# ZenGo-X/multi-party-ecdsa

Measured on AMD Instinct MI355X. Metric: GG20 signatures/sec (t=1, n=3; all parties of each session on the node's GPUs) + Paillier-2048 modexp/s per GPU, higher is better.
Workload: dtype u32 limbs (radix 2^29) / u64 accumulators

## Files before the change

multi_party_ecdsa_amd/csrc/mpe_gg20.h:

```cpp
#pragma once
#include <cstdio>
#include <cstdlib>

#include "mpe_gg20_msg.h"
#include "mpe_proofs.h"

namespace mpe {
namespace smp {
struct Bounds { uint32_t *q, *q3, *Nm2, *qNt, *q3Nt; };
__global__ void bounds_kernel(int count, const uint32_t* __restrict__ N, const uint32_t* __restrict__ Nt, Bounds b) {
  const int g = blockIdx.x * blockDim.x + threadIdx.x;
  if (g > count) return;
  const uint32_t q[8] = {0xD0364141u, 0xBFD25E8Cu, 0xAF48A03Bu, 0xBAAEDCE6u, 0xFFFFFFFEu, 0xFFFFFFFFu, 0xFFFFFFFFu, 0xFFFFFFFFu};
  uint32_t q2[16], q3[24];
  sm::mul(q2, q, 8, q, 8);
  sm::mul(q3, q2, 16, q, 8);
  if (g == count) {
    for (int j = 0; j < 8; ++j) b.q[j] = q[j];
    for (int j = 0; j < 24; ++j) b.q3[j] = q3[j];
    return;
  }
  const uint32_t two[1] = {2u};
  sm::sub(b.Nm2 + (size_t)g * 64, 64, N + (size_t)g * 64, 64, two, 1);
  sm::mul(b.qNt + (size_t)g * 72, Nt + (size_t)g * 64, 64, q, 8);
  sm::mul(b.q3Nt + (size_t)g * 88, Nt + (size_t)g * 64, 64, q3, 24);
}
}
}

struct mpe_gg20_keys {
  int t = 0, n = 0, S = 0, K = 1, n_own = 0;
  int signers[8] = {0};
  int nsets = 1;
  uint32_t sets4[256] = {0};
  uint32_t masks[256] = {0};
  uint32_t* d_sets = nullptr;
  int own[8] = {0};
  int own_slot[8] = {0};
  mpe_paillier* pub = nullptr;
  mpe_paillier* prv = nullptr;
  mpe_statements* stm = nullptr;
  void* blob = nullptr;
  size_t blob_bytes = 0;
  uint32_t* x = nullptr;
  uint32_t* X = nullptr;
  uint32_t* y = nullptr;
  uint32_t* gw = nullptr;
  mpe::smp::Bounds bounds{};
};

namespace mpe {
namespace gg {

struct Dim {
  int B, S, n, L, V, PV, K, n_own;
  int loc[8];
  int sg[8];
  int oslot[8];
  const int32_t* ks;
  ec::Enc enc;
  const int32_t* ss;
  const uint32_t* sets;
  uint32_t sg4;
  int nsets;
  int lparty;
};
__device__ __forceinline__ int ind_of(int i, int jj) { return jj < i ? jj : jj + 1; }
__device__ __forceinline__ int jme_of(int i, int ind) { return i < ind ? i : i - 1; }
__device__ __forceinline__ int ks_of(const Dim& d, int b) { return d.ks ? d.ks[b] : 0; }
__device__ __forceinline__ bool ss_valid(const Dim& d, int b) { return !d.ss || (unsigned)d.ss[b] < (unsigned)d.nsets; }
__device__ __forceinline__ int ss_of(const Dim& d, int b) { return d.ss && ss_valid(d, b) ? d.ss[b] : 0; }
__device__ __forceinline__ uint32_t set4_of(const Dim& d, int b) { return d.ss ? d.sets[ss_of(d, b)] : d.sg4; }
__device__ __forceinline__ int sg_of(const Dim& d, int b, int i) { return (int)((set4_of(d, b) >> (4 * i)) & 15u); }
__device__ __forceinline__ int rank_in(uint32_t set4, int S, int party) {
  int r = -1;
  for (int i = 0; i < S; ++i) if ((int)((set4 >> (4 * i)) & 15u) == party) r = i;
  return r;
}
__device__ __forceinline__ int loc_of(const Dim& d, int b, int li) {
  if (d.lparty < 0) return d.loc[li];
  const int r = rank_in(set4_of(d, b), d.S, d.lparty);
  return r < 0 ? 0 : r;
}
__device__ __forceinline__ int kpub(const Dim& d, int b, int i) { return ks_of(d, b) * d.n + sg_of(d, b, i); }
__device__ __forceinline__ int kown(const Dim& d, int b, int i) { return ks_of(d, b) * d.n_own + d.oslot[d.lparty >= 0 ? d.lparty : sg_of(d, b, i)]; }
__device__ __forceinline__ const uint32_t* gw_of(const Dim& d, const uint32_t* gw, int b, int ind) {
  return gw + (((size_t)ks_of(d, b) * d.nsets + ss_of(d, b)) * d.S + ind) * 16;
}

struct Slab { const uint32_t* p; long long off[8]; int W; };
__device__ __forceinline__ long long rec_index(const Slab& s, int j, int b) { return s.off[j] + b; }
__device__ __forceinline__ const uint32_t* rec_of(const Slab& s, int j, int b) { return s.p + (size_t)(s.off[j] + b) * (size_t)s.W; }

struct Idx {
  int32_t *kown_pi;
  int32_t *pi_ap, *kown_ap, *st_ap;
  int32_t *ca_vi, *kpub_vi, *st_vi;
  int32_t *ca_mb, *kpub_mb, *kown_mb;
  int32_t *pi_pp, *kown_pp, *st_pp;
  int32_t *ca_pv, *pi_pv, *kpub_pv, *st_pv;
};
__global__ void idx_kernel(Dim d, Idx x, int total) {
  const int g = blockIdx.x * blockDim.x + threadIdx.x;
  if (g >= total) return;
  const int S = d.S, n = d.n, L = d.L, P1 = S - 1;
  if (g < d.B * L) { const int b = g / L; x.kown_pi[g] = kown(d, b, loc_of(d, b, g % L)); }
  if (g < d.B * L * n) {
    const int pi = g / n, b = pi / L;
    x.pi_ap[g] = pi; x.kown_ap[g] = kown(d, b, loc_of(d, b, pi % L)); x.st_ap[g] = ks_of(d, b) * n + g % n;
  }
  if (g < d.B * L * P1 * d.V * n) {
    const int st = g % n, r1 = g / n, r2 = r1 / d.V, jj = r2 % P1, pi = r2 / P1, b = pi / L, i = loc_of(d, b, pi % L);
    const int ind = ind_of(i, jj);
    x.ca_vi[g] = ind * d.B + b; x.kpub_vi[g] = kpub(d, b, ind); x.st_vi[g] = ks_of(d, b) * n + st;
  }
  if (g < d.B * L * P1 * 2) {
    const int pp = g >> 1, jj = pp % P1, pi = pp / P1, b = pi / L, i = loc_of(d, b, pi % L), ind = ind_of(i, jj);
    x.ca_mb[g] = ind * d.B + b; x.kpub_mb[g] = kpub(d, b, ind); x.kown_mb[g] = kown(d, b, i);
  }
  if (g < d.B * L * P1) {
    const int jj = g % P1, pi = g / P1, b = pi / L, i = loc_of(d, b, pi % L);
    x.pi_pp[g] = pi; x.kown_pp[g] = kown(d, b, i); x.st_pp[g] = ks_of(d, b) * n + sg_of(d, b, ind_of(i, jj));
  }
  if (g < d.B * d.PV * S * P1) {
    const int jj = g % P1, r1 = g / P1, i = r1 % S, r2 = r1 / S, vl = r2 % d.PV, b = r2 / d.PV;
    x.ca_pv[g] = i * d.B + b; x.pi_pv[g] = b * L + vl; x.kpub_pv[g] = kpub(d, b, i);
    x.st_pv[g] = ks_of(d, b) * n + sg_of(d, b, ind_of(i, jj));
  }
}

__global__ void gather_field_kernel(Slab s, int S, int B, int src_off, int words, uint32_t* __restrict__ dst) {
  MPE_FOREGROUND();
  const size_t g = (size_t)blockIdx.x * blockDim.x + threadIdx.x;
  if (g >= (size_t)S * B * words) return;
  const int w = (int)(g % words);
  const size_t jb = g / words;
  dst[g] = rec_of(s, (int)(jb / B), (int)(jb % B))[src_off + w];
}
constexpr int NR = 9;
__device__ __forceinline__ void fail(int32_t* status, uint32_t* bad, int pi, int code, uint32_t mask) {
  if (status[pi] == 0) { status[pi] = code; bad[pi] = mask; }
}
__device__ __forceinline__ int resolve_status(const int32_t* status, size_t nPI, int pi, int upto, const uint32_t* bad, uint32_t* bad_out) {
  for (int r = 0; r <= upto; ++r) {
    const int st = status[(size_t)r * nPI + pi];
    if (st) { if (bad_out) *bad_out = bad[(size_t)r * nPI + pi]; return st; }
  }
  if (bad_out) *bad_out = 0;
  return 0;
}

__global__ void pack_field_kernel(int nitems, int per, int L, int B, int nsub, int sub0, int subw, int dst_off,
                                  const uint32_t* __restrict__ src, int words, const int32_t* __restrict__ status, int round,
                                  uint32_t* __restrict__ out) {
  MPE_FOREGROUND();
  const size_t g = (size_t)blockIdx.x * blockDim.x + threadIdx.x;
  if (g >= (size_t)nitems * words) return;
  const int w = (int)(g % words), item = (int)(g / words), pi = item / per, li = pi % L, b = pi / L;
  const bool stopped = resolve_status(status, (size_t)L * B, pi, round, nullptr, nullptr) != 0;
  out[((size_t)(li * B + b) * nsub + sub0 + item % per) * subw + dst_off + w] = stopped ? 0u : src[g];
}
__device__ __forceinline__ bool pt_ok(const uint32_t* p) { return ec::aff_valid(ec::aff_load(p)); }
__global__ void __launch_bounds__(64) validate_kernel(Dim d, Slab in, int round, int32_t* __restrict__ status, uint32_t* __restrict__ bad) {
  MPE_FOREGROUND();
  const int pi = blockIdx.x * blockDim.x + threadIdx.x;
  if (pi >= d.B * d.L) return;
  const int b = pi / d.L, i = loc_of(d, b, pi % d.L), P1 = d.S - 1;
  uint32_t mask = 0;
  for (int j = 0; j < d.S; ++j) {
    if (j == i) continue;
    const uint32_t* m = rec_of(in, j, b);
    bool good = true;
    if (round == 2) {
      for (int v = 0; v < 2; ++v) {
        const uint32_t* mb = m + (size_t)(jme_of(i, j) * 2 + v) * SUB1;
        good = good && pt_ok(mb + M1.b_pk.off) && pt_ok(mb + M1.b_R.off) && pt_ok(mb + M1.bt_pk.off) && pt_ok(mb + M1.bt_R.off);
      }
    } else if (round == 3) {
      good = pt_ok(m + M2.T.off) && pt_ok(m + M2.a1.off) && pt_ok(m + M2.a2.off) && pt_ok(m + M2.com.off);
    } else if (round == 4) {
      good = pt_ok(m + M3.g_gamma.off);
    } else if (round == 5) {
      for (int jj = 0; jj < P1; ++jj) good = good && pt_ok(m + (size_t)jj * SUB4 + M4P.u1.off);
      good = good && pt_ok(m + (size_t)P1 * SUB4 + M4R.R_dash.off);
    } else if (round == 6) {
      good = pt_ok(m + M5.S.off) && pt_ok(m + M5.T.off) && pt_ok(m + M5.A3.off);
    }
    if (!good) mask |= 1u << j;
  }
  if (mask) fail(status, bad, pi, 100 * round + 90, mask);
}

__device__ inline ec::U256 lagrange0(const int* sg, int S, int i) {
  ec::U256 num = ec::u256_one(), den = ec::u256_one();
  for (int j = 0; j < S; ++j) {
    if (j == i) continue;
    ec::U256 xj = ec::u256_zero(); xj.w[0] = (uint32_t)(sg[j] + 1);
    ec::U256 xi = ec::u256_zero(); xi.w[0] = (uint32_t)(sg[i] + 1);
    num = ec::sc_mul(num, xj);
    den = ec::sc_mul(den, ec::sc_sub(xj, xi));
  }
  return ec::sc_mul(num, ec::sc_inv(den));
}
__device__ inline ec::U256 lagrange0(uint32_t set4, int S, int i) {
  ec::U256 num = ec::u256_one(), den = ec::u256_one();
  ec::U256 xi = ec::u256_zero(); xi.w[0] = ((set4 >> (4 * i)) & 15u) + 1u;
  for (int j = 0; j < S; ++j) {
    if (j == i) continue;
    ec::U256 xj = ec::u256_zero(); xj.w[0] = ((set4 >> (4 * j)) & 15u) + 1u;
    num = ec::sc_mul(num, xj);
    den = ec::sc_mul(den, ec::sc_sub(xj, xi));
  }
  return ec::sc_mul(num, ec::sc_inv(den));
}
__global__ void __launch_bounds__(64) MPE_EC_OCC gw_kernel(Dim d, const uint32_t* __restrict__ Xs, uint32_t* __restrict__ gw) {
  const int g = blockIdx.x * blockDim.x + threadIdx.x;
  if (g >= d.K * d.nsets * d.S) return;
  const int kk = g / (d.nsets * d.S), j = g % d.S;
  const uint32_t set4 = d.sets[(g / d.S) % d.nsets];
  ec::aff_store(gw + (size_t)g * 16, ec::mul_aff(lagrange0(set4, d.S, j), ec::aff_load(Xs + ((size_t)kk * d.n + ((set4 >> (4 * j)) & 15u)) * 16)));
}

__global__ void __launch_bounds__(64) MPE_EC_OCC r0_kernel(Dim d, const uint32_t* __restrict__ xs, const uint32_t* __restrict__ k_in,
                          const uint32_t* __restrict__ gamma_in, const uint32_t* __restrict__ blind, uint32_t* __restrict__ kq,
                          uint32_t* __restrict__ gq, uint32_t* __restrict__ w, uint32_t* __restrict__ k64, uint32_t* __restrict__ g_gamma,
                          uint32_t* __restrict__ com, int32_t* __restrict__ status, uint32_t* __restrict__ bad) {
  const int pi = blockIdx.x * blockDim.x + threadIdx.x;
  if (pi >= d.B * d.L) return;
  const int b = pi / d.L, i = loc_of(d, b, pi % d.L);
  if (!ss_valid(d, b) || (d.lparty >= 0 && rank_in(set4_of(d, b), d.S, d.lparty) < 0)) fail(status, bad, pi, MPE_GG20_STATUS_BAD_SET, 0);
  const bool k_ok = ec::sc_is_canonical_nonzero(k_in + (size_t)pi * 8), g_ok = ec::sc_is_canonical_nonzero(gamma_in + (size_t)pi * 8);
  if (!k_ok || !g_ok) fail(status, bad, pi, MPE_GG20_STATUS_BAD_NONCE, 0);
  const ec::U256 k = ec::sc_reduce(k_in + (size_t)pi * 8, 8), g = ec::sc_reduce(gamma_in + (size_t)pi * 8, 8);
  const ec::U256 wi = ec::sc_mul(lagrange0(set4_of(d, b), d.S, i), ec::sc_reduce(xs + (size_t)kown(d, b, i) * 8, 8));
  ec::u256_store(kq + (size_t)pi * 8, k);
  ec::u256_store(gq + (size_t)pi * 8, g);
  ec::u256_store(w + (size_t)pi * 8, wi);
  for (int j = 0; j < 64; ++j) k64[(size_t)pi * 64 + j] = j < 8 ? k.w[j] : 0u;
  const ec::Aff gg = ec::jac_to_aff(ec::jac_mul_gen(g));
  ec::aff_store(g_gamma + (size_t)pi * 16, gg);
  ec::u256_store(com + (size_t)pi * 8, sig::commit_point(gg, blind + (size_t)pi * 8, d.enc));
}

__global__ void idx1_kernel(Dim d, Slab in0, int32_t* __restrict__ sub0_vi) {
  const int g = blockIdx.x * blockDim.x + threadIdx.x;
  const int P1 = d.S - 1;
  if (g >= d.B * d.L * P1 * d.V * d.n) return;
  const int st = g % d.n, r1 = g / d.n, r2 = r1 / d.V, jj = r2 % P1, pi = r2 / P1, b = pi / d.L, i = loc_of(d, b, pi % d.L);
  sub0_vi[g] = (int32_t)(rec_index(in0, ind_of(i, jj), b) * (d.n + 1) + st);
}
__global__ void mb_prep_kernel(Dim d, const uint32_t* __restrict__ gq, const uint32_t* __restrict__ w,
                               const uint32_t* __restrict__ beta_tag, uint32_t* __restrict__ bsel,
                               uint32_t* __restrict__ btq, uint32_t* __restrict__ beta) {
  const int mb = blockIdx.x * blockDim.x + threadIdx.x;
  if (mb >= d.B * d.L * (d.S - 1) * 2) return;
  const int pi = (mb >> 1) / (d.S - 1);
  const uint32_t* src = (mb & 1) ? w + (size_t)pi * 8 : gq + (size_t)pi * 8;
  for (int j = 0; j < 8; ++j) bsel[(size_t)mb * 8 + j] = src[j];
  const ec::U256 t = ec::sc_reduce(beta_tag + (size_t)mb * 64, 64);
  ec::u256_store(btq + (size_t)mb * 8, t);
  ec::u256_store(beta + (size_t)mb * 8, ec::sc_neg(t));
}
__global__ void status1_kernel(Dim d, const uint8_t* __restrict__ ok_vi, int32_t* __restrict__ status, uint32_t* __restrict__ bad) {
  const int pi = blockIdx.x * blockDim.x + threadIdx.x;
  if (pi >= d.B * d.L) return;
  const int per = (d.S - 1) * d.V * d.n;
  bool good = true;
  for (int q = 0; q < per; ++q) good = good && ok_vi[(size_t)pi * per + q];
  if (!good) fail(status, bad, pi, 101, 0);
}

__global__ void idx2_kernel(Dim d, Slab in1, int32_t* __restrict__ sub1_rv) {
  MPE_FOREGROUND();
  const int g = blockIdx.x * blockDim.x + threadIdx.x;
  const int P1 = d.S - 1;
  if (g >= d.B * d.L * P1 * 2) return;
  const int v = g & 1, pp = g >> 1, jj = pp % P1, pi = pp / P1, b = pi / d.L, i = loc_of(d, b, pi % d.L), ind = ind_of(i, jj);
  sub1_rv[g] = (int32_t)(rec_index(in1, ind, b) * (2 * P1) + jme_of(i, ind) * 2 + v);
}
__device__ __forceinline__ void r2a_finish(const Dim& d, int rv, int v, int pp, int b, int ind, const ec::Aff& Bpk, bool good,
                                           const uint32_t* gw, uint32_t* bpk_in, uint8_t* code) {
  uint8_t c = good ? 0 : 1;
  if (v == 1) { if (!c && !ec::aff_eq(Bpk, ec::aff_load(gw_of(d, gw, b, ind)))) c = 2; }
  else ec::aff_store(bpk_in + (size_t)pp * 16, Bpk);
  code[rv] = c;
}
__global__ void __launch_bounds__(64) MPE_EC_OCC r2a_kernel(Dim d, const int32_t* __restrict__ sub1_rv, const uint32_t* __restrict__ in1,
                           const uint32_t* __restrict__ alpha_full, const uint32_t* __restrict__ kq, const uint32_t* __restrict__ gw,
                           uint32_t* __restrict__ alpha, uint32_t* __restrict__ bpk_in, uint8_t* __restrict__ code) {
  MPE_FOREGROUND();
  const int rv = blockIdx.x * blockDim.x + threadIdx.x;
  const int P1 = d.S - 1;
  if (rv >= d.B * d.L * P1 * 2) return;
  const int v = rv & 1, pp = rv >> 1, jj = pp % P1, pi = pp / P1, b = pi / d.L, i = loc_of(d, b, pi % d.L), ind = ind_of(i, jj);
  const uint32_t* m = in1 + (size_t)sub1_rv[rv] * SUB1;
  const ec::U256 al = ec::sc_reduce(alpha_full + (size_t)rv * 64, 64);
  ec::u256_store(alpha + (size_t)rv * 8, al);
  const ec::Aff Bpk = ec::aff_load(m + M1.b_pk.off), BTpk = ec::aff_load(m + M1.bt_pk.off);
  const ec::Aff R1 = ec::aff_load(m + M1.b_R.off), R2 = ec::aff_load(m + M1.bt_R.off);
  const bool good = sig::mta_alpha_holds(al, ec::u256_load(kq + (size_t)pi * 8), Bpk, R1, ec::sc_reduce(m + M1.b_z.off, 8), BTpk, R2,
                                         ec::sc_reduce(m + M1.bt_z.off, 8), d.enc);
  r2a_finish(d, rv, v, pp, b, ind, Bpk, good, gw, bpk_in, code);
}

__global__ void __launch_bounds__(64) MPE_EC_OCC ped_ahead_kernel(Dim d, const uint32_t* __restrict__ l_in, const uint32_t* __restrict__ s1_in,
                                                       const uint32_t* __restrict__ s2_in, uint32_t* __restrict__ ped_pre) {
  const int pi = blockIdx.x * blockDim.x + threadIdx.x;
  if (pi >= d.B * d.L) return;
  uint32_t* o = ped_pre + (size_t)pi * 48;
  ec::aff_store(o, ec::jac_to_aff(ec::jac_mul_h2(ec::sc_reduce(l_in + (size_t)pi * 8, 8))));
  ec::aff_store(o + 16, ec::jac_to_aff(ec::jac_mul_gen(ec::sc_reduce(s1_in + (size_t)pi * 8, 8))));
  ec::aff_store(o + 32, ec::jac_to_aff(ec::jac_mul_h2(ec::sc_reduce(s2_in + (size_t)pi * 8, 8))));
}
struct Ped { uint32_t *T, *e, *a1, *a2, *z1, *z2; };
__global__ void __launch_bounds__(64) MPE_EC_OCC r2b_kernel(Dim d, const uint32_t* __restrict__ kq, const uint32_t* __restrict__ gq,
                           const uint32_t* __restrict__ w, const uint32_t* __restrict__ alpha,
                           const uint32_t* __restrict__ beta, const uint8_t* __restrict__ code, const uint32_t* __restrict__ l_in,
                           const uint32_t* __restrict__ s1_in, const uint32_t* __restrict__ s2_in,
                           uint32_t* __restrict__ delta_i, uint32_t* __restrict__ sigma_i, uint32_t* __restrict__ lq, Ped p,
                           int32_t* __restrict__ status, uint32_t* __restrict__ bad, const uint32_t* __restrict__ alpha_full,
                           uint32_t* __restrict__ miu, int fault_step, uint32_t fault_mask, const uint32_t* __restrict__ ped_pre) {
  MPE_FOREGROUND();
  const int pi = blockIdx.x * blockDim.x + threadIdx.x;
  if (pi >= d.B * d.L) return;
  const int P1 = d.S - 1;
  for (int jj = 0; jj < P1; ++jj)
    for (int w_ = 0; w_ < 64; ++w_) miu[((size_t)pi * P1 + jj) * 64 + w_] = alpha_full[(((size_t)pi * P1 + jj) * 2 + 1) * 64 + w_];
  const ec::U256 k = ec::u256_load(kq + (size_t)pi * 8);
  ec::U256 de = ec::sc_mul(k, ec::u256_load(gq + (size_t)pi * 8)), si = ec::sc_mul(k, ec::u256_load(w + (size_t)pi * 8));
  int st = 0;
  for (int jj = 0; jj < P1; ++jj) {
    const size_t m0 = ((size_t)pi * P1 + jj) * 2;
    de = ec::sc_add(de, ec::sc_add(ec::u256_load(alpha + m0 * 8), ec::u256_load(beta + m0 * 8)));
    si = ec::sc_add(si, ec::sc_add(ec::u256_load(alpha + (m0 + 1) * 8), ec::u256_load(beta + (m0 + 1) * 8)));
    for (int v = 0; v < 2 && !st; ++v) if (code[m0 + v]) st = 200 + code[m0 + v];
  }
  if (st) fail(status, bad, pi, st, 0);
  if ((fault_mask >> loc_of(d, pi / d.L, pi % d.L)) & 1u) {
    if (fault_step == 5) de = ec::sc_add(de, de);
    if (fault_step == 6) si = ec::sc_add(si, si);
  }
  ec::u256_store(delta_i + (size_t)pi * 8, de);
  ec::u256_store(sigma_i + (size_t)pi * 8, si);
  const ec::U256 l = ec::sc_reduce(l_in + (size_t)pi * 8, 8);
  ec::u256_store(lq + (size_t)pi * 8, l);
  const uint32_t* pre = ped_pre ? ped_pre + (size_t)pi * 48 : nullptr;
  const ec::Aff T = ec::jac_to_aff(ec::jac_add(ec::jac_mul_gen(si), pre ? ec::jac_from_aff(ec::aff_load(pre)) : ec::jac_mul_h2(l)));
  const ec::U256 s1 = ec::sc_reduce(s1_in + (size_t)pi * 8, 8), s2 = ec::sc_reduce(s2_in + (size_t)pi * 8, 8);
  const ec::Aff a1 = pre ? ec::aff_load(pre + 16) : ec::jac_to_aff(ec::jac_mul_gen(s1)), a2 = pre ? ec::aff_load(pre + 32) : ec::jac_to_aff(ec::jac_mul_h2(s2));
  ec::U256 e, z1, z2;
  sig::pedersen_prove_body(si, l, s1, s2, T, a1, a2, d.enc, e, z1, z2);
  ec::aff_store(p.T + (size_t)pi * 16, T);
  ec::u256_store(p.e + (size_t)pi * 8, e);
  ec::aff_store(p.a1 + (size_t)pi * 16, a1);
  ec::aff_store(p.a2 + (size_t)pi * 16, a2);
  ec::u256_store(p.z1 + (size_t)pi * 8, z1);
  ec::u256_store(p.z2 + (size_t)pi * 8, z2);
}

__device__ __forceinline__ bool words_eq(const uint32_t* a, const uint32_t* b, int n) {
  uint32_t o = 0;
  for (int i = 0; i < n; ++i) o |= a[i] ^ b[i];
  return o == 0;
}
__device__ __forceinline__ void r3_finish(int pi, bool com_ok, bool ped_ok, const ec::U256& sum, uint32_t* dinv, int32_t* status,
                                          uint32_t* bad) {
  if (!com_ok) fail(status, bad, pi, 303, 0);
  const bool inv_ok = !ec::u256_is_zero(sum);
  if (!inv_ok) fail(status, bad, pi, 301, 0);
  ec::u256_store(dinv + (size_t)pi * 8, inv_ok ? ec::sc_inv(sum) : ec::u256_zero());
  if (!ped_ok) fail(status, bad, pi, 302, 0);
}
__global__ void __launch_bounds__(64) MPE_EC_OCC r3_kernel(Dim d, Slab in2, uint32_t* __restrict__ dinv, int32_t* __restrict__ status,
                                                uint32_t* __restrict__ bad) {
  MPE_FOREGROUND();
  const int pi = blockIdx.x * blockDim.x + threadIdx.x;
  if (pi >= d.B * d.L) return;
  const int b = pi / d.L;
  ec::U256 sum = ec::u256_zero();
  bool com_ok = true, ped_ok = true;
  for (int j = 0; j < d.S; ++j) {
    const uint32_t* m = rec_of(in2, j, b);
    sum = ec::sc_add(sum, ec::sc_reduce(m + M2.delta.off, 8));
    com_ok = com_ok && words_eq(m + M2.T.off, m + M2.com.off, M2.T.words);
    const ec::Aff C = ec::aff_load(m + M2.com.off), a1 = ec::aff_load(m + M2.a1.off), a2 = ec::aff_load(m + M2.a2.off);
    const bool holds = sig::pedersen_verify_body(C, a1, a2, ec::sc_reduce(m + M2.z1.off, 8), ec::sc_reduce(m + M2.z2.off, 8), d.enc);
    ped_ok = ped_ok && holds;
  }
  r3_finish(pi, com_ok, ped_ok, sum, dinv, status, bad);
}

__global__ void __launch_bounds__(64) MPE_EC_OCC r4_kernel(Dim d, Slab in3, const uint32_t* __restrict__ dinv, const uint32_t* __restrict__ com_all,
                          const uint32_t* __restrict__ bpk_in, const uint32_t* __restrict__ kq, uint32_t* __restrict__ R,
                          uint32_t* __restrict__ Rbar, int32_t* __restrict__ status, uint32_t* __restrict__ bad, int with_rbar) {
  MPE_FOREGROUND();
  const int pi = blockIdx.x * blockDim.x + threadIdx.x;
  if (pi >= d.B * d.L) return;
  const int P1 = d.S - 1, b = pi / d.L, i = loc_of(d, b, pi % d.L);
  uint32_t mask = 0;
  for (int jj = 0; jj < P1; ++jj) {
    const int ind = ind_of(i, jj);
    const uint32_t* m = rec_of(in3, ind, b);
    const ec::Aff gg = ec::aff_load(m + M3.g_gamma.off);
    bool good = ec::aff_eq(ec::aff_load(bpk_in + ((size_t)pi * P1 + jj) * 16), gg);
    good = good && ec::u256_eq(sig::commit_point(gg, m + M3.blind.off, d.enc), ec::u256_load(com_all + ((size_t)ind * d.B + b) * 8));
    if (!good) mask |= 1u << ind;
  }
  if (mask) fail(status, bad, pi, 401, mask);
  ec::Jac acc = ec::jac_inf();
  for (int j = 0; j < d.S; ++j) acc = ec::jac_add(acc, ec::jac_from_aff(ec::aff_load(rec_of(in3, j, b) + M3.g_gamma.off)));
  const ec::Aff Rp = ec::mul_aff(ec::u256_load(dinv + (size_t)pi * 8), ec::jac_to_aff(acc));
  ec::aff_store(R + (size_t)pi * 16, Rp);
  if (with_rbar) ec::aff_store(Rbar + (size_t)pi * 16, ec::mul_aff(ec::u256_load(kq + (size_t)pi * 8), Rp));
}
__global__ void __launch_bounds__(64) MPE_EC_OCC r4_rbar_kernel(Dim d, const uint32_t* __restrict__ kq, const uint32_t* __restrict__ R, uint32_t* __restrict__ Rbar) {
  MPE_FOREGROUND();
  const int pi = blockIdx.x * blockDim.x + threadIdx.x;
  if (pi >= d.B * d.L) return;
  ec::aff_store(Rbar + (size_t)pi * 16, ec::mul_aff(ec::u256_load(kq + (size_t)pi * 8), ec::aff_load(R + (size_t)pi * 16)));
}

__global__ void idx5_kernel(Dim d, Slab in4, int32_t* __restrict__ sub4_pv, int32_t* __restrict__ rdash_pv) {
  const int g = blockIdx.x * blockDim.x + threadIdx.x;
  const int P1 = d.S - 1;
  if (g >= d.B * d.PV * d.S * P1) return;
  const int jj = g % P1, r1 = g / P1, i = r1 % d.S, b = r1 / d.S / d.PV;
  const long long r = rec_index(in4, i, b) * d.S;
  sub4_pv[g] = (int32_t)(r + jj); rdash_pv[g] = (int32_t)(r + P1);
}
struct Heg { uint32_t *S, *T, *A3, *z1, *z2; };
__global__ void __launch_bounds__(64) MPE_EC_OCC r5_status_kernel(Dim d, Slab in4, const uint8_t* __restrict__ pdl_ok, int32_t* __restrict__ status,
                                                       uint32_t* __restrict__ bad) {
  const int pi = blockIdx.x * blockDim.x + threadIdx.x;
  if (pi >= d.B * d.L) return;
  const int P1 = d.S - 1, li = pi % d.L, b = pi / d.L;
  const int vo = d.PV == 1 ? 0 : li;
  uint32_t mask = 0;
  for (int i = 0; i < d.S && !mask; ++i)
    for (int jj = 0; jj < P1; ++jj)
      if (!pdl_ok[(((size_t)b * d.PV + vo) * d.S + i) * P1 + jj]) mask = 1u << i;
  if (mask) fail(status, bad, pi, 501, mask);
  ec::Jac acc = ec::jac_inf();
  for (int j = 0; j < d.S; ++j) acc = ec::jac_add(acc, ec::jac_from_aff(ec::aff_load(rec_of(in4, j, b) + (size_t)P1 * SUB4 + M4R.R_dash.off)));
  if (!ec::jac_eq_aff(acc, ec::aff_gen())) fail(status, bad, pi, 502, 0);
}
__global__ void __launch_bounds__(64) MPE_EC_OCC r5_prove_kernel(Dim d, const uint32_t* __restrict__ R, const uint32_t* __restrict__ sigma_i,
                          const uint32_t* __restrict__ lq, const uint32_t* __restrict__ pedT, const uint32_t* __restrict__ s1_in,
                          const uint32_t* __restrict__ s2_in, Heg h) {
  const int pi = blockIdx.x * blockDim.x + threadIdx.x;
  if (pi >= d.B * d.L) return;
  const ec::Aff G = ec::aff_gen(), H = ec::aff_h2();
  const ec::Aff Rp = ec::aff_load(R + (size_t)pi * 16), T = ec::aff_load(pedT + (size_t)pi * 16);
  const ec::U256 si = ec::u256_load(sigma_i + (size_t)pi * 8), l = ec::u256_load(lq + (size_t)pi * 8);
  const ec::Aff Sp = ec::mul_aff(si, Rp);
  const ec::U256 s1 = ec::sc_reduce(s1_in + (size_t)pi * 8, 8), s2 = ec::sc_reduce(s2_in + (size_t)pi * 8, 8);
  ec::Aff TT, A3;
  ec::U256 z1, z2;
  sig::heg_prove_body<sig::VAR, sig::H2, sig::GEN>(l, si, s1, s2, Rp, H, G, T, Sp, d.enc, TT, A3, z1, z2);
  ec::aff_store(h.S + (size_t)pi * 16, Sp);
  ec::aff_store(h.T + (size_t)pi * 16, TT);
  ec::aff_store(h.A3 + (size_t)pi * 16, A3);
  ec::u256_store(h.z1 + (size_t)pi * 8, z1);
  ec::u256_store(h.z2 + (size_t)pi * 8, z2);
}

__global__ void __launch_bounds__(64) MPE_EC_OCC r6_kernel(Dim d, Slab in5, const uint32_t* __restrict__ R, const uint32_t* __restrict__ tvec,
                          const uint32_t* __restrict__ y, int32_t* __restrict__ status, uint32_t* __restrict__ bad) {
  const int pi = blockIdx.x * blockDim.x + threadIdx.x;
  if (pi >= d.B * d.L) return;
  const int b = pi / d.L;
  const ec::Aff G = ec::aff_gen(), H = ec::aff_h2(), Rp = ec::aff_load(R + (size_t)pi * 16);
  uint32_t mask = 0;
  ec::Jac acc = ec::jac_inf();
  for (int j = 0; j < d.S; ++j) {
    const uint32_t* m = rec_of(in5, j, b);
    const ec::Aff E = ec::aff_load(m + M5.S.off), TT = ec::aff_load(m + M5.T.off), A3 = ec::aff_load(m + M5.A3.off),
                  D = ec::aff_load(tvec + ((size_t)j * d.B + b) * 16);
    if (!sig::heg_verify_body<sig::VAR, sig::H2, sig::GEN>(Rp, H, G, D, E, TT, A3, ec::sc_reduce(m + M5.z1.off, 8), ec::sc_reduce(m + M5.z2.off, 8), d.enc))
      mask |= 1u << j;
    acc = ec::jac_add_aff(acc, E);
  }
  if (mask) fail(status, bad, pi, 601, mask);
  if (!ec::jac_eq_aff(acc, ec::aff_load(y + (size_t)ks_of(d, b) * 16))) fail(status, bad, pi, 602, 0);
}

struct JacSlots { ec::Jac v[64]; };

__global__ void __launch_bounds__(64) MPE_EC_OCC r2a_group_kernel(Dim d, const int32_t* __restrict__ sub1_rv, const uint32_t* __restrict__ in1,
                           const uint32_t* __restrict__ alpha_full, const uint32_t* __restrict__ kq, const uint32_t* __restrict__ gw,
                           uint32_t* __restrict__ alpha, uint32_t* __restrict__ bpk_in, uint8_t* __restrict__ code) {
  MPE_FOREGROUND();
  __shared__ JacSlots vs, fs;
  const int gid = blockIdx.x * 64 + threadIdx.x, rv = gid >> 2, sub = gid & 3, base = (int)threadIdx.x - sub;
  const int P1 = d.S - 1;
  const bool live = rv < d.B * d.L * P1 * 2;
  const int rvc = live ? rv : 0;
  const int v = rvc & 1, pp = rvc >> 1, jj = pp % P1, pi = pp / P1, b = pi / d.L, i = loc_of(d, b, pi % d.L), ind = ind_of(i, jj);
  const uint32_t* m = in1 + (size_t)sub1_rv[rvc] * SUB1;
  const ec::U256 al = ec::sc_reduce(alpha_full + (size_t)rvc * 64, 64);
  const ec::Aff Bpk = ec::aff_load(m + M1.b_pk.off), BTpk = ec::aff_load(m + M1.bt_pk.off);
  const ec::Aff R1 = ec::aff_load(m + M1.b_R.off), R2 = ec::aff_load(m + M1.bt_R.off);
  ec::Jac res = ec::jac_inf(), fr = ec::jac_inf();
  if (live && sub < 3) {
    const ec::U256 sc = sub == 0 ? ec::u256_load(kq + (size_t)pi * 8) : (sub == 1 ? sig::dlog_challenge(R1, Bpk, d.enc) : sig::dlog_challenge(R2, BTpk, d.enc));
    res = ec::jac_mul(sc, sub == 2 ? BTpk : Bpk);
    const ec::U256 fk = sub == 0 ? al : ec::sc_reduce(m + (sub == 1 ? M1.b_z.off : M1.bt_z.off), 8);
    fr = ec::jac_mul_gen(fk);
  }
  vs.v[threadIdx.x] = res;
  fs.v[threadIdx.x] = fr;
  __syncthreads();
  if (!live || sub) return;
  ec::u256_store(alpha + (size_t)rv * 8, al);
  const bool good = sig::mta_relation_holds(fs.v[base], vs.v[base], BTpk)
                    && sig::dlog_holds(fs.v[base + 1], vs.v[base + 1], R1) && sig::dlog_holds(fs.v[base + 2], vs.v[base + 2], R2);
  r2a_finish(d, rv, v, pp, b, ind, Bpk, good, gw, bpk_in, code);
}

__global__ void __launch_bounds__(64) MPE_EC_OCC r3_group_kernel(Dim d, int G, Slab in2, uint32_t* __restrict__ dinv, int32_t* __restrict__ status,
                                                      uint32_t* __restrict__ bad) {
  MPE_FOREGROUND();
  __shared__ JacSlots vs, fs;
  const int gid = blockIdx.x * 64 + threadIdx.x, pi = gid / G, sub = gid % G, base = (int)threadIdx.x - sub;
  const bool live = pi < d.B * d.L;
  const int b = live ? pi / d.L : 0;
  ec::Jac res = ec::jac_inf(), fr = ec::jac_inf();
  if (live && sub < d.S) {
    const uint32_t* m = rec_of(in2, sub, b);
    const ec::Aff C = ec::aff_load(m + M2.com.off), a1 = ec::aff_load(m + M2.a1.off), a2 = ec::aff_load(m + M2.a2.off);
    res = ec::jac_mul(sig::pedersen_challenge(C, a1, a2, d.enc), C);
  }
  if (live && sub < 2 * d.S) {
    const uint32_t* m = rec_of(in2, sub >> 1, b);
    fr = ec::jac_mul_fixed(ec::sc_reduce(m + ((sub & 1) ? M2.z2.off : M2.z1.off), 8), sub & 1);
  }
  vs.v[threadIdx.x] = res;
  fs.v[threadIdx.x] = fr;
  __syncthreads();
  if (!live || sub) return;
  ec::U256 sum = ec::u256_zero();
  bool com_ok = true, ped_ok = true;
  for (int j = 0; j < d.S; ++j) {
    const uint32_t* m = rec_of(in2, j, b);
    sum = ec::sc_add(sum, ec::sc_reduce(m + M2.delta.off, 8));
    com_ok = com_ok && words_eq(m + M2.T.off, m + M2.com.off, M2.T.words);
    const ec::Aff a1 = ec::aff_load(m + M2.a1.off), a2 = ec::aff_load(m + M2.a2.off);
    const bool holds = sig::pedersen_holds(fs.v[base + 2 * j], fs.v[base + 2 * j + 1], vs.v[base + j], a1, a2);
    ped_ok = ped_ok && holds;
  }
  r3_finish(pi, com_ok, ped_ok, sum, dinv, status, bad);
}

__global__ void __launch_bounds__(64) MPE_EC_OCC r6_group_kernel(Dim d, int G, Slab in5, const uint32_t* __restrict__ R, const uint32_t* __restrict__ tvec,
                          const uint32_t* __restrict__ y, int32_t* __restrict__ status, uint32_t* __restrict__ bad) {
  __shared__ JacSlots vs, fs;
  const int gid = blockIdx.x * 64 + threadIdx.x, pi = gid / G, sub = gid % G, base = (int)threadIdx.x - sub;
  const bool live = pi < d.B * d.L;
  const int pic = live ? pi : 0, b = pic / d.L;
  const ec::Aff Gp = ec::aff_gen(), H = ec::aff_h2(), Rp = ec::aff_load(R + (size_t)pic * 16);
  ec::Jac res = ec::jac_inf(), fr = ec::jac_inf();
  if (live && sub < 3 * d.S) {
    const int j = sub / 3, kind = sub % 3;
    const uint32_t* m = rec_of(in5, j, b);
    const ec::Aff E = ec::aff_load(m + M5.S.off), TT = ec::aff_load(m + M5.T.off), A3 = ec::aff_load(m + M5.A3.off),
                  D = ec::aff_load(tvec + ((size_t)j * d.B + b) * 16);
    const ec::U256 e = sig::heg_challenge(TT, A3, Rp, H, Gp, D, E, d.enc);
    res = ec::jac_mul(kind == 1 ? ec::sc_reduce(m + M5.z2.off, 8) : e, kind == 0 ? D : (kind == 1 ? Rp : E));
  }
  if (live && sub < 2 * d.S) {
    const uint32_t* m = rec_of(in5, sub >> 1, b);
    fr = ec::jac_mul_fixed(ec::sc_reduce(m + ((sub & 1) ? M5.z2.off : M5.z1.off), 8), (sub & 1) ? 0 : 1);
  }
  vs.v[threadIdx.x] = res;
  fs.v[threadIdx.x] = fr;
  __syncthreads();
  if (!live || sub) return;
  uint32_t mask = 0;
  ec::Jac acc = ec::jac_inf();
  for (int j = 0; j < d.S; ++j) {
    const uint32_t* m = rec_of(in5, j, b);
    const ec::Aff E = ec::aff_load(m + M5.S.off), TT = ec::aff_load(m + M5.T.off), A3 = ec::aff_load(m + M5.A3.off);
    if (!sig::heg_holds(fs.v[base + 2 * j], fs.v[base + 2 * j + 1], vs.v[base + 3 * j], TT, vs.v[base + 3 * j + 1], vs.v[base + 3 * j + 2], A3))
      mask |= 1u << j;
    acc = ec::jac_add_aff(acc, E);
  }
  if (mask) fail(status, bad, pi, 601, mask);
  if (!ec::jac_eq_aff(acc, ec::aff_load(y + (size_t)ks_of(d, b) * 16))) fail(status, bad, pi, 602, 0);
}

__global__ void __launch_bounds__(64) MPE_EC_OCC r7_kernel(Dim d, const uint32_t* __restrict__ msg, const uint32_t* __restrict__ R,
                          const uint32_t* __restrict__ kq, const uint32_t* __restrict__ sigma_i, uint32_t* __restrict__ mq,
                          uint32_t* __restrict__ rq, uint32_t* __restrict__ s_i, int fault_step, uint32_t fault_mask) {
  const int pi = blockIdx.x * blockDim.x + threadIdx.x;
  if (pi >= d.B * d.L) return;
  const int b = pi / d.L;
  const ec::U256 m = ec::sc_reduce(msg + (size_t)b * 8, 8), r = ec::sc_reduce(R + (size_t)pi * 16, 8);
  ec::u256_store(mq + (size_t)pi * 8, m);
  ec::u256_store(rq + (size_t)pi * 8, r);
  ec::U256 si = ec::sc_add(ec::sc_mul(m, ec::u256_load(kq + (size_t)pi * 8)), ec::sc_mul(r, ec::u256_load(sigma_i + (size_t)pi * 8)));
  if (fault_step == 7 && ((fault_mask >> loc_of(d, b, pi % d.L)) & 1u)) si = ec::sc_add(si, si);
  ec::u256_store(s_i + (size_t)pi * 8, si);
}
__device__ __forceinline__ bool output_signature_check(ec::U256& s, int& recid, const ec::U256& m, const ec::U256& r, const ec::U256& ry,
                                                       const uint32_t* y16) {
  recid = (int)(ry.w[0] & 1u);
  const ec::U256 neg = ec::sc_neg(s);
  {
    bool gt = false;
    for (int j = 7; j >= 0; --j) { if (s.w[j] != neg.w[j]) { gt = s.w[j] > neg.w[j]; break; } }
    if (gt) { s = neg; recid ^= 1; }
  }
  bool okv = !ec::u256_is_zero(s);
  if (okv) {
    const ec::U256 bi = ec::sc_inv(s), u1 = ec::sc_mul(m, bi), u2 = ec::sc_mul(r, bi);
    const ec::Aff V = ec::jac_to_aff(ec::jac_add(ec::jac_mul_gen(u1), ec::jac_mul(u2, ec::aff_load(y16))));
    okv = !V.inf && ec::u256_eq(ec::sc_reduce(V.x.w, 8), r);
  }
  return okv;
}
__global__ void __launch_bounds__(64) MPE_EC_OCC complete_kernel(Dim d, Slab in6, const uint32_t* __restrict__ R, const uint32_t* __restrict__ mq,
                          const uint32_t* __restrict__ rq, const uint32_t* __restrict__ s_i, const uint32_t* __restrict__ y,
                          int32_t* __restrict__ status, uint32_t* __restrict__ bad, uint32_t* __restrict__ r_out,
                          uint32_t* __restrict__ s_out, int32_t* __restrict__ recid_out) {
  const int pi = blockIdx.x * blockDim.x + threadIdx.x;
  if (pi >= d.B * d.L) return;
  const int li = pi % d.L, b = pi / d.L, i = loc_of(d, b, li);
  ec::U256 s = ec::u256_load(s_i + (size_t)pi * 8);
  for (int j = 0; j < d.S; ++j) if (j != i) s = ec::sc_add(s, ec::sc_reduce(rec_of(in6, j, b) + M7.s_i.off, 8));
  const ec::U256 m = ec::u256_load(mq + (size_t)pi * 8), r = ec::u256_load(rq + (size_t)pi * 8);
  const ec::U256 ry = ec::sc_reduce(R + (size_t)pi * 16 + 8, 8);
  int recid;
  const bool okv = output_signature_check(s, recid, m, r, ry, y + (size_t)ks_of(d, b) * 16);
  const size_t nPI = (size_t)d.B * d.L;
  if (!okv) fail(status + 8 * nPI, bad + 8 * nPI, pi, 701, 0);
  const bool good = resolve_status(status, nPI, pi, NR - 1, nullptr, nullptr) == 0;
  const size_t o = (size_t)li * d.B + b;
  ec::u256_store(r_out + o * 8, good ? r : ec::u256_zero());
  ec::u256_store(s_out + o * 8, good ? s : ec::u256_zero());
  recid_out[o] = good ? recid : 0;
}
__global__ void result_kernel(Dim d, const int32_t* __restrict__ status, const uint32_t* __restrict__ bad, const uint32_t* __restrict__ R,
                              int32_t* __restrict__ st_out, uint32_t* __restrict__ bad_out, uint32_t* __restrict__ R_out) {
  const int pi = blockIdx.x * blockDim.x + threadIdx.x;
  if (pi >= d.B * d.L) return;
  const size_t o = (size_t)(pi % d.L) * d.B + pi / d.L;
  uint32_t bm = 0;
  const int stv = resolve_status(status, (size_t)d.B * d.L, pi, NR - 1, bad, &bm);
  if (st_out) st_out[o] = stv;
  if (bad_out) bad_out[o] = bm;
  if (R_out) for (int j = 0; j < 16; ++j) R_out[o * 16 + j] = R[(size_t)pi * 16 + j];
}
__global__ void sign_finish_kernel(int B, int L, int b0, const int32_t* __restrict__ pst, const uint32_t* __restrict__ pr,
                                   const uint32_t* __restrict__ ps, const int32_t* __restrict__ prec, const uint32_t* __restrict__ pR,
                                   uint32_t* __restrict__ r_out, uint32_t* __restrict__ s_out, int32_t* __restrict__ recid_out,
                                   uint32_t* __restrict__ R_out, int32_t* __restrict__ status) {
  const int b = blockIdx.x * blockDim.x + threadIdx.x;
  if (b >= B) return;
  int st = 0;
  for (int li = 0; li < L; ++li) { const int s = pst[(size_t)li * B + b]; if (s && (!st || s < st)) st = s; }
  const size_t o = (size_t)b0 + b;
  for (int j = 0; j < 8; ++j) { r_out[o * 8 + j] = st ? 0u : pr[(size_t)b * 8 + j]; s_out[o * 8 + j] = st ? 0u : ps[(size_t)b * 8 + j]; }
  recid_out[o] = st ? 0 : prec[b];
  if (R_out) for (int j = 0; j < 16; ++j) R_out[o * 16 + j] = pR[(size_t)b * 16 + j];
  status[o] = st;
}

enum class PdlStage { idle, first_queued, ready };
struct Ahead {
  bool lockstep = false;
  uint32_t* cinv = nullptr;
  uint8_t* cinv_ok = nullptr; bool cinv_done = false;
  uint32_t* ped = nullptr;
  uint32_t *pdl_bn = nullptr, *pdl_scratch = nullptr;
  PdlStage pdl = PdlStage::idle;
};

}
}

struct mpe_gg20_session {
  mpe_ctx* ctx = nullptr;
  const mpe_gg20_keys* K = nullptr;
  int B = 0, L = 0, dedup = 0, next_round = 0;
  bool any_set = false;
  bool failed = false;
  mpe::gg::Dim d{};
  mpe_gg20_nonces Z{};
  void* mem = nullptr;
  size_t mem_bytes = 0;
  bool from_cache = false;
  mpe::gg::Idx ix{};
  uint32_t *kq = nullptr, *gq = nullptr, *w = nullptr, *k64 = nullptr, *g_gamma = nullptr, *com = nullptr, *c_a = nullptr, *beta = nullptr;
  uint32_t *ca_all = nullptr, *com_all = nullptr, *bpk_in = nullptr, *delta_i = nullptr, *sigma_i = nullptr, *lq = nullptr, *pedT = nullptr;
  uint32_t *tvec = nullptr, *dinv = nullptr, *R = nullptr, *Rbar = nullptr, *mq = nullptr, *rq = nullptr, *s_i = nullptr, *bad = nullptr;
  uint32_t *sig_r = nullptr, *sig_s = nullptr;
  uint32_t* miu = nullptr;
  int32_t *status = nullptr, *sig_recid = nullptr;
  int32_t *sub0_vi = nullptr, *sub4_pv = nullptr, *rdash_pv = nullptr;
  uint8_t *ok_vi = nullptr, *ok_pv = nullptr;
  mpe::gg::Ahead ahead{};
  int fault_step = 0;
  uint32_t fault_mask = 0;
  char* tmp = nullptr;
  size_t tmp_bytes = 0;
};

namespace mpe {
namespace gg {

static void gg_trace(const mpe_ctx* ctx, hipStream_t st, const char* what, int rc) {
  if (!ctx->gg20_trace) return;
  const hipError_t e = hipStreamSynchronize(st);
  fprintf(stderr, "[gg20] %-28s rc=%d sync=%s\n", what, rc, hipGetErrorString(e));
  fflush(stderr);
}
#define GG_LAUNCH(kernel, nitems, ...)                                                                   \
  do {                                                                                                    \
    if (rc == MPE_OK && (nitems) > 0)                                                                     \
      hipLaunchKernelGGL(kernel, dim3(blocks_for((int)(nitems), 64)), dim3(64), 0, st, __VA_ARGS__);      \
    gg_trace(s->ctx, st, #kernel, rc);                                                                            \
  } while (0)

static Counts counts_of(const Dim& d) { return counts_of(d.B, d.S, d.n, d.L, d.V, d.PV); }
static void dim_of_keys(Dim& d, const mpe_gg20_keys* K, const int32_t* d_keyset, const int32_t* d_sigset) {
  d.S = K->S; d.n = K->n; d.K = K->K; d.n_own = K->n_own; d.ks = d_keyset;
  d.ss = d_sigset; d.sets = K->d_sets; d.sg4 = K->sets4[0]; d.nsets = K->nsets; d.lparty = -1;
  for (int i = 0; i < 8; ++i) { d.sg[i] = K->signers[i]; d.oslot[i] = K->own_slot[i] < 0 ? 0 : K->own_slot[i]; }
}
static int local_parties(Dim& d, const mpe_gg20_keys* K, int n_local, const int32_t* h_local, const int32_t* d_sigset, int by_party) {
  if (n_local < 1 || n_local > K->S || !h_local) return MPE_E_ARG;
  d.L = n_local;
  for (int i = 0; i < 8; ++i) d.loc[i] = 0;
  if (by_party) {
    if (n_local != 1) { mpe_set_error_msg("gg20: one local party by index"); return MPE_E_ARG; }
    const int p = h_local[0];
    if (p < 0 || p >= K->n || K->own_slot[p] < 0) { mpe_set_error_msg("gg20: the local party's secrets are not in the key object"); return MPE_E_ARG; }
    if (d_sigset) { d.lparty = p; return MPE_OK; }
    for (int i = 0; i < K->S; ++i) if (K->signers[i] == p) { d.loc[0] = i; return MPE_OK; }
    mpe_set_error_msg("gg20: the local party is not a signer"); return MPE_E_ARG;
  }
  for (int i = 0; i < n_local; ++i) {
    if (h_local[i] < 0 || h_local[i] >= K->S || (i && h_local[i] <= h_local[i - 1])) return MPE_E_ARG;
    d.loc[i] = h_local[i];
    for (int k = 0; k < (d_sigset ? K->nsets : 1); ++k)
      if (K->own_slot[(K->sets4[k] >> (4 * h_local[i])) & 15u] < 0) { mpe_set_error_msg("gg20: a local party's secrets are not in the key object"); return MPE_E_ARG; }
  }
  return MPE_OK;
}
static bool small_batch(const mpe_ctx* ctx, size_t items) { return ctx->allow_par && items <= (size_t)ctx->par_items; }
static size_t ec_lanes_fit(const mpe_ctx* ctx) { return ctx->ec_lane_groups ? (size_t)ctx->cus * 4 * 64 * 2 / ctx->device_share : 0; }
static size_t layout(mpe_gg20_session* s, char* base) {
  const Dim& d = s->d;
  const Counts c = counts_of(d);
  Bump m(base);
  Idx& x = s->ix;
  x.kown_pi = m.i(c.nPI);
  x.pi_ap = m.i(c.nAP); x.kown_ap = m.i(c.nAP); x.st_ap = m.i(c.nAP);
  x.ca_vi = m.i(c.nVI); x.kpub_vi = m.i(c.nVI); x.st_vi = m.i(c.nVI);
  x.ca_mb = m.i(c.nMB); x.kpub_mb = m.i(c.nMB); x.kown_mb = m.i(c.nMB);
  x.pi_pp = m.i(c.nPP); x.kown_pp = m.i(c.nPP); x.st_pp = m.i(c.nPP);
  x.ca_pv = m.i(c.nPV); x.pi_pv = m.i(c.nPV); x.kpub_pv = m.i(c.nPV); x.st_pv = m.i(c.nPV);
  s->kq = m.w(c.nPI * 8); s->gq = m.w(c.nPI * 8); s->w = m.w(c.nPI * 8); s->k64 = m.w(c.nPI * 64);
  s->g_gamma = m.w(c.nPI * 16); s->com = m.w(c.nPI * 8); s->c_a = m.w(c.nPI * 128); s->beta = m.w(c.nMB * 8);
  s->ca_all = m.w(c.SB * 128); s->com_all = m.w(c.SB * 8); s->bpk_in = m.w(c.nPP * 16);
  s->delta_i = m.w(c.nPI * 8); s->sigma_i = m.w(c.nPI * 8); s->lq = m.w(c.nPI * 8); s->pedT = m.w(c.nPI * 16);
  s->tvec = m.w(c.SB * 16); s->dinv = m.w(c.nPI * 8); s->R = m.w(c.nPI * 16); s->Rbar = m.w(c.nPI * 16);
  s->mq = m.w(c.nPI * 8); s->rq = m.w(c.nPI * 8); s->s_i = m.w(c.nPI * 8); s->bad = m.w(c.nPI * NR);
  s->sig_r = m.w(c.nPI * 8); s->sig_s = m.w(c.nPI * 8); s->miu = m.w(c.nPP * 64);
  s->status = m.i(c.nPI * NR); s->sig_recid = m.i(c.nPI);
  s->sub0_vi = m.i(c.nVI); s->ok_vi = m.f(c.nVI); s->sub4_pv = m.i(c.nPV); s->rdash_pv = m.i(c.nPV); s->ok_pv = m.f(c.nPV);
  Ahead& a = s->ahead; const bool small = small_batch(s->ctx, c.nVI);
  a.cinv = small ? m.w(c.nVI * 128) : nullptr; a.cinv_ok = small ? m.f(c.nVI) : nullptr;
  a.ped = m.w(c.nPI * 48);
  a.pdl_bn = small ? m.w(c.nPP * 128) : nullptr; a.pdl_scratch = small ? m.w(modexp_nn_scratch_words(c.nPP)) : nullptr;
  s->tmp_bytes = tmp_bytes_of(c);
  s->tmp = (char*)m.take(s->tmp_bytes);
  return m.off;
}
static Slab slab_of(const mpe_gg20_session* s, const uint32_t* p, const int64_t* h_off, int round) {
  Slab sl;
  sl.p = p; sl.W = msg_words(s->d.S, s->d.n, round);
  for (int j = 0; j < 8; ++j) sl.off[j] = j < s->d.S ? (h_off ? (long long)h_off[j] : (long long)j * s->B) : 0;
  return sl;
}
static int round_enter(mpe_gg20_session* s, int round, const void* in, const void* out, bool need_in, bool need_out) {
  if (!s || (need_in && !in) || (need_out && !out)) return MPE_E_ARG;
  if (s->failed) { mpe_set_error_msg("gg20: a round call of this batch failed (or the batch was aborted): re-arm the session"); return MPE_E_ARG; }
  if (s->next_round != round) { mpe_set_error_msg("gg20: rounds must be run in order"); return MPE_E_ARG; }
  s->d.enc = s->ctx->enc;
  return MPE_OK;
}
static int round_exit(mpe_gg20_session* s, int rc, const char* what) {
  if (rc != MPE_OK) { s->failed = true; return rc; }
  const hipError_t e = hipGetLastError();
  if (e != hipSuccess) { s->failed = true; mpe_set_error(what, e); return MPE_E_HIP; }
  s->next_round++;
  return MPE_OK;
}
#define STAT(r) (s->status + (size_t)(r) * c.nPI)
#define BADR(r) (s->bad + (size_t)(r) * c.nPI)
#define PACK(nitems, per, nsub, sub0, subw, field, src)                                                                                 \
  GG_LAUNCH(pack_field_kernel, (size_t)(nitems) * (field).words, (int)(nitems), (int)(per), d.L, d.B, (int)(nsub), (int)(sub0), (int)(subw),   \
            (field).off, (const uint32_t*)(src), (field).words, s->status, s->next_round, d_out)

static bool round1_merges(const mpe_ctx* ctx, const Counts& c) {
  const bool par = small_batch(ctx, c.nVI);
  const size_t resident_groups = (size_t)ctx->cus * ctx->modexp_waves_per_cu * 16 / ctx->device_share;
  return ctx->merge_r1 && ctx->use_pair && ctx->use_multiexp && c.nVI > 0 && c.nMB > 0 && c.nVI + c.nMB < ((size_t)1 << 30) &&
         (!par || 4 * (c.nVI + c.nMB) > (size_t)ctx->merge_r1_quarters * resident_groups);
}
__global__ void ca_all_from_local_kernel(int S, int B, const uint32_t* __restrict__ c_a, uint32_t* __restrict__ ca_all) {
  const size_t g = (size_t)blockIdx.x * blockDim.x + threadIdx.x;
  if (g >= (size_t)S * B * 128) return;
  const int w = (int)(g % 128);
  const size_t jb = g / 128;
  const int ind = (int)(jb / B), b = (int)(jb % B);
  ca_all[g] = c_a[((size_t)b * S + ind) * 128 + w];
}
static size_t ws_need_inversion_ahead(const mpe_paillier* pk, size_t nVI) { return nVI * (128 + 128 + 1) * 4 + modinv_ws_words(pk->ms_nn, (int)nVI) * 4 + 16384; }

static bool pdl_ahead_eligible(const mpe_gg20_session* s, const Counts& c) {
  const mpe_ctx* ctx = s->ctx; const Ahead& a = s->ahead;
  return a.lockstep && a.pdl_bn && ctx->use_prio && !ctx->no_pdl_ahead && ctx->use_pair && ctx->use_crt && ctx->use_pown && c.nPP > 0 && small_batch(ctx, c.nPP);
}
static int pdl_ahead_queue(mpe_gg20_session* s, const Counts& c, bool finish) {
  mpe_ctx* ctx = s->ctx; const mpe_paillier* prv = s->K->prv; Ahead& a = s->ahead; hipStream_t sa = ctx->aux[1];
  const int phase = !finish ? 1 : (a.pdl == PdlStage::first_queued ? 2 : 0);
  const int keep = ctx->ladder_prio;
  ctx->ladder_prio = 0;
  const int rc = modexp_nn(ctx, prv, (int)c.nPP, sel_of(s->ix.kown_pp, prv->nkeys), rows(s->Z.pdl_beta, 64, nullptr, 64),
                           tab_rows(prv->N, 64, s->ix.kown_pp, prv->nkeys), 64, true, a.pdl_bn, sa, true, a.pdl_scratch, phase);
  ctx->ladder_prio = keep;
  if (rc == MPE_OK && !finish) a.pdl = PdlStage::first_queued;
  else if (rc == MPE_OK) { (void)hipEventRecord(ctx->ev_ahead, sa); a.pdl = PdlStage::ready; }
  gg_trace(ctx, sa, finish ? "PDL beta^N, ahead" : "PDL beta^N, first ladder, ahead", rc);
  return rc;
}
static Handed pdl_ahead_take(const mpe_gg20_session* s) { return s->ahead.pdl == PdlStage::ready ? Handed{s->ahead.pdl_bn, s->ctx->ev_ahead} : Handed{}; }
static void pdl_ahead_consumed(mpe_gg20_session* s) { if (s->ahead.pdl == PdlStage::ready) s->ahead.pdl = PdlStage::idle; }
static void ahead_drain(mpe_gg20_session* s, hipStream_t st) {
  mpe_ctx* ctx = s->ctx; Ahead& a = s->ahead;
  if (a.pdl == PdlStage::idle) return;
  if (a.pdl == PdlStage::first_queued) (void)hipEventRecord(ctx->ev_ahead, ctx->aux[1]);
  (void)hipStreamWaitEvent(st, ctx->ev_ahead, 0);
  a.pdl = PdlStage::idle;
}

static int round0(mpe_gg20_session* s, uint32_t* d_out, hipStream_t st) {
  int rc = round_enter(s, 0, nullptr, d_out, false, true);
  if (rc != MPE_OK) return rc;
  mpe_ctx* ctx = s->ctx; const mpe_gg20_keys* K = s->K; const Dim& d = s->d; const Counts c = counts_of(d); const mpe_gg20_nonces& Z = s->Z; Ahead& a = s->ahead;
  const int n = d.n;
  (void)hipMemsetAsync(d_out, 0, c.nPI * (size_t)msg_words(d.S, n, 0) * 4, st);
  const bool par = small_batch(ctx, c.nAP);
  const size_t nXN = c.nPI + c.nAP;
  bool all_local_in_order = d.L == d.S;
  for (int l = 0; l < d.L && all_local_in_order; ++l) all_local_in_order = d.loc[l] == l;
  const bool ahead = par && a.lockstep && a.cinv && all_local_in_order && !ctx->no_r1_inversion_ahead && round1_merges(ctx, c);
  a.cinv_done = false;
  if (par && rc == MPE_OK) {
    rc = ws_reserve(ctx, ws_need_encrypt((int)c.nPI) + ws_need_alice_generate((int)c.nAP) + nXN * (64 + 128 + 1 + CRT_WS_WORDS) * 4 + 65536 +
                         (ahead ? ws_need_inversion_ahead(K->pub, c.nVI) : 0), st);
    if (rc == MPE_OK) ctx->ws_hold++;
  }
  const bool held = par && rc == MPE_OK;
  const uint32_t *rn_pre = nullptr, *bn_pre = nullptr;
  Fork g(ctx, st, 2, held, 2);
  GG_LAUNCH(r0_kernel, c.nPI, d, K->x, Z.k, Z.gamma, Z.blind, s->kq, s->gq, s->w, s->k64, s->g_gamma, s->com, STAT(0), BADR(0));
  if (g.on) (void)hipEventRecord(ctx->ev_fork[0], st);
  GG_LAUNCH(ped_ahead_kernel, c.nPI, d, Z.l, Z.ped_s1, Z.ped_s2, a.ped);
  hipEvent_t xn_ready = nullptr;
  if (held && ctx->merge_xn) {
    hipStream_t sx = g.s(1);
    uint32_t* xs = ws_array<uint32_t>(ctx, nXN * 64);
    uint32_t* xn = ws_array<uint32_t>(ctx, nXN * 128);
    int32_t* kx = ws_array<int32_t>(ctx, nXN);
    if (!xs || !xn || !kx) rc = MPE_E_NOMEM;
    if (rc == MPE_OK) {
      (void)hipMemcpyAsync(xs, Z.r_a, c.nPI * 64 * 4, hipMemcpyDeviceToDevice, sx);
      (void)hipMemcpyAsync(xs + c.nPI * 64, Z.al_beta, c.nAP * 64 * 4, hipMemcpyDeviceToDevice, sx);
      (void)hipMemcpyAsync(kx, s->ix.kown_pi, c.nPI * 4, hipMemcpyDeviceToDevice, sx);
      (void)hipMemcpyAsync(kx + c.nPI, s->ix.kown_ap, c.nAP * 4, hipMemcpyDeviceToDevice, sx);
      rc = modexp_nn(ctx, K->prv, (int)nXN, key_selector(K->prv, kx), rows(xs, 64, nullptr, 64), key_rows(K->prv, K->prv->N, 64, kx), 64, true, xn, sx, true);
      rn_pre = xn; bn_pre = xn + c.nPI * 128;
      if (rc == MPE_OK && g.on) { (void)hipEventRecord(ctx->ev_mid, sx); xn_ready = ctx->ev_mid; }
    }
  }
  if (g.on) (void)hipStreamWaitEvent(g.s(1), ctx->ev_fork[0], 0);
  if (rc == MPE_OK) rc = paillier_encrypt(ctx, K->prv, (int)c.nPI, s->ix.kown_pi, s->k64, Z.r_a, s->c_a, true, g.s(1), rn_pre);
  gg_trace(s->ctx, st, "encrypt k", rc);
  hipEvent_t c_ready = nullptr;
  if (ahead && held && g.on && xn_ready && rc == MPE_OK) {
    hipStream_t sx = g.s(1);
    (void)hipEventRecord(ctx->ev_mid, sx); c_ready = ctx->ev_mid;
    hipLaunchKernelGGL(ca_all_from_local_kernel, dim3((unsigned)((c.SB * 128 + 255) / 256)), dim3(256), 0, sx, d.S, d.B, s->c_a, s->ca_all);
    Seq q{ctx, sx, (int)c.nVI};
    const Rows ksel = sel_of(s->ix.kpub_vi, K->pub->nkeys);
    uint8_t* ok = q.flags();
    uint32_t* cred = q.modmul(K->pub->ms_nn, ksel, rows(s->ca_all, 128, s->ix.ca_vi), rows(K->pub->ms_nn->one_words, 0, nullptr, 1));
    uint32_t* cinv = q.modinv(K->pub->ms_nn, ksel, rows(cred, 128), ok);
    rc = q.rc;
    if (rc == MPE_OK) {
      (void)hipMemcpyAsync(a.cinv, cinv, c.nVI * 128 * 4, hipMemcpyDeviceToDevice, sx);
      (void)hipMemcpyAsync(a.cinv_ok, ok, c.nVI, hipMemcpyDeviceToDevice, sx);
      a.cinv_done = true;
    }
    gg_trace(s->ctx, sx, "round 1's inversion, ahead", rc);
  }
  Bump t(s->tmp);
  const Round0Tmp r0 = Round0Tmp::carve(t, c);
  mpe_alice_proof ap{r0.z, r0.e, r0.s, r0.s1, r0.s2};
  mpe_alice_nonces an{Z.al_alpha, Z.al_beta, Z.al_gamma, Z.al_rho};
  if (rc == MPE_OK)
    rc = alice_generate(ctx, K->prv, K->stm, (int)c.nAP, s->ix.kown_ap, s->ix.st_ap, rows(s->kq, 8, s->ix.pi_ap),
                        rows(s->c_a, 128, s->ix.pi_ap), rows(Z.r_a, 64, s->ix.pi_ap), &an, &ap, st, &g, Handed{bn_pre, c_ready ? c_ready : xn_ready}, c_ready);
  g.join();
  if (rc == MPE_OK && c_ready && pdl_ahead_eligible(s, c)) { (void)hipStreamWaitEvent(ctx->aux[1], c_ready, 0); rc = pdl_ahead_queue(s, c, false); }
  if (held) ctx->ws_hold--;
  gg_trace(s->ctx, st, "alice_generate", rc);
  PACK(c.nAP, n, n + 1, 0, SUB0, M0A.z, ap.z); PACK(c.nAP, n, n + 1, 0, SUB0, M0A.e, ap.e); PACK(c.nAP, n, n + 1, 0, SUB0, M0A.s, ap.s);
  PACK(c.nAP, n, n + 1, 0, SUB0, M0A.s1, ap.s1); PACK(c.nAP, n, n + 1, 0, SUB0, M0A.s2, ap.s2);
  PACK(c.nPI, 1, n + 1, n, SUB0, M0L.c, s->c_a); PACK(c.nPI, 1, n + 1, n, SUB0, M0L.com, s->com);
  return round_exit(s, rc, "gg20 round0");
}

__global__ void gather_rows_kernel(int n, Rows src, int src_words, int words, uint32_t* __restrict__ dst) {
  const size_t g = (size_t)blockIdx.x * blockDim.x + threadIdx.x;
  if (g >= (size_t)n * words) return;
  const int w = (int)(g % words), i = (int)(g / words);
  dst[g] = w < src_words ? row_of(src, i)[w] : 0u;
}
static size_t ws_need_round1_merged(const mpe_paillier* pk, size_t nVI, size_t nMB) {
  return (nVI + nMB) * (size_t)(64 + 128 + 8 + 1 + 128) * 4 + nVI * (128 + 128 + 1) * 4 + modinv_ws_words(pk->ms_nn, (int)nVI) * 4 + 65536;
}
static int round1_merged_ladders(mpe_ctx* ctx, const mpe_paillier* pk, size_t nVI, const int32_t* kpub_vi, Rows cipher_vi, Rows s_vi, Rows e_vi,
                                 size_t nMB, const int32_t* kpub_mb, Rows ca_mb, const uint32_t* bsel, const uint32_t* mb_r,
                                 const uint32_t** m_vi, const uint8_t** inv_ok_vi, const uint32_t** x_mb, hipStream_t st,
                                 Handed cinv_pre = {}, const uint8_t* cinv_ok_pre = nullptr) {
  const size_t n = nVI + nMB;
  Seq q{ctx, st, (int)nVI};
  const Rows ksel = sel_of(kpub_vi, pk->nkeys);
  const uint8_t* inv_ok = cinv_ok_pre;
  const uint32_t* cinv = cinv_pre.p;
  cinv_pre.wait(st);
  if (!cinv_pre) {
    uint8_t* ok = q.flags();
    uint32_t* cred = q.modmul(pk->ms_nn, ksel, cipher_vi, rows(pk->ms_nn->one_words, 0, nullptr, 1));
    cinv = q.modinv(pk->ms_nn, ksel, rows(cred, 128), ok);
    inv_ok = ok;
  }
  if (q.rc != MPE_OK) return q.rc;
  uint32_t* b1 = ws_array<uint32_t>(ctx, n * 64);
  uint32_t* b2 = ws_array<uint32_t>(ctx, n * 128);
  uint32_t* e2 = ws_array<uint32_t>(ctx, n * 8);
  int32_t* key = ws_array<int32_t>(ctx, n);
  uint32_t* out = ws_array<uint32_t>(ctx, n * 128);
  if (!b1 || !b2 || !e2 || !key || !out) { mpe_set_error_msg("round1: workspace under-reserved"); return MPE_E_NOMEM; }
  auto gather = [&](size_t cnt, Rows src, int sw, int words, uint32_t* dst) {
    if (cnt) hipLaunchKernelGGL(gather_rows_kernel, dim3((unsigned)((cnt * words + 255) / 256)), dim3(256), 0, st, (int)cnt, src, sw, words, dst);
  };
  gather(nVI, s_vi, 64, 64, b1);              gather(nMB, rows(mb_r, 64), 64, 64, b1 + nVI * 64);
  gather(nVI, rows(cinv, 128), 128, 128, b2); gather(nMB, ca_mb, 128, 128, b2 + nVI * 128);
  gather(nVI, e_vi, 8, 8, e2);                gather(nMB, rows(bsel, 8), 8, 8, e2 + nVI * 8);
  (void)hipMemcpyAsync(key, kpub_vi, nVI * 4, hipMemcpyDeviceToDevice, st);
  (void)hipMemcpyAsync(key + nVI, kpub_mb, nMB * 4, hipMemcpyDeviceToDevice, st);
  MPE_TRY(modexp_nn2(ctx, pk, (int)n, key_selector(pk, key), rows(b1, 64, nullptr, 64), key_rows(pk, pk->N, 64, key), 64, rows(b2, 128), rows(e2, 8), 8, out, st));
  *m_vi = out; *inv_ok_vi = inv_ok; *x_mb = out + nVI * 128;
  return MPE_OK;
}

static int round1(mpe_gg20_session* s, const uint32_t* d_in, const int64_t* h_off, uint32_t* d_out, hipStream_t st) {
  int rc = round_enter(s, 1, d_in, d_out, true, true);
  if (rc != MPE_OK) return rc;
  mpe_ctx* ctx = s->ctx; const mpe_gg20_keys* K = s->K; const Dim& d = s->d; const Counts c = counts_of(d); const mpe_gg20_nonces& Z = s->Z;
  const int n = d.n, P1 = d.S - 1;
  const Slab in0 = slab_of(s, d_in, h_off, 0);
  (void)hipMemsetAsync(d_out, 0, c.nPI * (size_t)msg_words(d.S, n, 1) * 4, st);
  GG_LAUNCH(gather_field_kernel, c.SB * M0L.c.words, in0, d.S, d.B, n * SUB0 + M0L.c.off, M0L.c.words, s->ca_all);
  GG_LAUNCH(gather_field_kernel, c.SB * M0L.com.words, in0, d.S, d.B, n * SUB0 + M0L.com.off, M0L.com.words, s->com_all);
  Bump t(s->tmp);
  int32_t* sub0_vi = s->sub0_vi;
  uint8_t* ok_vi = s->ok_vi;
  const Round1Tmp r1 = Round1Tmp::carve(t, c);
  uint32_t *bsel = r1.bsel, *btq = r1.btq, *c_b = r1.c_b;
  uint32_t *Bpk = r1.Bpk, *BR = r1.BR, *Bz = r1.Bz, *BTpk = r1.BTpk, *BTR = r1.BTR, *BTz = r1.BTz;
  GG_LAUNCH(idx1_kernel, c.nVI, d, in0, sub0_vi);
  const bool par = small_batch(ctx, c.nVI);
  const bool merged = round1_merges(ctx, c);
  const bool ahead = merged && s->ahead.cinv_done;
  s->ahead.cinv_done = false;
  if (par && !merged && rc == MPE_OK) { rc = ws_reserve(ctx, ws_need_alice_verify((int)c.nVI) + ws_need_mul_add_enc((int)c.nMB), st); if (rc == MPE_OK) ctx->ws_hold++; }
  bool held = par && !merged && rc == MPE_OK;
  const uint32_t *m_vi = nullptr, *x_mb = nullptr;
  const uint8_t* inv_ok_vi = nullptr;
  AliceProofRows pr{rows(d_in + M0A.z.off, SUB0, sub0_vi), rows(d_in + M0A.e.off, SUB0, sub0_vi), rows(d_in + M0A.s.off, SUB0, sub0_vi),
                    rows(d_in + M0A.s1.off, SUB0, sub0_vi), rows(d_in + M0A.s2.off, SUB0, sub0_vi)};
  if (merged && rc == MPE_OK) {
    rc = ws_reserve(ctx, ws_need_alice_verify((int)c.nVI) + ws_need_mul_add_enc((int)c.nMB) + ws_need_round1_merged(K->pub, c.nVI, c.nMB), st);
    if (rc == MPE_OK) { ctx->ws_hold++; held = true; }
  }
  if (rc == MPE_OK && c.nMB > 0)
    hipLaunchKernelGGL(mb_prep_kernel, dim3(blocks_for((int)c.nMB, 64)), dim3(64), 0, st, d, s->gq, s->w, Z.mb_beta_tag, bsel, btq, s->beta);
  Fork g(ctx, st, 2, held && par, 2);
  hipEvent_t m_ready = nullptr;
  auto dlog_proofs = [&](hipStream_t sd) {
    if (rc != MPE_OK || c.nMB == 0) return;
    hipLaunchKernelGGL(dlog_prove_kernel, dim3(blocks_for((int)c.nMB, 64)), dim3(64), 0, sd, (int)c.nMB, ctx->enc, bsel, Z.mb_nonce_b, Bpk, BR, Bz);
    hipLaunchKernelGGL(dlog_prove_kernel, dim3(blocks_for((int)c.nMB, 64)), dim3(64), 0, sd, (int)c.nMB, ctx->enc, btq, Z.mb_nonce_bt, BTpk, BTR, BTz);
  };
  const bool dlog_first = ahead && g.on && !ctx->no_r1_dlog_first;
  if (dlog_first) dlog_proofs(st);
  {
    hipStream_t st2 = g.s(1);
    if (merged && rc == MPE_OK) {
      rc = round1_merged_ladders(ctx, K->pub, c.nVI, s->ix.kpub_vi, rows(s->ca_all, 128, s->ix.ca_vi), with_words(pr.s, 64), pr.e, c.nMB, s->ix.kpub_mb,
                                 rows(s->ca_all, 128, s->ix.ca_mb), bsel, Z.mb_r, &m_vi, &inv_ok_vi, &x_mb, st2,
                                 ahead ? Handed{s->ahead.cinv} : Handed{}, ahead ? s->ahead.cinv_ok : nullptr);
      if (rc == MPE_OK && g.on) { (void)hipEventRecord(ctx->ev_mid, st2); m_ready = ctx->ev_mid; }
      gg_trace(s->ctx, st2, "round 1 merged ladders", rc);
    }
    if (rc == MPE_OK)
      rc = paillier_mul_add_enc(ctx, K->pub, (int)c.nMB, s->ix.kpub_mb, rows(s->ca_all, 128, s->ix.ca_mb), rows(bsel, 8), 8, Z.mb_beta_tag,
                                Z.mb_r, c_b, st2, x_mb);
    gg_trace(s->ctx, st2, "MessageB ciphertext", rc);
    if (!dlog_first) dlog_proofs(st2);
  }
  if (rc == MPE_OK)
    rc = alice_verify(ctx, K->pub, K->stm, (int)c.nVI, s->ix.kpub_vi, s->ix.st_vi, rows(s->ca_all, 128, s->ix.ca_vi), pr, ok_vi, st, Handed{m_vi, m_ready}, inv_ok_vi);
  gg_trace(s->ctx, st, "alice_verify", rc);
  g.join();
  if (held) ctx->ws_hold--;
  GG_LAUNCH(status1_kernel, c.nPI, d, ok_vi, STAT(1), BADR(1));
  const int per = 2 * P1;
  PACK(c.nMB, per, per, 0, SUB1, M1.c, c_b); PACK(c.nMB, per, per, 0, SUB1, M1.b_pk, Bpk); PACK(c.nMB, per, per, 0, SUB1, M1.b_R, BR);
  PACK(c.nMB, per, per, 0, SUB1, M1.b_z, Bz); PACK(c.nMB, per, per, 0, SUB1, M1.bt_pk, BTpk); PACK(c.nMB, per, per, 0, SUB1, M1.bt_R, BTR);
  PACK(c.nMB, per, per, 0, SUB1, M1.bt_z, BTz);
  return round_exit(s, rc, "gg20 round1");
}

static int round2(mpe_gg20_session* s, const uint32_t* d_in, const int64_t* h_off, uint32_t* d_out, hipStream_t st) {
  int rc = round_enter(s, 2, d_in, d_out, true, true);
  if (rc != MPE_OK) return rc;
  mpe_ctx* ctx = s->ctx; const mpe_gg20_keys* K = s->K; const Dim& d = s->d; const Counts c = counts_of(d); const mpe_gg20_nonces& Z = s->Z;
  const Slab in1 = slab_of(s, d_in, h_off, 1);
  (void)hipMemsetAsync(d_out, 0, c.nPI * (size_t)W2 * 4, st);
  GG_LAUNCH(validate_kernel, c.nPI, d, in1, 2, STAT(2), BADR(2));
  Bump t(s->tmp);
  const Round2Tmp r2 = Round2Tmp::carve(t, c);
  int32_t* sub1_rv = r2.sub1_rv;
  uint32_t *alpha_full = r2.alpha_full, *alpha = r2.alpha;
  uint8_t* code = r2.code;
  Ped ped{s->pedT, r2.e, r2.a1, r2.a2, r2.z1, r2.z2};
  GG_LAUNCH(idx2_kernel, c.nMB, d, in1, sub1_rv);
  const bool pdl_ahead = rc == MPE_OK && pdl_ahead_eligible(s, c) && ensure_aux(ctx);
  if (pdl_ahead) { (void)hipEventRecord(ctx->ev_fork[0], st); (void)hipStreamWaitEvent(ctx->aux[1], ctx->ev_fork[0], 0); }
  if (rc == MPE_OK)
    rc = paillier_decrypt(ctx, K->prv, (int)c.nMB, s->ix.kown_mb, rows(d_in + M1.c.off, SUB1, sub1_rv), alpha_full, st);
  gg_trace(s->ctx, st, "decrypt", rc);
  if (pdl_ahead && rc == MPE_OK) rc = pdl_ahead_queue(s, c, true);
  if (c.nMB * 4 <= ec_lanes_fit(ctx)) GG_LAUNCH(r2a_group_kernel, c.nMB * 4, d, sub1_rv, d_in, alpha_full, s->kq, K->gw, alpha, s->bpk_in, code);
  else GG_LAUNCH(r2a_kernel, c.nMB, d, sub1_rv, d_in, alpha_full, s->kq, K->gw, alpha, s->bpk_in, code);
  GG_LAUNCH(r2b_kernel, c.nPI, d, s->kq, s->gq, s->w, alpha, s->beta, code, Z.l, Z.ped_s1, Z.ped_s2, s->delta_i, s->sigma_i, s->lq, ped,
            STAT(2), BADR(2), alpha_full, s->miu, s->fault_step, s->fault_mask, s->ahead.ped);
  PACK(c.nPI, 1, 1, 0, W2, M2.delta, s->delta_i); PACK(c.nPI, 1, 1, 0, W2, M2.T, ped.T); PACK(c.nPI, 1, 1, 0, W2, M2.e, ped.e);
  PACK(c.nPI, 1, 1, 0, W2, M2.a1, ped.a1); PACK(c.nPI, 1, 1, 0, W2, M2.a2, ped.a2); PACK(c.nPI, 1, 1, 0, W2, M2.com, ped.T);
  PACK(c.nPI, 1, 1, 0, W2, M2.z1, ped.z1); PACK(c.nPI, 1, 1, 0, W2, M2.z2, ped.z2);
  return round_exit(s, rc, "gg20 round2");
}

static int round3(mpe_gg20_session* s, const uint32_t* d_in, const int64_t* h_off, uint32_t* d_out, hipStream_t st) {
  int rc = round_enter(s, 3, d_in, d_out, true, true);
  if (rc != MPE_OK) return rc;
  mpe_ctx* ctx = s->ctx; const Dim& d = s->d; const Counts c = counts_of(d);
  const Slab in2 = slab_of(s, d_in, h_off, 2);
  (void)hipMemsetAsync(d_out, 0, c.nPI * (size_t)W3 * 4, st);
  GG_LAUNCH(validate_kernel, c.nPI, d, in2, 3, STAT(3), BADR(3));
  GG_LAUNCH(gather_field_kernel, c.SB * M2.T.words, in2, d.S, d.B, M2.T.off, M2.T.words, s->tvec);
  const int g3 = 2 * d.S <= 4 ? 4 : (2 * d.S <= 8 ? 8 : 16);
  if (c.nPI * g3 <= ec_lanes_fit(ctx)) GG_LAUNCH(r3_group_kernel, c.nPI * g3, d, g3, in2, s->dinv, STAT(3), BADR(3));
  else GG_LAUNCH(r3_kernel, c.nPI, d, in2, s->dinv, STAT(3), BADR(3));
  PACK(c.nPI, 1, 1, 0, W3, M3.blind, s->Z.blind); PACK(c.nPI, 1, 1, 0, W3, M3.g_gamma, s->g_gamma);
  return round_exit(s, rc, "gg20 round3");
}

static int round4(mpe_gg20_session* s, const uint32_t* d_in, const int64_t* h_off, uint32_t* d_out, hipStream_t st) {
  int rc = round_enter(s, 4, d_in, d_out, true, true);
  if (rc != MPE_OK) return rc;
  mpe_ctx* ctx = s->ctx; const mpe_gg20_keys* K = s->K; const Dim& d = s->d; const Counts c = counts_of(d); const mpe_gg20_nonces& Z = s->Z;
  const int S = d.S, P1 = S - 1;
  const Slab in3 = slab_of(s, d_in, h_off, 3);
  (void)hipMemsetAsync(d_out, 0, c.nPI * (size_t)msg_words(S, d.n, 4) * 4, st);
  GG_LAUNCH(validate_kernel, c.nPI, d, in3, 4, STAT(4), BADR(4));
  Fork g(ctx, st, 2, small_batch(ctx, c.nPP), 2);
  hipEvent_t R_ready = nullptr;
  if (rc == MPE_OK && c.nPI > 0) {
    hipLaunchKernelGGL(r4_kernel, dim3(blocks_for((int)c.nPI, 64)), dim3(64), 0, g.s(1), d, in3, s->dinv, s->com_all, s->bpk_in, s->kq, s->R, s->Rbar,
                       STAT(4), BADR(4), g.on ? 0 : 1);
    if (g.on) {
      (void)hipEventRecord(ctx->ev_mid, g.s(1)); R_ready = ctx->ev_mid;
      hipLaunchKernelGGL(r4_rbar_kernel, dim3(blocks_for((int)c.nPI, 64)), dim3(64), 0, g.s(1), d, s->kq, s->R, s->Rbar);
    }
  }
  Bump t(s->tmp);
  const Round4Tmp r4 = Round4Tmp::carve(t, c);
  mpe_pdl_proof pp{r4.z, r4.u1, r4.u2, r4.u3, r4.s1, r4.s2, r4.s3};
  mpe_pdl_nonces pn{Z.pdl_alpha, Z.pdl_beta, Z.pdl_rho, Z.pdl_gamma};
  if (rc == MPE_OK)
    rc = pdl_prove(ctx, K->prv, K->stm, (int)c.nPP, s->ix.kown_pp, s->ix.st_pp, rows(s->c_a, 128, s->ix.pi_pp), rows(s->Rbar, 16, s->ix.pi_pp),
                   rows(s->R, 16, s->ix.pi_pp), rows(s->kq, 8, s->ix.pi_pp), rows(Z.r_a, 64, s->ix.pi_pp), &pn, &pp, st, &g,
                   pdl_ahead_take(s), R_ready);
  else g.join();
  if (rc == MPE_OK) pdl_ahead_consumed(s);
  gg_trace(s->ctx, st, "pdl_prove", rc);
  PACK(c.nPP, P1, S, 0, SUB4, M4P.z, pp.z); PACK(c.nPP, P1, S, 0, SUB4, M4P.u1, pp.u1); PACK(c.nPP, P1, S, 0, SUB4, M4P.u2, pp.u2);
  PACK(c.nPP, P1, S, 0, SUB4, M4P.u3, pp.u3); PACK(c.nPP, P1, S, 0, SUB4, M4P.s1, pp.s1); PACK(c.nPP, P1, S, 0, SUB4, M4P.s2, pp.s2);
  PACK(c.nPP, P1, S, 0, SUB4, M4P.s3, pp.s3);
  PACK(c.nPI, 1, S, P1, SUB4, M4R.R_dash, s->Rbar);
  return round_exit(s, rc, "gg20 round4");
}

static int round5(mpe_gg20_session* s, const uint32_t* d_in, const int64_t* h_off, uint32_t* d_out, hipStream_t st) {
  int rc = round_enter(s, 5, d_in, d_out, true, true);
  if (rc != MPE_OK) return rc;
  mpe_ctx* ctx = s->ctx; const mpe_gg20_keys* K = s->K; const Dim& d = s->d; const Counts c = counts_of(d); const mpe_gg20_nonces& Z = s->Z;
  const Slab in4 = slab_of(s, d_in, h_off, 4);
  (void)hipMemsetAsync(d_out, 0, c.nPI * (size_t)W5 * 4, st);
  GG_LAUNCH(validate_kernel, c.nPI, d, in4, 5, STAT(5), BADR(5));
  Bump t(s->tmp);
  int32_t *sub4_pv = s->sub4_pv, *rdash_pv = s->rdash_pv;
  uint8_t* ok_pv = s->ok_pv;
  const Round5Tmp r5 = Round5Tmp::carve(t, c);
  Heg heg{r5.S, r5.T, r5.A3, r5.z1, r5.z2};
  GG_LAUNCH(idx5_kernel, c.nPV, d, in4, sub4_pv, rdash_pv);
  const bool par = small_batch(ctx, c.nPV);
  PdlProofRows pr{rows(d_in + M4P.z.off, SUB4, sub4_pv), rows(d_in + M4P.u1.off, SUB4, sub4_pv), rows(d_in + M4P.u2.off, SUB4, sub4_pv),
                  rows(d_in + M4P.u3.off, SUB4, sub4_pv), rows(d_in + M4P.s1.off, SUB4, sub4_pv), rows(d_in + M4P.s2.off, SUB4, sub4_pv),
                  rows(d_in + M4P.s3.off, SUB4, sub4_pv)};
  Fork g(ctx, st, 2, par, 2);
  if (rc == MPE_OK && c.nPI > 0)
    hipLaunchKernelGGL(r5_prove_kernel, dim3(blocks_for((int)c.nPI, 64)), dim3(64), 0, g.s(1), d, s->R, s->sigma_i, s->lq, s->pedT, Z.heg_s1, Z.heg_s2, heg);
  if (rc == MPE_OK)
    rc = pdl_verify(ctx, K->pub, K->stm, (int)c.nPV, s->ix.kpub_pv, s->ix.st_pv, rows(s->ca_all, 128, s->ix.ca_pv), rows(d_in + M4R.R_dash.off, SUB4, rdash_pv),
                    rows(s->R, 16, s->ix.pi_pv), pr, ok_pv, st);
  gg_trace(s->ctx, st, "pdl_verify", rc);
  g.join();
  GG_LAUNCH(r5_status_kernel, c.nPI, d, in4, ok_pv, STAT(5), BADR(5));
  PACK(c.nPI, 1, 1, 0, W5, M5.S, heg.S); PACK(c.nPI, 1, 1, 0, W5, M5.T, heg.T); PACK(c.nPI, 1, 1, 0, W5, M5.A3, heg.A3);
  PACK(c.nPI, 1, 1, 0, W5, M5.z1, heg.z1); PACK(c.nPI, 1, 1, 0, W5, M5.z2, heg.z2);
  return round_exit(s, rc, "gg20 round5");
}

static int round6(mpe_gg20_session* s, const uint32_t* d_in, const int64_t* h_off, hipStream_t st) {
  int rc = round_enter(s, 6, d_in, nullptr, true, false);
  if (rc != MPE_OK) return rc;
  mpe_ctx* ctx = s->ctx; const Dim& d = s->d; const Counts c = counts_of(d);
  const Slab in5 = slab_of(s, d_in, h_off, 5);
  GG_LAUNCH(validate_kernel, c.nPI, d, in5, 6, STAT(6), BADR(6));
  const int g6 = 3 * d.S <= 8 ? 8 : (3 * d.S <= 16 ? 16 : 32);
  if (c.nPI * g6 <= ec_lanes_fit(ctx)) GG_LAUNCH(r6_group_kernel, c.nPI * g6, d, g6, in5, s->R, s->tvec, s->K->y, STAT(6), BADR(6));
  else GG_LAUNCH(r6_kernel, c.nPI, d, in5, s->R, s->tvec, s->K->y, STAT(6), BADR(6));
  return round_exit(s, rc, "gg20 round6");
}

static int round7(mpe_gg20_session* s, const uint32_t* d_msg, uint32_t* d_out, hipStream_t st) {
  int rc = round_enter(s, 7, d_msg, d_out, true, true);
  if (rc != MPE_OK) return rc;
  const Dim& d = s->d; const Counts c = counts_of(d);
  GG_LAUNCH(r7_kernel, c.nPI, d, d_msg, s->R, s->kq, s->sigma_i, s->mq, s->rq, s->s_i, s->fault_step, s->fault_mask);
  PACK(c.nPI, 1, 1, 0, W6, M7.s_i, s->s_i);
  return round_exit(s, rc, "gg20 round7");
}
static int complete(mpe_gg20_session* s, const uint32_t* d_in, const int64_t* h_off, hipStream_t st) {
  int rc = round_enter(s, 8, d_in, nullptr, true, false);
  if (rc != MPE_OK) return rc;
  const Dim& d = s->d; const Counts c = counts_of(d);
  const Slab in6 = slab_of(s, d_in, h_off, 7);
  GG_LAUNCH(complete_kernel, c.nPI, d, in6, s->R, s->mq, s->rq, s->s_i, s->K->y, s->status, s->bad, s->sig_r, s->sig_s, s->sig_recid);
  return round_exit(s, rc, "gg20 complete");
}

static void launch_idx(mpe_gg20_session* s, hipStream_t st) {
  const Counts c = counts_of(s->d);
  size_t total = 0;
  for (const size_t v : {c.nVI, c.nMB, c.nAP, c.nPV, c.nPI}) if (v > total) total = v;
  hipLaunchKernelGGL(idx_kernel, dim3(blocks_for((int)total, 64)), dim3(64), 0, st, s->d, s->ix, (int)total);
}
static hipError_t wipe_batch_state(mpe_gg20_session* s, hipStream_t st) {
  ahead_drain(s, st);
  return hipMemsetAsync(s->kq, 0, (size_t)((char*)s->mem + s->mem_bytes - (char*)s->kq), st);
}

static void session_release(mpe_gg20_session* s, hipStream_t st) {
  if (!s) return;
  ahead_drain(s, st);
  if (s->mem) {
    (void)hipMemsetAsync(s->mem, 0, s->mem_bytes, st);
    if (s->from_cache) s->ctx->sess_in_use = false;
    else { (void)hipStreamSynchronize(st); (void)hipFree(s->mem); }
  }
  delete s;
}

}
}

extern "C" {

int mpe_gg20_keys_create(mpe_ctx* ctx, int t, int n, int n_signers, const int32_t* h_signers, int nkeysets, int n_own,
                         const int32_t* h_own, const uint32_t* d_x, const uint32_t* d_p, const uint32_t* d_q, const uint32_t* d_N,
                         const uint32_t* d_Nt, const uint32_t* d_h1, const uint32_t* d_h2, const uint32_t* d_y, const uint32_t* d_X,
                         mpe_gg20_keys** out, void* stream) {
  return mpe_gg20_keys_create_sets(ctx, t, n, n_signers, 1, h_signers, nkeysets, n_own, h_own, d_x, d_p, d_q, d_N, d_Nt, d_h1, d_h2, d_y, d_X, out, stream);
}

int mpe_gg20_keys_create_sets(mpe_ctx* ctx, int t, int n, int n_signers, int n_sets, const int32_t* h_sets, int nkeysets, int n_own,
                              const int32_t* h_own, const uint32_t* d_x, const uint32_t* d_p, const uint32_t* d_q, const uint32_t* d_N,
                              const uint32_t* d_Nt, const uint32_t* d_h1, const uint32_t* d_h2, const uint32_t* d_y, const uint32_t* d_X,
                              mpe_gg20_keys** out, void* stream) {
  const int32_t* h_signers = h_sets;
  if (!ctx || !h_signers || !h_own || !d_x || !d_p || !d_q || !d_N || !d_Nt || !d_h1 || !d_h2 || !d_y || !d_X || !out) return MPE_E_ARG;
  if (n < 2 || n > 8 || n_signers < 2 || n_signers > n || t < 1 || n_signers <= t || nkeysets < 1 || n_own < 1 || n_own > n) return MPE_E_ARG;
  if (n_sets < 1 || n_sets > 256) return MPE_E_ARG;
  uint32_t sets4[256], masks[256];
  for (int k = 0; k < n_sets; ++k) {
    const int32_t* row = h_sets + (size_t)k * n_signers;
    sets4[k] = 0; masks[k] = 0;
    for (int i = 0; i < n_signers; ++i) {
      if (row[i] < 0 || row[i] >= n || (i && row[i] <= row[i - 1])) return MPE_E_ARG;
      sets4[k] |= (uint32_t)row[i] << (4 * i); masks[k] |= 1u << row[i];
    }
    for (int m = 0; m < k; ++m) if (sets4[m] == sets4[k]) { mpe_set_error_msg("gg20 keys: two equal signer sets"); return MPE_E_ARG; }
  }
  for (int i = 0; i < n_own; ++i)
    if (h_own[i] < 0 || h_own[i] >= n || (i && h_own[i] <= h_own[i - 1])) return MPE_E_ARG;
  hipStream_t st = (hipStream_t)stream;
  mpe_gg20_keys* K = new (std::nothrow) mpe_gg20_keys();
  if (!K) return MPE_E_NOMEM;
  K->t = t; K->n = n; K->S = n_signers; K->K = nkeysets; K->n_own = n_own; K->nsets = n_sets;
  for (int k = 0; k < n_sets; ++k) { K->sets4[k] = sets4[k]; K->masks[k] = masks[k]; }
  for (int a = 0; a < 8; ++a) K->own_slot[a] = -1;
  for (int i = 0; i < n_signers; ++i) K->signers[i] = h_signers[i];
  for (int i = 0; i < n_own; ++i) { K->own[i] = h_own[i]; K->own_slot[h_own[i]] = i; }
  const size_t kk = (size_t)nkeysets;
  const size_t ngw = kk * n_sets * n_signers;
  const size_t words = kk * n_own * 8 + kk * n * 16 + kk * 16 + ngw * 16 + 32 + kk * n * (64 + 72 + 88) + 2 * (size_t)n_sets;
  hipError_t e = hipMalloc(&K->blob, words * 4);
  if (e != hipSuccess) { delete K; mpe_set_error("hipMalloc(gg20 keys)", e); return MPE_E_NOMEM; }
  K->blob_bytes = words * 4;
  K->x = (uint32_t*)K->blob; K->X = K->x + kk * n_own * 8; K->y = K->X + kk * n * 16; K->gw = K->y + kk * 16;
  K->bounds.q = K->gw + ngw * 16; K->bounds.q3 = K->bounds.q + 8; K->bounds.Nm2 = K->bounds.q3 + 24;
  K->bounds.qNt = K->bounds.Nm2 + kk * n * 64; K->bounds.q3Nt = K->bounds.qNt + kk * n * 72;
  K->d_sets = K->bounds.q3Nt + kk * n * 88;
  (void)hipMemcpyAsync(K->d_sets, K->sets4, (size_t)n_sets * 4, hipMemcpyHostToDevice, st);
  (void)hipMemcpyAsync(K->d_sets + n_sets, K->masks, (size_t)n_sets * 4, hipMemcpyHostToDevice, st);
  hipLaunchKernelGGL(mpe::smp::bounds_kernel, dim3(mpe::blocks_for(nkeysets * n + 1, 64)), dim3(64), 0, st, nkeysets * n, d_N, d_Nt, K->bounds);
  (void)hipMemcpyAsync(K->x, d_x, kk * n_own * 8 * 4, hipMemcpyDeviceToDevice, st);
  (void)hipMemcpyAsync(K->X, d_X, kk * n * 16 * 4, hipMemcpyDeviceToDevice, st);
  (void)hipMemcpyAsync(K->y, d_y, kk * 16 * 4, hipMemcpyDeviceToDevice, st);
  {
    mpe::gg::Dim d{};
    d.S = n_signers; d.n = n; d.K = nkeysets; d.nsets = n_sets; d.sets = K->d_sets; d.lparty = -1;
    hipLaunchKernelGGL(mpe::gg::gw_kernel, dim3(mpe::blocks_for((int)ngw, 64)), dim3(64), 0, st, d, K->X, K->gw);
  }
  int rc = mpe_paillier_create_public(ctx, nkeysets * n, d_N, &K->pub, stream);
  if (rc == MPE_OK) rc = mpe_paillier_create_private(ctx, nkeysets * n_own, d_p, d_q, &K->prv, stream);
  if (rc == MPE_OK) {
    size_t free_b = 0, total_b = 0;
    (void)hipMemGetInfo(&free_b, &total_b);
    size_t budget = ctx->fb_budget_bytes ? ctx->fb_budget_bytes : free_b / 4;
    if (!ctx->fb_budget_bytes && mpe_statements_table_bytes(nkeysets * n, 4) > budget && mpe_statements_table_bytes(nkeysets * n, 4) <= free_b / 2) budget = free_b / 2;
    int wb = ctx->fb_window_bits;
    while (wb > 4 && mpe_statements_table_bytes(nkeysets * n, wb) > budget) --wb;
    if (mpe_statements_table_bytes(nkeysets * n, wb) > budget) wb = 0;
    rc = mpe_statements_create_wb(ctx, nkeysets * n, d_Nt, d_h1, d_h2, wb, &K->stm, stream);
  }
  if (rc != MPE_OK) { mpe_gg20_keys_destroy(K); return rc; }
  *out = K;
  return MPE_OK;
}

int mpe_gg20_keys_destroy(mpe_gg20_keys* K) {
  if (!K) return MPE_E_ARG;
  if (K->pub) mpe_paillier_destroy(K->pub);
  if (K->prv) mpe_paillier_destroy(K->prv);
  if (K->stm) mpe_statements_destroy(K->stm);
  if (K->blob) { (void)hipMemset(K->blob, 0, K->blob_bytes); (void)hipFree(K->blob); }
  delete K;
  return MPE_OK;
}
int mpe_gg20_keys_fb_window_bits(const mpe_gg20_keys* K) { return (K && K->stm) ? K->stm->fb_wb : MPE_E_ARG; }

int mpe_gg20_msg_words(int n_signers, int n, int round) { return mpe::gg::msg_words(n_signers, n, round); }

int mpe_gg20_session_create(mpe_ctx* ctx, const mpe_gg20_keys* keys, int batch, int n_local, const int32_t* h_local,
                            const int32_t* d_keyset, const mpe_gg20_nonces* nonces, int dedup_verify, mpe_gg20_session** out, void* stream) {
  return mpe_gg20_session_create_sets(ctx, keys, batch, n_local, h_local, d_keyset, nullptr, 0, nonces, dedup_verify, out, stream);
}
int mpe_gg20_session_create_sets(mpe_ctx* ctx, const mpe_gg20_keys* keys, int batch, int n_local, const int32_t* h_local, const int32_t* d_keyset,
                                 const int32_t* d_sigset, int local_by_party, const mpe_gg20_nonces* nonces, int dedup_verify,
                                 mpe_gg20_session** out, void* stream) {
  if (!ctx || !keys || !nonces || !out || batch <= 0 || n_local < 1 || n_local > keys->S || !h_local) return MPE_E_ARG;
  mpe::gg::Dim d0{};
  mpe::gg::dim_of_keys(d0, keys, d_keyset, d_sigset);
  MPE_TRY(mpe::gg::local_parties(d0, keys, n_local, h_local, d_sigset, local_by_party));
  if (keys->K > 1 && !d_keyset) return MPE_E_ARG;
  hipStream_t st = (hipStream_t)stream;
  mpe_gg20_session* s = new (std::nothrow) mpe_gg20_session();
  if (!s) return MPE_E_NOMEM;
  s->ctx = ctx; s->K = keys; s->B = batch; s->L = n_local; s->dedup = dedup_verify ? 1 : 0; s->Z = *nonces; s->any_set = d_sigset != nullptr;
  mpe::gg::Dim& d = s->d;
  d = d0;
  d.B = batch; d.V = dedup_verify ? 1 : 2; d.PV = dedup_verify ? 1 : n_local; d.enc = ctx->enc;
  const size_t bytes = mpe::gg::layout(s, nullptr);
  if (!ctx->sess_in_use) {
    if (bytes > ctx->sess_bytes) {
      if (ctx->sess_buf) { (void)hipStreamSynchronize(st); (void)hipFree(ctx->sess_buf); ctx->sess_buf = nullptr; ctx->sess_bytes = 0; }
      const hipError_t e = hipMalloc(&ctx->sess_buf, bytes);
      if (e != hipSuccess) { delete s; mpe_set_error("hipMalloc(gg20 session)", e); return MPE_E_NOMEM; }
      ctx->sess_bytes = bytes;
    }
    s->mem = ctx->sess_buf; s->from_cache = true; ctx->sess_in_use = true;
  } else {
    const hipError_t e = hipMalloc(&s->mem, bytes);
    if (e != hipSuccess) { delete s; mpe_set_error("hipMalloc(gg20 session)", e); return MPE_E_NOMEM; }
  }
  s->mem_bytes = bytes;
  (void)mpe::gg::layout(s, (char*)s->mem);
  const mpe::gg::Counts c = mpe::gg::counts_of(d);
  (void)hipMemsetAsync(s->status, 0, c.nPI * mpe::gg::NR * 4, st);
  (void)hipMemsetAsync(s->bad, 0, c.nPI * mpe::gg::NR * 4, st);
  mpe::gg::launch_idx(s, st);
  const hipError_t e = hipGetLastError();
  if (e != hipSuccess) { mpe_set_error("gg20 idx_kernel", e); mpe::gg::session_release(s, st); return MPE_E_HIP; }
  *out = s;
  return MPE_OK;
}
int mpe_gg20_session_destroy(mpe_gg20_session* s, void* stream) {
  if (!s) return MPE_E_ARG;
  mpe::gg::session_release(s, (hipStream_t)stream);
  return MPE_OK;
}

int mpe_gg20_session_rearm(mpe_gg20_session* s, const int32_t* d_keyset, const mpe_gg20_nonces* nonces, void* stream) {
  return mpe_gg20_session_rearm_sets(s, d_keyset, nullptr, nonces, stream);
}
int mpe_gg20_session_rearm_sets(mpe_gg20_session* s, const int32_t* d_keyset, const int32_t* d_sigset, const mpe_gg20_nonces* nonces, void* stream) {
  if (!s || !nonces) return MPE_E_ARG;
  if (s->K->K > 1 && !d_keyset) return MPE_E_ARG;
  if (d_sigset && !s->any_set) { mpe_set_error_msg("gg20 session rearm: the session was created without per-session signer sets"); return MPE_E_ARG; }
  if (s->next_round != 0 && s->next_round <= 8 && !s->failed) { mpe_set_error_msg("gg20 session rearm: the previous batch has not completed (finish it, or mpe_gg20_session_abort)"); return MPE_E_ARG; }
  hipStream_t st = (hipStream_t)stream;
  const hipError_t em = mpe::gg::wipe_batch_state(s, st);
  if (em != hipSuccess) { mpe_set_error("gg20 session rearm (wipe)", em); return MPE_E_HIP; }
  s->Z = *nonces; s->d.ks = d_keyset; s->d.ss = d_sigset; s->next_round = 0; s->failed = false; s->fault_step = 0; s->fault_mask = 0;
  mpe::gg::launch_idx(s, st);
  const hipError_t e = hipGetLastError();
  if (e != hipSuccess) { mpe_set_error("gg20 session rearm", e); return MPE_E_HIP; }
  return MPE_OK;
}

int mpe_gg20_session_abort(mpe_gg20_session* s, void* stream) {
  if (!s) return MPE_E_ARG;
  const hipError_t em = mpe::gg::wipe_batch_state(s, (hipStream_t)stream);
  if (em != hipSuccess) { mpe_set_error("gg20 session abort (wipe)", em); return MPE_E_HIP; }
  s->failed = true;
  s->next_round = 9;
  return MPE_OK;
}

int mpe_gg20_session_fault_inject(mpe_gg20_session* s, int step, uint32_t party_mask) {
  if (!s || (step != 0 && step != 5 && step != 6 && step != 7)) return MPE_E_ARG;
  s->fault_step = step; s->fault_mask = party_mask;
  return MPE_OK;
}
int mpe_gg20_round0(mpe_gg20_session* s, uint32_t* d_out, void* stream) { return s ? mpe::gg::round0(s, d_out, (hipStream_t)stream) : MPE_E_ARG; }
int mpe_gg20_round1(mpe_gg20_session* s, const uint32_t* d_in, const int64_t* h_in_off, uint32_t* d_out, void* stream) {
  return s ? mpe::gg::round1(s, d_in, h_in_off, d_out, (hipStream_t)stream) : MPE_E_ARG;
}
int mpe_gg20_round2(mpe_gg20_session* s, const uint32_t* d_in, const int64_t* h_in_off, uint32_t* d_out, void* stream) {
  return s ? mpe::gg::round2(s, d_in, h_in_off, d_out, (hipStream_t)stream) : MPE_E_ARG;
}
int mpe_gg20_round3(mpe_gg20_session* s, const uint32_t* d_in, const int64_t* h_in_off, uint32_t* d_out, void* stream) {
  return s ? mpe::gg::round3(s, d_in, h_in_off, d_out, (hipStream_t)stream) : MPE_E_ARG;
}
int mpe_gg20_round4(mpe_gg20_session* s, const uint32_t* d_in, const int64_t* h_in_off, uint32_t* d_out, void* stream) {
  return s ? mpe::gg::round4(s, d_in, h_in_off, d_out, (hipStream_t)stream) : MPE_E_ARG;
}
int mpe_gg20_round5(mpe_gg20_session* s, const uint32_t* d_in, const int64_t* h_in_off, uint32_t* d_out, void* stream) {
  return s ? mpe::gg::round5(s, d_in, h_in_off, d_out, (hipStream_t)stream) : MPE_E_ARG;
}
int mpe_gg20_round6(mpe_gg20_session* s, const uint32_t* d_in, const int64_t* h_in_off, void* stream) {
  return s ? mpe::gg::round6(s, d_in, h_in_off, (hipStream_t)stream) : MPE_E_ARG;
}
int mpe_gg20_round7(mpe_gg20_session* s, const uint32_t* d_msg, uint32_t* d_out, void* stream) {
  return s ? mpe::gg::round7(s, d_msg, d_out, (hipStream_t)stream) : MPE_E_ARG;
}
int mpe_gg20_complete(mpe_gg20_session* s, const uint32_t* d_in, const int64_t* h_in_off, void* stream) {
  return s ? mpe::gg::complete(s, d_in, h_in_off, (hipStream_t)stream) : MPE_E_ARG;
}
int mpe_gg20_session_result(const mpe_gg20_session* s, int32_t* d_status, uint32_t* d_bad_actors, uint32_t* d_r, uint32_t* d_s,
                            int32_t* d_recid, uint32_t* d_R, void* stream) {
  if (!s) return MPE_E_ARG;
  hipStream_t st = (hipStream_t)stream;
  const mpe::gg::Counts c = mpe::gg::counts_of(s->d);
  hipLaunchKernelGGL(mpe::gg::result_kernel, dim3(mpe::blocks_for((int)c.nPI, 64)), dim3(64), 0, st, s->d, s->status, s->bad, s->R, d_status,
                     d_bad_actors, d_R);
  if (s->next_round > 8) {
    if (d_r) (void)hipMemcpyAsync(d_r, s->sig_r, c.nPI * 32, hipMemcpyDeviceToDevice, st);
    if (d_s) (void)hipMemcpyAsync(d_s, s->sig_s, c.nPI * 32, hipMemcpyDeviceToDevice, st);
    if (d_recid) (void)hipMemcpyAsync(d_recid, s->sig_recid, c.nPI * 4, hipMemcpyDeviceToDevice, st);
  } else if (d_r || d_s || d_recid) {
    mpe_set_error_msg("gg20: the signature exists after mpe_gg20_complete");
    return MPE_E_ARG;
  }
  const hipError_t e = hipGetLastError();
  if (e != hipSuccess) { mpe_set_error("gg20 result", e); return MPE_E_HIP; }
  return MPE_OK;
}

}

namespace mpe {
namespace gg {

struct LockstepChunk {
  mpe_gg20_session* s;
  int b0, B;
  const uint32_t* msg;
  uint32_t* M6;
  int32_t* pst; uint32_t *pr, *ps; int32_t* prec; uint32_t* pR;
};
template <class Tail>
static int lockstep_pass(mpe_ctx* ctx, const mpe_gg20_keys* keys, int batch, const int32_t* d_keyset, const int32_t* d_sigset, const mpe_gg20_nonces* nonces,
                         int dedup_verify, int chunk, void* stream, Tail tail) {
  const int S = keys->S, n = keys->n;
  for (int k = 0; k < (d_sigset ? keys->nsets : 1); ++k)
    for (int i = 0; i < S; ++i)
      if (keys->own_slot[(keys->sets4[k] >> (4 * i)) & 15u] < 0) { mpe_set_error_msg("mpe_gg20_sign needs every signer's secrets"); return MPE_E_ARG; }
  hipStream_t st = (hipStream_t)stream;
  int maxw = 0;
  for (int r = 0; r < 8; ++r) { const int w = mpe::gg::msg_words(S, n, r); if (w > maxw) maxw = w; }
  if (chunk <= 0) {
    const size_t P = (size_t)S * (S - 1), V = dedup_verify ? 1 : 2, PV = dedup_verify ? 1 : S;
    const size_t nVI = P * V * n, nPV = PV * P;
    const size_t words = (size_t)S * 1200 + (size_t)S * n * 260 + nVI * 8 + P * 2 * 300 + P * 470 + nPV * 8 +
                         (nVI > nPV ? nVI : nPV) * 2300 + (size_t)S * n * 2100 +
                         2 * (size_t)S * maxw;
    size_t fit = ((size_t)64 << 30) / (words * 4);
    fit = fit >= 1024 ? (fit / 1024) * 1024 : (fit ? fit : 1);
    chunk = (int)(fit < 65536 ? fit : 65536);
  }
  int32_t local[8];
  for (int i = 0; i < S; ++i) local[i] = i;
  const int Bc = batch < chunk ? batch : chunk;
  size_t slab_off[7];
  const size_t slab_one = (size_t)S * Bc * maxw, slab_words = 2 * slab_one;
  for (int q = 0; q < 7; ++q) slab_off[q] = (q & 1) ? slab_one : 0;
  const size_t res_words = (size_t)S * Bc * (1 + 8 + 8 + 1 + 16);
  const size_t need = (slab_words + res_words) * 4 + 4096;
  if (need > ctx->slab_bytes) {
    if (ctx->slab_buf) { (void)hipStreamSynchronize(st); (void)hipFree(ctx->slab_buf); ctx->slab_buf = nullptr; ctx->slab_bytes = 0; }
    const hipError_t e = hipMalloc(&ctx->slab_buf, need);
    if (e != hipSuccess) { mpe_set_error("hipMalloc(gg20 message slabs)", e); return MPE_E_NOMEM; }
    ctx->slab_bytes = need;
  }
  uint32_t* M[7];
  for (int q = 0; q < 7; ++q) M[q] = (uint32_t*)ctx->slab_buf + slab_off[q];
  int32_t* pst = (int32_t*)((uint32_t*)ctx->slab_buf + slab_words);
  uint32_t* pr = (uint32_t*)(pst + (size_t)S * Bc);
  uint32_t* ps = pr + (size_t)S * Bc * 8;
  int32_t* prec = (int32_t*)(ps + (size_t)S * Bc * 8);
  uint32_t* pR = (uint32_t*)(prec + (size_t)S * Bc);
  for (int b0 = 0; b0 < batch; b0 += chunk) {
    const int B = batch - b0 < chunk ? batch - b0 : chunk;
    const size_t oPI = (size_t)b0 * S, oAP = oPI * n, oPP = oPI * (S - 1), oMB = oPP * 2;
    mpe_gg20_nonces Z = *nonces;
    Z.k += oPI * 8; Z.gamma += oPI * 8; Z.blind += oPI * 8; Z.r_a += oPI * 64;
    Z.al_alpha += oAP * 24; Z.al_beta += oAP * 64; Z.al_gamma += oAP * 88; Z.al_rho += oAP * 72;
    Z.mb_beta_tag += oMB * 64; Z.mb_r += oMB * 64; Z.mb_nonce_b += oMB * 8; Z.mb_nonce_bt += oMB * 8;
    Z.l += oPI * 8; Z.ped_s1 += oPI * 8; Z.ped_s2 += oPI * 8;
    Z.pdl_alpha += oPP * 24; Z.pdl_beta += oPP * 64; Z.pdl_rho += oPP * 72; Z.pdl_gamma += oPP * 88;
    Z.heg_s1 += oPI * 8; Z.heg_s2 += oPI * 8;
    if (Z.msg) Z.msg += (size_t)b0 * 8;
    mpe_gg20_session* s = nullptr;
    int rc = mpe_gg20_session_create_sets(ctx, keys, B, S, local, d_keyset ? d_keyset + b0 : nullptr, d_sigset ? d_sigset + b0 : nullptr, 0, &Z, dedup_verify, &s, stream);
    if (rc != MPE_OK) return rc;
    s->ahead.lockstep = true;
    rc = mpe::gg::round0(s, M[0], st);
    if (rc == MPE_OK) rc = mpe::gg::round1(s, M[0], nullptr, M[1], st);
    if (rc == MPE_OK) rc = mpe::gg::round2(s, M[1], nullptr, M[2], st);
    if (rc == MPE_OK) rc = mpe::gg::round3(s, M[2], nullptr, M[3], st);
    if (rc == MPE_OK) rc = mpe::gg::round4(s, M[3], nullptr, M[4], st);
    if (rc == MPE_OK) rc = mpe::gg::round5(s, M[4], nullptr, M[5], st);
    if (rc == MPE_OK) rc = mpe::gg::round6(s, M[5], nullptr, st);
    if (rc == MPE_OK) rc = tail(LockstepChunk{s, b0, B, Z.msg, M[6], pst, pr, ps, prec, pR}, st);
    mpe::gg::session_release(s, st);
    if (rc != MPE_OK) return rc;
  }
  (void)hipMemsetAsync(ctx->slab_buf, 0, need, st);
  return mpe_ctx_wipe(ctx, stream);
}

}
}

extern "C" {

int mpe_gg20_sign(mpe_ctx* ctx, const mpe_gg20_keys* keys, int batch, const int32_t* d_keyset, const mpe_gg20_nonces* nonces, uint32_t* d_r,
                  uint32_t* d_s, int32_t* d_recid, uint32_t* d_R, int32_t* d_status, int dedup_verify, int chunk, void* stream) {
  return mpe_gg20_sign_sets(ctx, keys, batch, d_keyset, nullptr, nonces, d_r, d_s, d_recid, d_R, d_status, dedup_verify, chunk, stream);
}
int mpe_gg20_sign_sets(mpe_ctx* ctx, const mpe_gg20_keys* keys, int batch, const int32_t* d_keyset, const int32_t* d_sigset, const mpe_gg20_nonces* nonces,
                       uint32_t* d_r, uint32_t* d_s, int32_t* d_recid, uint32_t* d_R, int32_t* d_status, int dedup_verify, int chunk, void* stream) {
  if (!ctx || !keys || !nonces || !d_r || !d_s || !d_recid || !d_status || batch < 0) return MPE_E_ARG;
  const int S = keys->S;
  return mpe::gg::lockstep_pass(ctx, keys, batch, d_keyset, d_sigset, nonces, dedup_verify, chunk, stream, [&](const mpe::gg::LockstepChunk& c, hipStream_t st) {
    int rc = mpe::gg::round7(c.s, c.msg, c.M6, st);
    if (rc == MPE_OK) rc = mpe::gg::complete(c.s, c.M6, nullptr, st);
    if (rc == MPE_OK) rc = mpe_gg20_session_result(c.s, c.pst, nullptr, c.pr, c.ps, c.prec, c.pR, stream);
    if (rc == MPE_OK)
      hipLaunchKernelGGL(mpe::gg::sign_finish_kernel, dim3(mpe::blocks_for(c.B, 64)), dim3(64), 0, st, c.B, S, c.b0, c.pst, c.pr, c.ps, c.prec, c.pR, d_r, d_s,
                         d_recid, d_R, d_status);
    return rc;
  });
}

}
```

multi_party_ecdsa_amd/csrc/mpe_gg20_msg.h:

```cpp
#pragma once
#include <algorithm>
#include <cstddef>
#include <cstdint>

namespace mpe {
namespace gg {

struct Field { int off, words; };
struct NamedField { const char* name; Field f; };

constexpr int SUB0 = 256, SUB1 = 208, W2 = 96, W3 = 24, SUB4 = 450, W5 = 64, W6 = 8;

constexpr struct { Field z{0, 64}, e{64, 8}, s{72, 64}, s1{136, 25}, s2{161, 89}; } M0A{};
constexpr struct { Field c{0, 128}, com{128, 8}; } M0L{};
constexpr struct { Field c{0, 128}, b_pk{128, 16}, b_R{144, 16}, b_z{160, 8}, bt_pk{168, 16}, bt_R{184, 16}, bt_z{200, 8}; } M1{};
constexpr struct { Field delta{0, 8}, T{8, 16}, e{24, 8}, a1{32, 16}, a2{48, 16}, com{64, 16}, z1{80, 8}, z2{88, 8}; } M2{};
constexpr struct { Field blind{0, 8}, g_gamma{8, 16}; } M3{};
constexpr struct { Field z{0, 64}, u1{64, 16}, u2{80, 128}, u3{208, 64}, s1{272, 25}, s2{297, 64}, s3{361, 89}; } M4P{};
constexpr struct { Field R_dash{0, 16}; } M4R{};
constexpr struct { Field S{0, 16}, T{16, 16}, A3{32, 16}, z1{48, 8}, z2{56, 8}; } M5{};
constexpr struct { Field s_i{0, 8}; } M7{};

constexpr NamedField M0A_FIELDS[] = {{"z", M0A.z}, {"e", M0A.e}, {"s", M0A.s}, {"s1", M0A.s1}, {"s2", M0A.s2}};
constexpr NamedField M0L_FIELDS[] = {{"c", M0L.c}, {"com", M0L.com}};
constexpr NamedField M1_FIELDS[] = {{"c", M1.c}, {"b_pk", M1.b_pk}, {"b_R", M1.b_R}, {"b_z", M1.b_z},
                                    {"bt_pk", M1.bt_pk}, {"bt_R", M1.bt_R}, {"bt_z", M1.bt_z}};
constexpr NamedField M2_FIELDS[] = {{"delta", M2.delta}, {"T", M2.T}, {"e", M2.e}, {"a1", M2.a1}, {"a2", M2.a2}, {"com", M2.com},
                                    {"z1", M2.z1}, {"z2", M2.z2}};
constexpr NamedField M3_FIELDS[] = {{"blind", M3.blind}, {"g_gamma", M3.g_gamma}};
constexpr NamedField M4P_FIELDS[] = {{"z", M4P.z}, {"u1", M4P.u1}, {"u2", M4P.u2}, {"u3", M4P.u3}, {"s1", M4P.s1}, {"s2", M4P.s2},
                                     {"s3", M4P.s3}};
constexpr NamedField M4R_FIELDS[] = {{"R_dash", M4R.R_dash}};
constexpr NamedField M5_FIELDS[] = {{"S", M5.S}, {"T", M5.T}, {"A3", M5.A3}, {"z1", M5.z1}, {"z2", M5.z2}};
constexpr NamedField M7_FIELDS[] = {{"s_i", M7.s_i}};

template <class Record, int N>
constexpr int packed_end(const Record&, const NamedField (&fields)[N]) {
  if (sizeof(Record) != N * sizeof(Field)) return -1;
  int end = 0;
  for (int i = 0; i < N; ++i) {
    if (fields[i].f.off < end || fields[i].f.words <= 0) return -1;
    end = fields[i].f.off + fields[i].f.words;
  }
  return end;
}
static_assert(packed_end(M0A, M0A_FIELDS) == 250 && 250 <= SUB0, "Alice sub-record: 250 words, padded to SUB0 (part of the format)");
static_assert(packed_end(M0L, M0L_FIELDS) > 0 && packed_end(M0L, M0L_FIELDS) <= SUB0, "M0 last sub-record");
static_assert(packed_end(M1, M1_FIELDS) == SUB1, "M1 MessageB sub-record");
static_assert(packed_end(M2, M2_FIELDS) == W2, "M2");
static_assert(packed_end(M3, M3_FIELDS) == W3, "M3");
static_assert(packed_end(M4P, M4P_FIELDS) == SUB4, "M4 PDL sub-record");
static_assert(packed_end(M4R, M4R_FIELDS) > 0 && packed_end(M4R, M4R_FIELDS) <= SUB4, "M4 R_dash sub-record");
static_assert(packed_end(M5, M5_FIELDS) == W5, "M5");
static_assert(packed_end(M7, M7_FIELDS) == W6, "M7");

inline int msg_words(int S, int n, int round) {
  switch (round) {
    case 0: return SUB0 * (n + 1);
    case 1: return SUB1 * 2 * (S - 1);
    case 2: return W2;
    case 3: return W3;
    case 4: return SUB4 * S;
    case 5: return W5;
    case 7: return W6;
    default: return 0;
  }
}

struct Bump {
  char* base; size_t off = 0;
  explicit Bump(char* b) : base(b) {}
  void* take(size_t bytes) { const size_t o = off; off = (off + bytes + 255) & ~(size_t)255; return base ? base + o : nullptr; }
  uint32_t* w(size_t words) { return (uint32_t*)take(words * 4); }
  int32_t* i(size_t count) { return (int32_t*)take(count * 4); }
  uint8_t* f(size_t count) { return (uint8_t*)take(count); }
};
struct Counts { size_t nPI, nAP, nVI, nMB, nPP, nPV, SB; };
inline Counts counts_of(int B, int S, int n, int L, int V, int PV) {
  const size_t P1 = S - 1;
  Counts c;
  c.nPI = (size_t)B * L; c.nAP = c.nPI * n; c.nPP = c.nPI * P1; c.nMB = c.nPP * 2; c.nVI = c.nPP * V * n;
  c.nPV = (size_t)B * PV * S * P1; c.SB = (size_t)S * B;
  return c;
}
struct Round0Tmp {
  uint32_t *z, *e, *s, *s1, *s2;
  static Round0Tmp carve(Bump& t, const Counts& c) {
    return {t.w(c.nAP * M0A.z.words), t.w(c.nAP * M0A.e.words), t.w(c.nAP * M0A.s.words), t.w(c.nAP * M0A.s1.words), t.w(c.nAP * M0A.s2.words)};
  }
};
struct Round1Tmp {
  uint32_t *bsel, *btq, *c_b, *Bpk, *BR, *Bz, *BTpk, *BTR, *BTz;
  static Round1Tmp carve(Bump& t, const Counts& c) {
    return {t.w(c.nMB * 8), t.w(c.nMB * 8), t.w(c.nMB * M1.c.words), t.w(c.nMB * M1.b_pk.words), t.w(c.nMB * M1.b_R.words),
            t.w(c.nMB * M1.b_z.words), t.w(c.nMB * M1.bt_pk.words), t.w(c.nMB * M1.bt_R.words), t.w(c.nMB * M1.bt_z.words)};
  }
};
struct Round2Tmp {
  int32_t* sub1_rv;
  uint32_t *alpha_full, *alpha;
  uint8_t* code;
  uint32_t *e, *a1, *a2, *z1, *z2;
  static Round2Tmp carve(Bump& t, const Counts& c) {
    return {t.i(c.nMB), t.w(c.nMB * 64), t.w(c.nMB * 8), t.f(c.nMB),
            t.w(c.nPI * M2.e.words), t.w(c.nPI * M2.a1.words), t.w(c.nPI * M2.a2.words), t.w(c.nPI * M2.z1.words), t.w(c.nPI * M2.z2.words)};
  }
};
struct Round4Tmp {
  uint32_t *z, *u1, *u2, *u3, *s1, *s2, *s3;
  static Round4Tmp carve(Bump& t, const Counts& c) {
    return {t.w(c.nPP * M4P.z.words), t.w(c.nPP * M4P.u1.words), t.w(c.nPP * M4P.u2.words), t.w(c.nPP * M4P.u3.words),
            t.w(c.nPP * M4P.s1.words), t.w(c.nPP * M4P.s2.words), t.w(c.nPP * M4P.s3.words)};
  }
};
struct Round5Tmp {
  uint32_t *S, *T, *A3, *z1, *z2;
  static Round5Tmp carve(Bump& t, const Counts& c) {
    return {t.w(c.nPI * M5.S.words), t.w(c.nPI * M5.T.words), t.w(c.nPI * M5.A3.words), t.w(c.nPI * M5.z1.words), t.w(c.nPI * M5.z2.words)};
  }
};
template <class RoundTmp>
size_t tmp_take(const Counts& c) { Bump t(nullptr); (void)RoundTmp::carve(t, c); return t.off; }
inline size_t tmp_bytes_of(const Counts& c) {
  return std::max({tmp_take<Round0Tmp>(c), tmp_take<Round1Tmp>(c), tmp_take<Round2Tmp>(c), tmp_take<Round4Tmp>(c), tmp_take<Round5Tmp>(c)});
}

}
}
```

multi_party_ecdsa_amd/csrc/mpe_mta.h:

```cpp
#pragma once
#include "mpe_proofs.h"

namespace mpe {

__global__ void mta_idx_kernel(int total, int nst, int nkeys, const int32_t* __restrict__ key_idx, int32_t* __restrict__ b_of,
                               int32_t* __restrict__ st_of, int32_t* __restrict__ key_of_item) {
  const int g = blockIdx.x * blockDim.x + threadIdx.x;
  if (g >= total) return;
  const int b = g / nst;
  b_of[g] = b;
  st_of[g] = g - b * nst;
  key_of_item[g] = key_of(key_idx, nkeys, b);
}
__global__ void mta_all_kernel(int B, int nst, const uint8_t* __restrict__ ok_items, uint8_t* __restrict__ ok) {
  const int b = blockIdx.x * blockDim.x + threadIdx.x;
  if (b >= B) return;
  bool v = true;
  for (int s = 0; s < nst; ++s) v = v && ok_items[(size_t)b * nst + s];
  ok[b] = v ? 1 : 0;
}
__global__ void mta_beta_kernel(int B, const uint32_t* __restrict__ beta_tag, uint32_t* __restrict__ btq, uint32_t* __restrict__ beta) {
  const int i = blockIdx.x * blockDim.x + threadIdx.x;
  if (i >= B) return;
  const ec::U256 t = ec::sc_reduce(beta_tag + (size_t)i * 64, 64);
  ec::u256_store(btq + (size_t)i * 8, t);
  ec::u256_store(beta + (size_t)i * 8, ec::sc_neg(t));
}
__global__ void __launch_bounds__(64) MPE_EC_OCC mta_alpha_kernel(int B, ec::Enc enc, const uint32_t* __restrict__ share, const uint32_t* __restrict__ a,
                                 const uint32_t* __restrict__ pk, const uint32_t* __restrict__ R, const uint32_t* __restrict__ z,
                                 const uint32_t* __restrict__ tpk, const uint32_t* __restrict__ tR, const uint32_t* __restrict__ tz,
                                 uint32_t* __restrict__ alpha, uint8_t* __restrict__ ok) {
  const int i = blockIdx.x * blockDim.x + threadIdx.x;
  if (i >= B) return;
  const ec::U256 al = ec::sc_reduce(share + (size_t)i * 64, 64);
  ec::u256_store(alpha + (size_t)i * 8, al);
  const ec::Aff Bpk = ec::aff_load(pk + (size_t)i * 16), BTpk = ec::aff_load(tpk + (size_t)i * 16);
  const ec::Aff R1 = ec::aff_load(R + (size_t)i * 16), R2 = ec::aff_load(tR + (size_t)i * 16);
  if (!ec::aff_valid(Bpk) || !ec::aff_valid(BTpk) || !ec::aff_valid(R1) || !ec::aff_valid(R2)) { ok[i] = 0; return; }
  ok[i] = sig::mta_alpha_holds(al, ec::sc_reduce(a + (size_t)i * 8, 8), Bpk, R1, ec::sc_reduce(z + (size_t)i * 8, 8), BTpk, R2,
                               ec::sc_reduce(tz + (size_t)i * 8, 8), enc) ? 1 : 0;
}

static int mta_message_b_tail(mpe_ctx* ctx, const mpe_paillier* pk, int batch, const int32_t* d_key_idx, const uint32_t* d_b, const uint32_t* d_ca,
                              const uint32_t* d_r, const uint32_t* d_beta_tag, const uint32_t* d_nonce_b, const uint32_t* d_nonce_bt, uint32_t* btq,
                              uint32_t* d_cb, uint32_t* d_beta, const mpe_dlog_proof* b_proof, const mpe_dlog_proof* beta_tag_proof, hipStream_t st) {
  MPE_TRY(paillier_mul_add_enc(ctx, pk, batch, d_key_idx, rows(d_ca, 128), rows(d_b, 8), 8, d_beta_tag, d_r, d_cb,
                               st));
  MPE_LAUNCH_1D(mta_beta_kernel, batch, st, batch, d_beta_tag, btq, d_beta);
  MPE_LAUNCH_1D(dlog_prove_kernel, batch, st, batch, ctx->enc, d_b, d_nonce_b, b_proof->pk, b_proof->R, b_proof->z);
  MPE_LAUNCH_1D(dlog_prove_kernel, batch, st, batch, ctx->enc, btq, d_nonce_bt, beta_tag_proof->pk, beta_tag_proof->R, beta_tag_proof->z);
  return MPE_OK;
}

}

extern "C" {

int mpe_mta_message_a(mpe_ctx* ctx, const mpe_paillier* pk, const mpe_statements* stm, int batch, const int32_t* d_key_idx,
                      const uint32_t* d_a, const uint32_t* d_r, const mpe_alice_nonces* nonces, uint32_t* d_c,
                      const mpe_alice_proof* proofs, void* stream) {
  if (!ctx || !pk || !stm || !d_a || !d_r || !nonces || !d_c || !proofs || batch < 0) return MPE_E_ARG;
  if (!d_key_idx && pk->nkeys != 1 && pk->nkeys < batch) return MPE_E_ARG;
  if (batch == 0) return MPE_OK;
  hipStream_t st = (hipStream_t)stream;
  const int nst = stm->count, total = batch * nst;
  MPE_TRY(mpe::ws_reserve(ctx, ((size_t)total * 2100 + (size_t)batch * 1000) * 4 + (1u << 20), st));
  char* top = (char*)ctx->ws + ctx->ws_bytes;
  int32_t* b_of = (int32_t*)(top -= ((size_t)total * 4 + 255) & ~(size_t)255);
  int32_t* st_of = (int32_t*)(top -= ((size_t)total * 4 + 255) & ~(size_t)255);
  int32_t* key_it = (int32_t*)(top -= ((size_t)total * 4 + 255) & ~(size_t)255);
  uint32_t* a64 = (uint32_t*)(top -= ((size_t)batch * 64 * 4 + 255) & ~(size_t)255);
  mpe::WsTop hold(ctx, top);
  MPE_LAUNCH_1D(mpe::mta_idx_kernel, total, st, total, nst, pk->nkeys, d_key_idx, b_of, st_of, key_it);
  (void)hipMemsetAsync(a64, 0, (size_t)batch * 64 * 4, st);
  (void)hipMemcpy2DAsync(a64, 64 * 4, d_a, 8 * 4, 8 * 4, batch, hipMemcpyDeviceToDevice, st);
  MPE_TRY(mpe::paillier_encrypt(ctx, pk, batch, d_key_idx, a64, d_r, d_c, true, st));
  return mpe::alice_generate(ctx, pk, stm, total, key_it, st_of, mpe::rows(d_a, 8, b_of), mpe::rows(d_c, 128, b_of),
                             mpe::rows(d_r, 64, b_of), nonces, proofs, st);
}

int mpe_mta_message_b(mpe_ctx* ctx, const mpe_paillier* pk, const mpe_statements* stm, int batch, const int32_t* d_key_idx,
                      const uint32_t* d_b, const uint32_t* d_ca, const mpe_alice_proof* range_proofs, const uint32_t* d_r,
                      const uint32_t* d_beta_tag, const uint32_t* d_nonce_b, const uint32_t* d_nonce_bt, uint32_t* d_cb,
                      uint32_t* d_beta, const mpe_dlog_proof* b_proof, const mpe_dlog_proof* beta_tag_proof, uint8_t* d_ok,
                      void* stream) {
  if (!ctx || !pk || !stm || !d_b || !d_ca || !range_proofs || !d_r || !d_beta_tag || !d_nonce_b || !d_nonce_bt || !d_cb ||
      !d_beta || !b_proof || !beta_tag_proof || !d_ok || batch < 0)
    return MPE_E_ARG;
  if (!d_key_idx && pk->nkeys != 1 && pk->nkeys < batch) return MPE_E_ARG;
  if (batch == 0) return MPE_OK;
  hipStream_t st = (hipStream_t)stream;
  const int nst = stm->count, total = batch * nst;
  MPE_TRY(mpe::ws_reserve(ctx, ((size_t)total * 2400 + (size_t)batch * 700) * 4 + (1u << 20), st));
  char* top = (char*)ctx->ws + ctx->ws_bytes;
  auto take = [&](size_t bytes) { top -= (bytes + 255) & ~(size_t)255; return (void*)top; };
  int32_t* b_of = (int32_t*)take((size_t)total * 4);
  int32_t* st_of = (int32_t*)take((size_t)total * 4);
  int32_t* key_it = (int32_t*)take((size_t)total * 4);
  uint8_t* ok_items = (uint8_t*)take((size_t)total);
  uint32_t* btq = (uint32_t*)take((size_t)batch * 8 * 4);
  mpe::WsTop hold(ctx, top);
  MPE_LAUNCH_1D(mpe::mta_idx_kernel, total, st, total, nst, pk->nkeys, d_key_idx, b_of, st_of, key_it);
  MPE_TRY(mpe::alice_verify(ctx, pk, stm, total, key_it, st_of, mpe::rows(d_ca, 128, b_of), mpe::dense(range_proofs), ok_items, st));
  MPE_LAUNCH_1D(mpe::mta_all_kernel, batch, st, batch, nst, ok_items, d_ok);
  return mpe::mta_message_b_tail(ctx, pk, batch, d_key_idx, d_b, d_ca, d_r, d_beta_tag, d_nonce_b, d_nonce_bt, btq, d_cb, d_beta, b_proof, beta_tag_proof, st);
}

int mpe_mta_verify_get_alpha(mpe_ctx* ctx, const mpe_paillier* sk, int batch, const int32_t* d_key_idx, const uint32_t* d_cb,
                             const mpe_dlog_proof* b_proof, const mpe_dlog_proof* beta_tag_proof, const uint32_t* d_a,
                             uint32_t* d_alpha, uint32_t* d_alice_share, uint8_t* d_ok, void* stream) {
  if (!ctx || !sk || !d_cb || !b_proof || !beta_tag_proof || !d_a || !d_alpha || !d_alice_share || !d_ok || batch < 0) return MPE_E_ARG;
  if (!sk->has_private) { mpe_set_error_msg("mpe_mta_verify_get_alpha: key set has no private part"); return MPE_E_ARG; }
  if (!d_key_idx && sk->nkeys != 1 && sk->nkeys < batch) return MPE_E_ARG;
  if (batch == 0) return MPE_OK;
  hipStream_t st = (hipStream_t)stream;
  MPE_TRY(mpe::paillier_decrypt(ctx, sk, batch, d_key_idx, mpe::rows(d_cb, 128), d_alice_share, st));
  MPE_LAUNCH_1D(mpe::mta_alpha_kernel, batch, st, batch, ctx->enc, d_alice_share, d_a, b_proof->pk, b_proof->R, b_proof->z,
                beta_tag_proof->pk, beta_tag_proof->R, beta_tag_proof->z, d_alpha, d_ok);
  return MPE_OK;
}

}
```

multi_party_ecdsa_amd/csrc/mpe_proofs.h:

```cpp
#pragma once
#include "mpe_sigma_dev.h"
#include "mpe_internal.h"
#include "mpe_modinv.h"
#include "mpe_paillier.h"
#include "mpe_small.h"

struct mpe_statements {
  int count = 0;
  void* blob = nullptr;
  uint32_t* Nt = nullptr;
  uint32_t* h1 = nullptr;
  uint32_t* h2 = nullptr;
  mpe_modset* ms = nullptr;
  int fb_wb = 8;
  uint32_t* fb_tab = nullptr;
};

#include "mpe_fixedbase.h"

extern "C" int mpe_statements_create_wb(mpe_ctx* ctx, int count, const uint32_t* d_Nt, const uint32_t* d_h1, const uint32_t* d_h2,
                                        int wb, mpe_statements** out, void* stream);
static inline size_t mpe_statements_table_bytes(int count, int wb) {
  return (size_t)2 * count * mpe::fb_windows(wb) * ((size_t)1 << wb) * mpe::Cfg2048::K * sizeof(uint32_t);
}

namespace mpe {

static int launch_fb_modexp(mpe_ctx* ctx, const mpe_statements* stm, int B, Rows st_sel, int which, Rows exps, int ew,
                            uint32_t* out, hipStream_t st) {
  if (B == 0) return MPE_OK;
  using C = Cfg2048;
  const int cap = ctx->cus * ctx->modexp_waves_per_cu;
  int split = 1;
  if (ctx->fb_split > 0) { while (split * 2 <= ctx->fb_split && split * 2 <= (int)C::GROUPS) split *= 2; }
  else if (ctx->adaptive_lanes) { while (split * 2 <= (int)C::GROUPS && ((long)B * split * 2 + C::GROUPS - 1) / C::GROUPS <= cap / 2) split *= 2; }
  const int per_wave = C::GROUPS / split;
  const int units = (B + per_wave - 1) / per_wave;
  const int grid = ladder_grid(ctx, units, cap);
  int32_t* sst = (int32_t*)tables_for(ctx, SCHED_WORDS * sizeof(int32_t), st);
  if (!sst) return MPE_E_NOMEM;
  const SchedArgs sched = ladder_sched(ctx, units, cap, sst, st);
  ModsetView v;
  v.n_limbs = stm->ms->n_limbs; v.one_limbs = stm->ms->one_limbs; v.r2_limbs = stm->ms->r2_limbs;
  v.r2h_limbs = stm->ms->r2h_limbs; v.n0inv = stm->ms->n0inv; v.count = stm->ms->count;
  prof_begin(ctx, st, 5, C::BITS, ew, B, stm->fb_wb);
  hipLaunchKernelGGL(fb_modexp_kernel<C>, dim3(grid), dim3(64), 0, st, B, v, st_sel, which, stm->fb_tab, stm->fb_wb, exps, ew, out, sched, split);
  prof_end(ctx, st);
  hipError_t e = hipGetLastError();
  if (e != hipSuccess) { mpe_set_error("fb_modexp_kernel", e); return MPE_E_HIP; }
  return MPE_OK;
}

__global__ void __launch_bounds__(64) MPE_EC_OCC ec_mul_kernel(int B, const uint32_t* __restrict__ k, int kw, const uint32_t* __restrict__ P,
                              uint32_t* __restrict__ out) {
  const int i = blockIdx.x * blockDim.x + threadIdx.x;
  if (i >= B) return;
  const ec::U256 s = ec::sc_reduce(k + (size_t)i * kw, kw);
  const ec::Jac r = P ? ec::jac_mul(s, ec::aff_load(P + (size_t)i * 16)) : ec::jac_mul_gen(s);
  ec::aff_store(out + (size_t)i * 16, ec::jac_to_aff(r));
}
__global__ void __launch_bounds__(64) MPE_EC_OCC ec_add_kernel(int B, const uint32_t* __restrict__ P, const uint32_t* __restrict__ Q,
                              uint32_t* __restrict__ out) {
  const int i = blockIdx.x * blockDim.x + threadIdx.x;
  if (i >= B) return;
  const ec::Jac r = ec::jac_add(ec::jac_from_aff(ec::aff_load(P + (size_t)i * 16)),
                                ec::jac_from_aff(ec::aff_load(Q + (size_t)i * 16)));
  ec::aff_store(out + (size_t)i * 16, ec::jac_to_aff(r));
}

__global__ void __launch_bounds__(64) MPE_EC_OCC dlog_prove_kernel(int B, ec::Enc enc, const uint32_t* __restrict__ sk, const uint32_t* __restrict__ nonce,
                                  uint32_t* __restrict__ pk, uint32_t* __restrict__ R, uint32_t* __restrict__ z) {
  const int i = blockIdx.x * blockDim.x + threadIdx.x;
  if (i >= B) return;
  ec::Aff P, Rp;
  ec::U256 zz;
  sig::dlog_prove_body(ec::sc_reduce(sk + (size_t)i * 8, 8), ec::sc_reduce(nonce + (size_t)i * 8, 8), enc, P, Rp, zz);
  ec::aff_store(pk + (size_t)i * 16, P);
  ec::aff_store(R + (size_t)i * 16, Rp);
  ec::u256_store(z + (size_t)i * 8, zz);
}
__global__ void __launch_bounds__(64) MPE_EC_OCC dlog_verify_kernel(int B, ec::Enc enc, const uint32_t* __restrict__ pk, const uint32_t* __restrict__ R,
                                   const uint32_t* __restrict__ z, uint8_t* __restrict__ ok) {
  const int i = blockIdx.x * blockDim.x + threadIdx.x;
  if (i >= B) return;
  const ec::Aff P = ec::aff_load(pk + (size_t)i * 16), Rp = ec::aff_load(R + (size_t)i * 16);
  if (!ec::aff_valid(P) || !ec::aff_valid(Rp)) { ok[i] = 0; return; }
  ok[i] = sig::dlog_verify_body(P, Rp, ec::sc_reduce(z + (size_t)i * 8, 8), enc) ? 1 : 0;
}

__global__ void muladd_kernel(int B, Rows a, int na, Rows b, int nb, Rows c, int nc, uint32_t* __restrict__ r, int nr) {
  MPE_FOREGROUND();
  const int i = blockIdx.x * blockDim.x + threadIdx.x;
  if (i >= B) return;
  uint32_t x[90], y[90], t[180];
  sm::copy(x, row_of(a, i), na);
  sm::copy(y, row_of(b, i), nb);
  sm::mul(t, x, na, y, nb);
  for (int j = na + nb; j < nr; ++j) t[j] = 0;
  const uint32_t one[1] = {1};
  const uint32_t* cp = c.p ? row_of(c, i) : one;
  sm::add(t, nr, t, nr, cp, c.p ? nc : 1);
  uint32_t* o = r + (size_t)i * nr;
  for (int j = 0; j < nr; ++j) o[j] = t[j];
}

enum { HF_BIGINT = 0, HF_BIGINT_PLUS1 = 1, HF_POINT_COMPRESSED = 2 };
struct HashField { Rows r; int words; int kind; };
struct HashDesc { HashField f[14]; int n; };
__global__ void __launch_bounds__(64) MPE_EC_OCC hash_kernel(int B, ec::Enc enc, HashDesc d, uint32_t* __restrict__ out) {
  MPE_FOREGROUND();
  const int i = blockIdx.x * blockDim.x + threadIdx.x;
  if (i >= B) return;
  ec::Sha256 s;
  ec::sha_init(s);
  for (int k = 0; k < d.n; ++k) {
    const uint32_t* p = row_of(d.f[k].r, i);
    if (d.f[k].kind == HF_POINT_COMPRESSED) {
      ec::sha_point_compressed(s, ec::aff_load(p));
    } else if (d.f[k].kind == HF_BIGINT_PLUS1) {
      uint32_t t[130];
      const uint32_t one[1] = {1};
      t[d.f[k].words] = sm::add(t, d.f[k].words, p, d.f[k].words, one, 1);
      ec::sha_bigint(s, t, d.f[k].words + 1, enc);
    } else {
      ec::sha_bigint(s, p, d.f[k].words, enc);
    }
  }
  ec::u256_store(out + (size_t)i * 8, ec::sha_final(s));
}
static HashField hf(Rows r, int words, int kind = HF_BIGINT) { return HashField{r, words, kind}; }

__global__ void s1_range_kernel(int B, Rows s1, int words, uint8_t* __restrict__ ok) {
  const int i = blockIdx.x * blockDim.x + threadIdx.x;
  if (i >= B) return;
  uint32_t q[8], q2[16], q3[24];
  for (int j = 0; j < 8; ++j) q[j] = ec::FQ[j];
  sm::mul(q2, q, 8, q, 8);
  sm::mul(q3, q2, 16, q, 8);
  ok[i] = sm::cmp(row_of(s1, i), words, q3, 24) <= 0 ? 1 : 0;
}
__global__ void and_flags_kernel(int B, uint8_t* __restrict__ ok, const uint8_t* __restrict__ a, const uint8_t* __restrict__ b,
                                 const uint32_t* __restrict__ x, Rows y, int words) {
  const int i = blockIdx.x * blockDim.x + threadIdx.x;
  if (i >= B) return;
  bool v = ok[i] != 0;
  if (a) v = v && a[i];
  if (b) v = v && b[i];
  if (x) v = v && sm::cmp(x + (size_t)i * words, words, row_of(y, i), words) == 0;
  ok[i] = v ? 1 : 0;
}
__global__ void fill_u8_kernel(int B, uint8_t* p, uint8_t v) {
  const int i = blockIdx.x * blockDim.x + threadIdx.x;
  if (i < B) p[i] = v;
}
__global__ void __launch_bounds__(64) MPE_EC_OCC pdl_u1_check_kernel(int B, Rows s1, const uint32_t* __restrict__ e, Rows G, Rows Q, Rows u1,
                                    uint8_t* __restrict__ ok) {
  const int i = blockIdx.x * blockDim.x + threadIdx.x;
  if (i >= B) return;
  const ec::U256 a = ec::sc_reduce(row_of(s1, i), 25);
  const ec::U256 ne = ec::sc_neg(ec::sc_reduce(e + (size_t)i * 8, 8));
  const ec::Aff Gp = ec::aff_load(row_of(G, i)), Qp = ec::aff_load(row_of(Q, i)), U1 = ec::aff_load(row_of(u1, i));
  if (!ec::aff_valid(Gp) || !ec::aff_valid(Qp) || !ec::aff_valid(U1)) { ok[i] = 0; return; }
  const ec::Jac l = ec::jac_add(ec::jac_mul(a, Gp), ec::jac_mul(ne, Qp));
  if (!ec::jac_eq_aff(l, U1)) ok[i] = 0;
}
__global__ void __launch_bounds__(64) MPE_EC_OCC ec_mul_rows_kernel(int B, Rows k, int kw, Rows P, uint32_t* __restrict__ out) {
  MPE_FOREGROUND();
  const int i = blockIdx.x * blockDim.x + threadIdx.x;
  if (i >= B) return;
  const ec::U256 s = ec::sc_reduce(row_of(k, i), kw);
  const ec::Jac r = P.p ? ec::jac_mul(s, ec::aff_load(row_of(P, i))) : ec::jac_mul_gen(s);
  ec::aff_store(out + (size_t)i * 16, ec::jac_to_aff(r));
}

struct Seq {
  mpe_ctx* ctx;
  hipStream_t st;
  int B;
  int rc = MPE_OK;
  uint32_t* words(size_t per_item) {
    uint32_t* p = ws_array<uint32_t>(ctx, (size_t)B * per_item);
    if (!p && rc == MPE_OK) { rc = MPE_E_NOMEM; mpe_set_error_msg("workspace under-reserved"); }
    return p;
  }
  uint8_t* flags() {
    uint8_t* p = ws_array<uint8_t>(ctx, (size_t)B);
    if (!p && rc == MPE_OK) { rc = MPE_E_NOMEM; mpe_set_error_msg("workspace under-reserved"); }
    return p;
  }
  uint32_t* fb_modexp(const mpe_statements* stm, Rows sel, int which, Rows base, Rows exps, int ew) {
    if (!stm->fb_tab || !ctx->use_fixed_base) return modexp(stm->ms, sel, base, exps, ew);
    uint32_t* o = words(64);
    if (rc == MPE_OK) rc = launch_fb_modexp(ctx, stm, B, sel, which, exps, ew, o, st);
    return o;
  }
  uint32_t* modexp(const mpe_modset* ms, Rows sel, Rows base, Rows exps, int ew) {
    uint32_t* o = words(ms->bits / 32);
    if (rc == MPE_OK) rc = launch_modexp(ctx, ms, B, sel, base, no_rows(), exps, ew, o, st);
    return o;
  }
  uint32_t* modexp_nn(const mpe_paillier* pk, Rows sel, Rows base, Rows exps, int ew, bool holder, bool pow_n = false) {
    uint32_t* o = words(128);
    if (rc == MPE_OK) rc = mpe::modexp_nn(ctx, pk, B, sel, base, exps, ew, holder, o, st, pow_n);
    return o;
  }
  uint32_t* modexp_nn2(const mpe_paillier* pk, Rows sel, Rows base, Rows exps, int ew, Rows base2, Rows exps2, int ew2) {
    uint32_t* o = words(128);
    if (rc == MPE_OK) rc = mpe::modexp_nn2(ctx, pk, B, sel, base, exps, ew, base2, exps2, ew2, o, st);
    return o;
  }
  uint32_t* modexp_n(const mpe_paillier* pk, const int32_t* key_idx, Rows sel, Rows base, Rows exps, int ew) {
    if (!(pk->has_private && ctx->use_crt && ctx->use_pair && ctx->use_crt_n)) return modexp(pk->ms_n, sel, base, exps, ew);
    uint32_t* o = words(64);
    if (rc == MPE_OK) rc = mpe::modexp_n_holder(ctx, pk, B, key_idx, base, exps, ew, o, st);
    return o;
  }
  uint32_t* modmul(const mpe_modset* ms, Rows sel, Rows a, Rows b) {
    uint32_t* o = words(ms->bits / 32);
    if (rc == MPE_OK) rc = launch_modmul(ctx, ms, B, sel, a, b, o, st);
    return o;
  }
  void modmul_to(const mpe_modset* ms, Rows sel, Rows a, Rows b, uint32_t* o) {
    if (rc == MPE_OK) rc = launch_modmul(ctx, ms, B, sel, a, b, o, st);
  }
  uint32_t* modinv(const mpe_modset* ms, Rows sel, Rows a, uint8_t* ok) {
    uint32_t* o = words(ms->bits / 32);
    if (rc == MPE_OK) rc = launch_modinv(ctx, ms, B, sel, a, o, ok, st);
    return o;
  }
  void muladd(Rows a, int na, Rows b, int nb, Rows c, int nc, uint32_t* r, int nr) {
    if (rc != MPE_OK) return;
    hipLaunchKernelGGL(muladd_kernel, dim3(blocks_for(B, 64)), dim3(64), 0, st, B, a, na, b, nb, c, nc, r, nr);
  }
  void hash(const HashDesc& d, uint32_t* out) {
    if (rc != MPE_OK) return;
    hipLaunchKernelGGL(hash_kernel, dim3(blocks_for(B, 64)), dim3(64), 0, st, B, ctx->enc, d, out);
  }
  int finish(const char* what) {
    if (rc != MPE_OK) return rc;
    hipError_t e = hipGetLastError();
    if (e != hipSuccess) { mpe_set_error(what, e); return MPE_E_HIP; }
    return MPE_OK;
  }
};

static Rows sel_of(const int32_t* idx, int count) { return Rows{nullptr, idx, (idx == nullptr && count != 1) ? 1 : 0, 0}; }
static Rows tab_rows(const uint32_t* table, int stride, const int32_t* idx, int count, int words = 0) {
  if (idx) return Rows{table, idx, stride, words};
  return Rows{table, nullptr, count == 1 ? 0 : stride, words};
}

struct AliceProofRows { Rows z, e, s, s1, s2; };
struct PdlProofRows { Rows z, u1, u2, u3, s1, s2, s3; };
static AliceProofRows dense(const mpe_alice_proof* p) {
  return AliceProofRows{rows(p->z, 64), rows(p->e, 8), rows(p->s, 64), rows(p->s1, 25), rows(p->s2, 89)};
}
static PdlProofRows dense(const mpe_pdl_proof* p) {
  return PdlProofRows{rows(p->z, 64), rows(p->u1, 16), rows(p->u2, 128), rows(p->u3, 64), rows(p->s1, 25), rows(p->s2, 64),
                      rows(p->s3, 89)};
}
static Rows with_words(Rows r, int words) { r.words = words; return r; }
struct Handed {
  const uint32_t* p = nullptr; hipEvent_t ready = nullptr; explicit operator bool() const { return p != nullptr; }
  void wait(hipStream_t st) const { if (p && ready) (void)hipStreamWaitEvent(st, ready, 0); }
};

static inline size_t ws_need_alice_generate(int B) { return (size_t)B * (1400 + CRT_WS_WORDS + MODEXP_N_HOLDER_WS_WORDS) * 4 + 65536; }
static inline size_t ws_need_alice_verify(int B) { return (size_t)B * 2200 * 4 + 65536; }
static int merge_rc(const Seq& a, const Seq& b, const Seq& c) { return a.rc != MPE_OK ? a.rc : (b.rc != MPE_OK ? b.rc : c.rc); }

static int alice_generate(mpe_ctx* ctx, const mpe_paillier* pk, const mpe_statements* stm, int B, const int32_t* key_idx,
                          const int32_t* st_idx, Rows a, Rows cipher, Rows r,
                          const mpe_alice_nonces* nn, const mpe_alice_proof* out, hipStream_t st, Fork* outer = nullptr,
                          Handed bn_pre = {}, hipEvent_t cipher_ready = nullptr) {
  MPE_TRY(ws_reserve(ctx, ws_need_alice_generate(B), st));
  Fork f(ctx, st, 3, B <= ctx->par_items);
  Seq q{ctx, f.s(0), B}, q1{ctx, f.s(1), B}, q2{ctx, f.s(2), B};
  const Rows ksel = sel_of(key_idx, pk->nkeys), ssel = sel_of(st_idx, stm->count);
  const Rows h1 = tab_rows(stm->h1, 64, st_idx, stm->count), h2 = tab_rows(stm->h2, 64, st_idx, stm->count);
  const Rows Nrow = tab_rows(pk->N, 64, key_idx, pk->nkeys);
  uint32_t* z1 = q1.fb_modexp(stm, ssel, 0, h1,a, 8);
  uint32_t* z2 = q1.fb_modexp(stm, ssel, 1, h2,rows(nn->rho, 72), 72);
  q1.modmul_to(stm->ms, ssel, rows(z1, 64), rows(z2, 64), out->z);
  uint32_t* gu = q.words(128);
  q.muladd(rows(nn->alpha, 24), 24, Nrow, 64, no_rows(), 0, gu, 128);
  bn_pre.wait(f.s(0));
  const uint32_t* bn = bn_pre ? bn_pre.p : q.modexp_nn(pk, ksel, rows(nn->beta, 64, nullptr, 64), Nrow, 64, true, true);
  uint32_t* u = q.modmul(pk->ms_nn, ksel, rows(gu, 128), rows(bn, 128));
  uint32_t* w1 = q2.fb_modexp(stm, ssel, 0, h1,rows(nn->alpha, 24), 24);
  uint32_t* w2 = q2.fb_modexp(stm, ssel, 1, h2,rows(nn->gamma, 88), 88);
  uint32_t* w = q2.modmul(stm->ms, ssel, rows(w1, 64), rows(w2, 64));
  f.join();
  if (cipher_ready) (void)hipStreamWaitEvent(st, cipher_ready, 0);
  else if (outer) outer->join();
  q.rc = merge_rc(q, q1, q2);
  HashDesc d;
  d.n = 6;
  d.f[0] = hf(Nrow, 64); d.f[1] = hf(Nrow, 64, HF_BIGINT_PLUS1); d.f[2] = hf(cipher, 128);
  d.f[3] = hf(rows(out->z, 64), 64); d.f[4] = hf(rows(u, 128), 128); d.f[5] = hf(rows(w, 64), 64);
  q.hash(d, out->e);
  uint32_t* re = q.modexp_n(pk, key_idx, ksel, r, rows(out->e, 8), 8);
  q.modmul_to(pk->ms_n, ksel, rows(re, 64), rows(nn->beta, 64), out->s);
  q.muladd(rows(out->e, 8), 8, a, 8, rows(nn->alpha, 24), 24, out->s1, 25);
  q.muladd(rows(out->e, 8), 8, rows(nn->rho, 72), 72, rows(nn->gamma, 88), 88, out->s2, 89);
  return q.finish("alice_generate");
}

static int alice_verify(mpe_ctx* ctx, const mpe_paillier* pk, const mpe_statements* stm, int B, const int32_t* key_idx,
                        const int32_t* st_idx, Rows cipher, const AliceProofRows& pr, uint8_t* ok, hipStream_t st,
                        Handed m_pre = {}, const uint8_t* inv_ok_pre = nullptr) {
  MPE_TRY(ws_reserve(ctx, ws_need_alice_verify(B), st));
  Fork f(ctx, st, 3, B <= ctx->par_items);
  Seq q{ctx, f.s(0), B}, q1{ctx, f.s(1), B}, q2{ctx, f.s(2), B};
  const Rows ksel = sel_of(key_idx, pk->nkeys), ssel = sel_of(st_idx, stm->count);
  const Rows h1 = tab_rows(stm->h1, 64, st_idx, stm->count), h2 = tab_rows(stm->h2, 64, st_idx, stm->count);
  const Rows Nrow = tab_rows(pk->N, 64, key_idx, pk->nkeys);
  MPE_LAUNCH_1D(s1_range_kernel, B, st, B, pr.s1, 25, ok);
  uint8_t *inv_ok1 = q.flags(), *inv_ok2 = q.flags();
  uint32_t* ze = q1.modexp(stm->ms, ssel, pr.z, pr.e, 8);
  uint32_t* zei = q1.modinv(stm->ms, ssel, rows(ze, 64), inv_ok1);
  uint32_t* a1 = q2.fb_modexp(stm, ssel, 0, h1,pr.s1, 25);
  uint32_t* a2 = q2.fb_modexp(stm, ssel, 1, h2,pr.s2, 89);
  uint32_t* a12 = q2.modmul(stm->ms, ssel, rows(a1, 64), rows(a2, 64));
  uint32_t* gs1 = q.words(128);
  q.muladd(pr.s1, 25, Nrow, 64, no_rows(), 0, gs1, 128);
  uint32_t *u = nullptr, *b12 = nullptr, *cie = nullptr;
  if (m_pre) {
    inv_ok2 = const_cast<uint8_t*>(inv_ok_pre);
    m_pre.wait(f.s(0));
    u = q.modmul(pk->ms_nn, ksel, rows(gs1, 128), rows(m_pre.p, 128));
  } else if (f.on) {
    uint32_t* sn = q.modexp_nn(pk, ksel, with_words(pr.s, 64), Nrow, 64, false);
    b12 = q.modmul(pk->ms_nn, ksel, rows(gs1, 128), rows(sn, 128));
    uint32_t* cred = q2.modmul(pk->ms_nn, ksel, cipher, rows(pk->ms_nn->one_words, 0, nullptr, 1));
    uint32_t* cinv = q2.modinv(pk->ms_nn, ksel, rows(cred, 128), inv_ok2);
    cie = q2.modexp_nn(pk, ksel, rows(cinv, 128), pr.e, 8, false);
  } else if (ctx->use_multiexp) {
    uint32_t* cred = q.modmul(pk->ms_nn, ksel, cipher, rows(pk->ms_nn->one_words, 0, nullptr, 1));
    uint32_t* cinv = q.modinv(pk->ms_nn, ksel, rows(cred, 128), inv_ok2);
    uint32_t* m = q.modexp_nn2(pk, ksel, with_words(pr.s, 64), Nrow, 64, rows(cinv, 128), pr.e, 8);
    u = q.modmul(pk->ms_nn, ksel, rows(gs1, 128), rows(m, 128));
  } else {
    uint32_t* ce = q.modexp_nn(pk, ksel, cipher, pr.e, 8, false);
    uint32_t* cei = q.modinv(pk->ms_nn, ksel, rows(ce, 128), inv_ok2);
    uint32_t* sn = q.modexp_nn(pk, ksel, with_words(pr.s, 64), Nrow, 64, false);
    uint32_t* b12n = q.modmul(pk->ms_nn, ksel, rows(gs1, 128), rows(sn, 128));
    u = q.modmul(pk->ms_nn, ksel, rows(b12n, 128), rows(cei, 128));
  }
  f.join();
  q.rc = merge_rc(q, q1, q2);
  if (f.on && !m_pre) u = q.modmul(pk->ms_nn, ksel, rows(b12, 128), rows(cie, 128));
  uint32_t* w = q.modmul(stm->ms, ssel, rows(a12, 64), rows(zei, 64));
  uint32_t* e2 = q.words(8);
  HashDesc d;
  d.n = 6;
  d.f[0] = hf(Nrow, 64); d.f[1] = hf(Nrow, 64, HF_BIGINT_PLUS1); d.f[2] = hf(cipher, 128);
  d.f[3] = hf(pr.z, 64); d.f[4] = hf(rows(u, 128), 128); d.f[5] = hf(rows(w, 64), 64);
  q.hash(d, e2);
  if (q.rc == MPE_OK)
    hipLaunchKernelGGL(and_flags_kernel, dim3(blocks_for(B, 64)), dim3(64), 0, st, B, ok, inv_ok1, inv_ok2, e2, pr.e, 8);
  return q.finish("alice_verify");
}

static int pdl_prove(mpe_ctx* ctx, const mpe_paillier* pk, const mpe_statements* stm, int B, const int32_t* key_idx,
                     const int32_t* st_idx, Rows cipher, Rows Qp, Rows Gp, Rows x, Rows r, const mpe_pdl_nonces* nn,
                     const mpe_pdl_proof* out, hipStream_t st, Fork* outer = nullptr, Handed bn_pre = {},
                     hipEvent_t G_ready = nullptr) {
  MPE_TRY(ws_reserve(ctx, (size_t)B * (1400 + CRT_WS_WORDS + MODEXP_N_HOLDER_WS_WORDS) * 4 + 65536, st));
  Fork f(ctx, st, 3, B <= ctx->par_items);
  Seq q{ctx, f.s(0), B}, q1{ctx, f.s(1), B}, q2{ctx, f.s(2), B};
  const Rows ksel = sel_of(key_idx, pk->nkeys), ssel = sel_of(st_idx, stm->count);
  const Rows h1 = tab_rows(stm->h1, 64, st_idx, stm->count), h2 = tab_rows(stm->h2, 64, st_idx, stm->count);
  const Rows Nrow = tab_rows(pk->N, 64, key_idx, pk->nkeys);
  uint32_t* z1 = q1.fb_modexp(stm, ssel, 0, h1,x, 8);
  uint32_t* z2 = q1.fb_modexp(stm, ssel, 1, h2,rows(nn->rho, 72), 72);
  q1.modmul_to(stm->ms, ssel, rows(z1, 64), rows(z2, 64), out->z);
  if (G_ready) (void)hipStreamWaitEvent(f.s(1), G_ready, 0);
  else if (outer) outer->branch_done_wait(1, f.s(1));
  if (B > 0) hipLaunchKernelGGL(ec_mul_rows_kernel, dim3(blocks_for(B, 64)), dim3(64), 0, f.s(1), B, rows(nn->alpha, 24), 24, Gp, out->u1);
  uint32_t* ga = q.words(128);
  q.muladd(rows(nn->alpha, 24), 24, Nrow, 64, no_rows(), 0, ga, 128);
  bn_pre.wait(f.s(0));
  const uint32_t* bn = bn_pre ? bn_pre.p : q.modexp_nn(pk, ksel, rows(nn->beta, 64, nullptr, 64), Nrow, 64, true, true);
  q.modmul_to(pk->ms_nn, ksel, rows(ga, 128), rows(bn, 128), out->u2);
  uint32_t* w1 = q2.fb_modexp(stm, ssel, 0, h1,rows(nn->alpha, 24), 24);
  uint32_t* w2 = q2.fb_modexp(stm, ssel, 1, h2,rows(nn->gamma, 88), 88);
  q2.modmul_to(stm->ms, ssel, rows(w1, 64), rows(w2, 64), out->u3);
  f.join();
  if (outer) outer->join();
  q.rc = merge_rc(q, q1, q2);
  uint32_t* e = q.words(8);
  HashDesc d;
  d.n = 7;
  d.f[0] = hf(Gp, 16, HF_POINT_COMPRESSED); d.f[1] = hf(Qp, 16, HF_POINT_COMPRESSED);
  d.f[2] = hf(cipher, 128); d.f[3] = hf(rows(out->z, 64), 64);
  d.f[4] = hf(rows(out->u1, 16), 16, HF_POINT_COMPRESSED); d.f[5] = hf(rows(out->u2, 128), 128);
  d.f[6] = hf(rows(out->u3, 64), 64);
  q.hash(d, e);
  q.muladd(rows(e, 8), 8, x, 8, rows(nn->alpha, 24), 24, out->s1, 25);
  uint32_t* re = q.modexp_n(pk, key_idx, ksel, r, rows(e, 8), 8);
  q.modmul_to(pk->ms_n, ksel, rows(re, 64), rows(nn->beta, 64), out->s2);
  q.muladd(rows(e, 8), 8, rows(nn->rho, 72), 72, rows(nn->gamma, 88), 88, out->s3, 89);
  return q.finish("pdl_prove");
}

static int pdl_verify(mpe_ctx* ctx, const mpe_paillier* pk, const mpe_statements* stm, int B, const int32_t* key_idx,
                      const int32_t* st_idx, Rows cipher, Rows Qp, Rows Gp, const PdlProofRows& pr, uint8_t* ok,
                      hipStream_t st) {
  MPE_TRY(ws_reserve(ctx, (size_t)B * 2600 * 4 + 65536, st));
  const Rows ksel = sel_of(key_idx, pk->nkeys), ssel = sel_of(st_idx, stm->count);
  const Rows h1 = tab_rows(stm->h1, 64, st_idx, stm->count), h2 = tab_rows(stm->h2, 64, st_idx, stm->count);
  const Rows Nrow = tab_rows(pk->N, 64, key_idx, pk->nkeys);
  Seq q0{ctx, st, B};
  uint32_t* e = q0.words(8);
  HashDesc d;
  d.n = 7;
  d.f[0] = hf(Gp, 16, HF_POINT_COMPRESSED); d.f[1] = hf(Qp, 16, HF_POINT_COMPRESSED);
  d.f[2] = hf(cipher, 128); d.f[3] = hf(pr.z, 64);
  d.f[4] = hf(pr.u1, 16, HF_POINT_COMPRESSED); d.f[5] = hf(pr.u2, 128);
  d.f[6] = hf(pr.u3, 64);
  q0.hash(d, e);
  Fork f(ctx, st, 3, B <= ctx->par_items);
  Seq q{ctx, f.s(0), B}, q1{ctx, f.s(1), B}, q2{ctx, f.s(2), B};
  q.rc = q0.rc;
  if (B > 0) {
    hipLaunchKernelGGL(fill_u8_kernel, dim3(blocks_for(B, 64)), dim3(64), 0, f.s(1), B, ok, (uint8_t)1);
    hipLaunchKernelGGL(pdl_u1_check_kernel, dim3(blocks_for(B, 64)), dim3(64), 0, f.s(1), B, pr.s1, e, Gp, Qp, pr.u1, ok);
  }
  uint8_t *inv_ok1 = q.flags(), *inv_ok2 = q.flags();
  uint32_t* g1 = q.words(128);
  q.muladd(pr.s1, 25, Nrow, 64, no_rows(), 0, g1, 128);
  uint32_t *u2 = nullptr, *t2s = nullptr, *cies = nullptr;
  if (f.on) {
    uint32_t* s2n = q.modexp_nn(pk, ksel, with_words(pr.s2, 64), Nrow, 64, false);
    t2s = q.modmul(pk->ms_nn, ksel, rows(g1, 128), rows(s2n, 128));
    uint32_t* cred = q1.modmul(pk->ms_nn, ksel, cipher, rows(pk->ms_nn->one_words, 0, nullptr, 1));
    uint32_t* cinv = q1.modinv(pk->ms_nn, ksel, rows(cred, 128), inv_ok1);
    cies = q1.modexp_nn(pk, ksel, rows(cinv, 128), rows(e, 8), 8, false);
  } else {
    uint32_t* cred = q.modmul(pk->ms_nn, ksel, cipher, rows(pk->ms_nn->one_words, 0, nullptr, 1));
    uint32_t* cinv = q.modinv(pk->ms_nn, ksel, rows(cred, 128), inv_ok1);
    if (ctx->use_multiexp) {
      uint32_t* m = q.modexp_nn2(pk, ksel, with_words(pr.s2, 64), Nrow, 64, rows(cinv, 128), rows(e, 8), 8);
      u2 = q.modmul(pk->ms_nn, ksel, rows(g1, 128), rows(m, 128));
    } else {
      uint32_t* s2n = q.modexp_nn(pk, ksel, with_words(pr.s2, 64), Nrow, 64, false);
      uint32_t* t2 = q.modmul(pk->ms_nn, ksel, rows(g1, 128), rows(s2n, 128));
      uint32_t* cie = q.modexp_nn(pk, ksel, rows(cinv, 128), rows(e, 8), 8, false);
      u2 = q.modmul(pk->ms_nn, ksel, rows(t2, 128), rows(cie, 128));
    }
  }
  uint32_t* a1 = q2.fb_modexp(stm, ssel, 0, h1,pr.s1, 25);
  uint32_t* a2 = q2.fb_modexp(stm, ssel, 1, h2,pr.s3, 89);
  uint32_t* a12 = q2.modmul(stm->ms, ssel, rows(a1, 64), rows(a2, 64));
  uint32_t* zred = q2.modmul(stm->ms, ssel, pr.z, rows(stm->ms->one_words, 0, nullptr, 1));
  uint32_t* zinv = q2.modinv(stm->ms, ssel, rows(zred, 64), inv_ok2);
  uint32_t* zie = q2.modexp(stm->ms, ssel, rows(zinv, 64), rows(e, 8), 8);
  uint32_t* u3 = q2.modmul(stm->ms, ssel, rows(a12, 64), rows(zie, 64));
  f.join();
  q.rc = merge_rc(q, q1, q2);
  if (f.on) u2 = q.modmul(pk->ms_nn, ksel, rows(t2s, 128), rows(cies, 128));
  if (q.rc == MPE_OK) {
    hipLaunchKernelGGL(and_flags_kernel, dim3(blocks_for(B, 64)), dim3(64), 0, st, B, ok, inv_ok1, inv_ok2, u2, pr.u2, 128);
    hipLaunchKernelGGL(and_flags_kernel, dim3(blocks_for(B, 64)), dim3(64), 0, st, B, ok, (const uint8_t*)nullptr,
                       (const uint8_t*)nullptr, u3, pr.u3, 64);
  }
  return q.finish("pdl_verify");
}

}

extern "C" {

int mpe_statements_create(mpe_ctx* ctx, int count, const uint32_t* d_Nt, const uint32_t* d_h1, const uint32_t* d_h2,
                          mpe_statements** out, void* stream) {
  if (!ctx) return MPE_E_ARG;
  return mpe_statements_create_wb(ctx, count, d_Nt, d_h1, d_h2, ctx->fb_window_bits, out, stream);
}
int mpe_statements_create_wb(mpe_ctx* ctx, int count, const uint32_t* d_Nt, const uint32_t* d_h1, const uint32_t* d_h2, int wb,
                             mpe_statements** out, void* stream) {
  if (!ctx || !d_Nt || !d_h1 || !d_h2 || !out || count <= 0 || (wb != 0 && wb < 2) || wb > 16) return MPE_E_ARG;
  hipStream_t st = (hipStream_t)stream;
  mpe_statements* s = new (std::nothrow) mpe_statements();
  if (!s) return MPE_E_NOMEM;
  s->count = count;
  const size_t w = (size_t)count * 64;
  hipError_t e = hipMalloc(&s->blob, 3 * w * 4);
  if (e != hipSuccess) { delete s; mpe_set_error("hipMalloc(statements)", e); return MPE_E_NOMEM; }
  s->Nt = (uint32_t*)s->blob; s->h1 = s->Nt + w; s->h2 = s->h1 + w;
  (void)hipMemcpyAsync(s->Nt, d_Nt, w * 4, hipMemcpyDeviceToDevice, st);
  (void)hipMemcpyAsync(s->h1, d_h1, w * 4, hipMemcpyDeviceToDevice, st);
  (void)hipMemcpyAsync(s->h2, d_h2, w * 4, hipMemcpyDeviceToDevice, st);
  int rc = mpe::modset_create_dev(ctx, 2048, count, s->Nt, &s->ms, st);
  if (rc != MPE_OK) { (void)hipFree(s->blob); delete s; return rc; }
  s->fb_wb = 0;
  if (ctx->use_fixed_base && wb != 0) {
    using C = mpe::Cfg2048;
    s->fb_wb = wb;
    const int nwindows = mpe::fb_windows(s->fb_wb);
    const size_t bytes = (size_t)2 * count * nwindows * ((size_t)1 << s->fb_wb) * C::K * sizeof(uint32_t);
    e = hipMalloc((void**)&s->fb_tab, bytes);
    if (e != hipSuccess) { mpe_set_error("hipMalloc(fixed-base tables)", e); mpe_statements_destroy(s); return MPE_E_NOMEM; }
    mpe::ModsetView v;
    v.n_limbs = s->ms->n_limbs; v.one_limbs = s->ms->one_limbs; v.r2_limbs = s->ms->r2_limbs; v.r2h_limbs = s->ms->r2h_limbs;
    v.n0inv = s->ms->n0inv; v.count = s->ms->count;
    const int npairs = 2 * count, nrows = npairs * nwindows;
    hipLaunchKernelGGL(mpe::fb_bases_kernel<C>, dim3((npairs + C::GROUPS - 1) / C::GROUPS), dim3(64), 0, st, npairs, v, s->h1,
                       s->h2, s->fb_wb, s->fb_tab);
    hipLaunchKernelGGL(mpe::fb_fill_kernel<C>, dim3((nrows + C::GROUPS - 1) / C::GROUPS), dim3(64), 0, st, nrows, v, s->fb_wb,
                       s->fb_tab);
    e = hipGetLastError();
    if (e != hipSuccess) { mpe_set_error("fixed-base table build", e); mpe_statements_destroy(s); return MPE_E_HIP; }
  }
  *out = s;
  return MPE_OK;
}
int mpe_statements_destroy(mpe_statements* s) {
  if (!s) return MPE_E_ARG;
  if (s->ms) mpe_modset_destroy(s->ms);
  if (s->fb_tab) (void)hipFree(s->fb_tab);
  if (s->blob) (void)hipFree(s->blob);
  delete s;
  return MPE_OK;
}

int mpe_ec_mul_base(mpe_ctx* ctx, int batch, const uint32_t* d_k, int k_words, uint32_t* d_out, void* stream) {
  if (!ctx || !d_k || !d_out || batch < 0 || k_words <= 0 || k_words > 89) return MPE_E_ARG;
  hipStream_t st = (hipStream_t)stream;
  MPE_LAUNCH_1D(mpe::ec_mul_kernel, batch, st, batch, d_k, k_words, (const uint32_t*)nullptr, d_out);
  return MPE_OK;
}
int mpe_ec_mul(mpe_ctx* ctx, int batch, const uint32_t* d_k, int k_words, const uint32_t* d_P, uint32_t* d_out,
               void* stream) {
  if (!ctx || !d_k || !d_P || !d_out || batch < 0 || k_words <= 0 || k_words > 89) return MPE_E_ARG;
  hipStream_t st = (hipStream_t)stream;
  MPE_LAUNCH_1D(mpe::ec_mul_kernel, batch, st, batch, d_k, k_words, d_P, d_out);
  return MPE_OK;
}
int mpe_ec_add(mpe_ctx* ctx, int batch, const uint32_t* d_P, const uint32_t* d_Q, uint32_t* d_out, void* stream) {
  if (!ctx || !d_P || !d_Q || !d_out || batch < 0) return MPE_E_ARG;
  hipStream_t st = (hipStream_t)stream;
  MPE_LAUNCH_1D(mpe::ec_add_kernel, batch, st, batch, d_P, d_Q, d_out);
  return MPE_OK;
}
int mpe_dlog_prove(mpe_ctx* ctx, int batch, const uint32_t* d_sk, const uint32_t* d_nonce, uint32_t* d_pk,
                   uint32_t* d_R, uint32_t* d_z, void* stream) {
  if (!ctx || !d_sk || !d_nonce || !d_pk || !d_R || !d_z || batch < 0) return MPE_E_ARG;
  hipStream_t st = (hipStream_t)stream;
  MPE_LAUNCH_1D(mpe::dlog_prove_kernel, batch, st, batch, ctx->enc, d_sk, d_nonce, d_pk, d_R, d_z);
  return MPE_OK;
}
int mpe_dlog_verify(mpe_ctx* ctx, int batch, const uint32_t* d_pk, const uint32_t* d_R, const uint32_t* d_z,
                    uint8_t* d_ok, void* stream) {
  if (!ctx || !d_pk || !d_R || !d_z || !d_ok || batch < 0) return MPE_E_ARG;
  hipStream_t st = (hipStream_t)stream;
  MPE_LAUNCH_1D(mpe::dlog_verify_kernel, batch, st, batch, ctx->enc, d_pk, d_R, d_z, d_ok);
  return MPE_OK;
}
int mpe_modinv(mpe_ctx* ctx, const mpe_modset* ms, int batch, const int32_t* d_mod_idx, const uint32_t* d_a,
               uint32_t* d_out, uint8_t* d_ok, void* stream) {
  if (!ctx || !ms || !d_a || !d_out || !d_ok || batch < 0) return MPE_E_ARG;
  if (!d_mod_idx && ms->count != 1 && ms->count < batch) return MPE_E_ARG;
  MPE_TRY(mpe::ws_reserve(ctx, mpe::modinv_ws_words(ms, batch) * 4, (hipStream_t)stream));
  return mpe::launch_modinv(ctx, ms, batch, mpe::sel_of(d_mod_idx, ms->count), mpe::rows(d_a, ms->bits / 32), d_out, d_ok,
                            (hipStream_t)stream);
}

static bool proof_args_ok(const mpe_ctx* ctx, const mpe_paillier* pk, const mpe_statements* stm, int batch,
                          const int32_t* key_idx, const int32_t* st_idx) {
  if (!ctx || !pk || !stm || batch < 0) return false;
  if (!key_idx && pk->nkeys != 1 && pk->nkeys < batch) return false;
  if (!st_idx && stm->count != 1 && stm->count < batch) return false;
  return true;
}
int mpe_alice_generate(mpe_ctx* ctx, const mpe_paillier* pk, const mpe_statements* stm, int batch,
                       const int32_t* d_key_idx, const int32_t* d_st_idx, const uint32_t* d_a, const uint32_t* d_cipher,
                       const uint32_t* d_r, const mpe_alice_nonces* nonces, const mpe_alice_proof* out, void* stream) {
  if (!proof_args_ok(ctx, pk, stm, batch, d_key_idx, d_st_idx) || !d_a || !d_cipher || !d_r || !nonces || !out) return MPE_E_ARG;
  if (batch == 0) return MPE_OK;
  return mpe::alice_generate(ctx, pk, stm, batch, d_key_idx, d_st_idx, mpe::rows(d_a, 8), mpe::rows(d_cipher, 128),
                             mpe::rows(d_r, 64), nonces, out, (hipStream_t)stream);
}
int mpe_alice_verify(mpe_ctx* ctx, const mpe_paillier* pk, const mpe_statements* stm, int batch, const int32_t* d_key_idx,
                     const int32_t* d_st_idx, const uint32_t* d_cipher, const mpe_alice_proof* proof, uint8_t* d_ok,
                     void* stream) {
  if (!proof_args_ok(ctx, pk, stm, batch, d_key_idx, d_st_idx) || !d_cipher || !proof || !d_ok) return MPE_E_ARG;
  if (batch == 0) return MPE_OK;
  return mpe::alice_verify(ctx, pk, stm, batch, d_key_idx, d_st_idx, mpe::rows(d_cipher, 128), mpe::dense(proof), d_ok,
                           (hipStream_t)stream);
}
int mpe_pdl_prove(mpe_ctx* ctx, const mpe_paillier* pk, const mpe_statements* stm, int batch, const int32_t* d_key_idx,
                  const int32_t* d_st_idx, const uint32_t* d_cipher, const uint32_t* d_Q, const uint32_t* d_G,
                  const uint32_t* d_x, const uint32_t* d_r, const mpe_pdl_nonces* nonces, const mpe_pdl_proof* out,
                  void* stream) {
  if (!proof_args_ok(ctx, pk, stm, batch, d_key_idx, d_st_idx) || !d_cipher || !d_Q || !d_G || !d_x || !d_r || !nonces || !out)
    return MPE_E_ARG;
  if (batch == 0) return MPE_OK;
  return mpe::pdl_prove(ctx, pk, stm, batch, d_key_idx, d_st_idx, mpe::rows(d_cipher, 128), mpe::rows(d_Q, 16), mpe::rows(d_G, 16),
                        mpe::rows(d_x, 8), mpe::rows(d_r, 64), nonces, out, (hipStream_t)stream);
}
int mpe_pdl_verify(mpe_ctx* ctx, const mpe_paillier* pk, const mpe_statements* stm, int batch, const int32_t* d_key_idx,
                   const int32_t* d_st_idx, const uint32_t* d_cipher, const uint32_t* d_Q, const uint32_t* d_G,
                   const mpe_pdl_proof* proof, uint8_t* d_ok, void* stream) {
  if (!proof_args_ok(ctx, pk, stm, batch, d_key_idx, d_st_idx) || !d_cipher || !d_Q || !d_G || !proof || !d_ok) return MPE_E_ARG;
  if (batch == 0) return MPE_OK;
  return mpe::pdl_verify(ctx, pk, stm, batch, d_key_idx, d_st_idx, mpe::rows(d_cipher, 128), mpe::rows(d_Q, 16), mpe::rows(d_G, 16),
                         mpe::dense(proof), d_ok, (hipStream_t)stream);
}

}
```

Baseline: 18950.

## Share Paillier ciphertext inversions across verification items with the same ciphertext

Many range-proof and PDL verification items reference the same Paillier ciphertext under the same key. The modular inversion of that ciphertext mod N^2 was previously computed once per item. New index tables map each verify item to a unique ciphertext slot, so inversion runs once per distinct ciphertext and results and flags are gathered back per item. This adds index arrays and an expand-flags kernel, and changes the workspace sizing formulas.

```diff
diff --git a/multi_party_ecdsa_amd/csrc/mpe_gg20.h b/multi_party_ecdsa_amd/csrc/mpe_gg20.h
--- a/multi_party_ecdsa_amd/csrc/mpe_gg20.h
+++ b/multi_party_ecdsa_amd/csrc/mpe_gg20.h
@@ -99,6 +99,10 @@
   int32_t *ca_mb, *kpub_mb, *kown_mb;
   int32_t *pi_pp, *kown_pp, *st_pp;
   int32_t *ca_pv, *pi_pv, *kpub_pv, *st_pv;
+  int32_t *ci_of_vi;
+  int32_t *vi_of_ci, *ca_ci, *kpub_ci;
+  int32_t *cj_of_pv;
+  int32_t *pv_of_cj, *ca_cj, *kpub_cj;
 };
 __global__ void idx_kernel(Dim d, Idx x, int total) {
   const int g = blockIdx.x * blockDim.x + threadIdx.x;
@@ -113,6 +117,8 @@
     const int st = g % n, r1 = g / n, r2 = r1 / d.V, jj = r2 % P1, pi = r2 / P1, b = pi / L, i = loc_of(d, b, pi % L);
     const int ind = ind_of(i, jj);
     x.ca_vi[g] = ind * d.B + b; x.kpub_vi[g] = kpub(d, b, ind); x.st_vi[g] = ks_of(d, b) * n + st;
+    x.ci_of_vi[g] = r2;
+    if (g % (d.V * n) == 0) { x.vi_of_ci[r2] = g; x.ca_ci[r2] = ind * d.B + b; x.kpub_ci[r2] = kpub(d, b, ind); }
   }
   if (g < d.B * L * P1 * 2) {
     const int pp = g >> 1, jj = pp % P1, pi = pp / P1, b = pi / L, i = loc_of(d, b, pi % L), ind = ind_of(i, jj);
@@ -126,6 +132,8 @@
     const int jj = g % P1, r1 = g / P1, i = r1 % S, r2 = r1 / S, vl = r2 % d.PV, b = r2 / d.PV;
     x.ca_pv[g] = i * d.B + b; x.pi_pv[g] = b * L + vl; x.kpub_pv[g] = kpub(d, b, i);
     x.st_pv[g] = ks_of(d, b) * n + sg_of(d, b, ind_of(i, jj));
+    x.cj_of_pv[g] = r1;
+    if (jj == 0) { x.pv_of_cj[r1] = g; x.ca_cj[r1] = i * d.B + b; x.kpub_cj[r1] = kpub(d, b, i); }
   }
 }
 
@@ -760,6 +768,8 @@
   x.ca_mb = m.i(c.nMB); x.kpub_mb = m.i(c.nMB); x.kown_mb = m.i(c.nMB);
   x.pi_pp = m.i(c.nPP); x.kown_pp = m.i(c.nPP); x.st_pp = m.i(c.nPP);
   x.ca_pv = m.i(c.nPV); x.pi_pv = m.i(c.nPV); x.kpub_pv = m.i(c.nPV); x.st_pv = m.i(c.nPV);
+  x.ci_of_vi = m.i(c.nVI); x.vi_of_ci = m.i(c.nCI); x.ca_ci = m.i(c.nCI); x.kpub_ci = m.i(c.nCI);
+  x.cj_of_pv = m.i(c.nPV); x.pv_of_cj = m.i(c.nCJ); x.ca_cj = m.i(c.nCJ); x.kpub_cj = m.i(c.nCJ);
   s->kq = m.w(c.nPI * 8); s->gq = m.w(c.nPI * 8); s->w = m.w(c.nPI * 8); s->k64 = m.w(c.nPI * 64);
   s->g_gamma = m.w(c.nPI * 16); s->com = m.w(c.nPI * 8); s->c_a = m.w(c.nPI * 128); s->beta = m.w(c.nMB * 8);
   s->ca_all = m.w(c.SB * 128); s->com_all = m.w(c.SB * 8); s->bpk_in = m.w(c.nPP * 16);
@@ -770,7 +780,7 @@
   s->status = m.i(c.nPI * NR); s->sig_recid = m.i(c.nPI);
   s->sub0_vi = m.i(c.nVI); s->ok_vi = m.f(c.nVI); s->sub4_pv = m.i(c.nPV); s->rdash_pv = m.i(c.nPV); s->ok_pv = m.f(c.nPV);
   Ahead& a = s->ahead; const bool small = small_batch(s->ctx, c.nVI);
-  a.cinv = small ? m.w(c.nVI * 128) : nullptr; a.cinv_ok = small ? m.f(c.nVI) : nullptr;
+  a.cinv = small ? m.w(c.nCI * 128) : nullptr; a.cinv_ok = small ? m.f(c.nCI) : nullptr;
   a.ped = m.w(c.nPI * 48);
   a.pdl_bn = small ? m.w(c.nPP * 128) : nullptr; a.pdl_scratch = small ? m.w(modexp_nn_scratch_words(c.nPP)) : nullptr;
   s->tmp_bytes = tmp_bytes_of(c);
@@ -817,7 +827,10 @@
   const int ind = (int)(jb / B), b = (int)(jb % B);
   ca_all[g] = c_a[((size_t)b * S + ind) * 128 + w];
 }
-static size_t ws_need_inversion_ahead(const mpe_paillier* pk, size_t nVI) { return nVI * (128 + 128 + 1) * 4 + modinv_ws_words(pk->ms_nn, (int)nVI) * 4 + 16384; }
+static InvShare share_r1(const mpe_gg20_session* s, const Counts& c) { return InvShare{(int)c.nCI, s->ix.ci_of_vi, s->ix.kpub_ci, rows(s->ca_all, 128, s->ix.ca_ci)}; }
+static InvShare share_r5(const mpe_gg20_session* s, const Counts& c) {
+  return c.nCJ == c.nPV ? InvShare{} : InvShare{(int)c.nCJ, s->ix.cj_of_pv, s->ix.kpub_cj, rows(s->ca_all, 128, s->ix.ca_cj)};
+}
 
 static bool pdl_ahead_eligible(const mpe_gg20_session* s, const Counts& c) {
   const mpe_ctx* ctx = s->ctx; const Ahead& a = s->ahead;
@@ -860,7 +873,7 @@
   a.cinv_done = false;
   if (par && rc == MPE_OK) {
     rc = ws_reserve(ctx, ws_need_encrypt((int)c.nPI) + ws_need_alice_generate((int)c.nAP) + nXN * (64 + 128 + 1 + CRT_WS_WORDS) * 4 + 65536 +
-                         (ahead ? ws_need_inversion_ahead(K->pub, c.nVI) : 0), st);
+                         (ahead ? ws_need_invert_shared(K->pub, c.nCI) : 0), st);
     if (rc == MPE_OK) ctx->ws_hold++;
   }
   const bool held = par && rc == MPE_OK;
@@ -894,15 +907,11 @@
     hipStream_t sx = g.s(1);
     (void)hipEventRecord(ctx->ev_mid, sx); c_ready = ctx->ev_mid;
     hipLaunchKernelGGL(ca_all_from_local_kernel, dim3((unsigned)((c.SB * 128 + 255) / 256)), dim3(256), 0, sx, d.S, d.B, s->c_a, s->ca_all);
-    Seq q{ctx, sx, (int)c.nVI};
-    const Rows ksel = sel_of(s->ix.kpub_vi, K->pub->nkeys);
-    uint8_t* ok = q.flags();
-    uint32_t* cred = q.modmul(K->pub->ms_nn, ksel, rows(s->ca_all, 128, s->ix.ca_vi), rows(K->pub->ms_nn->one_words, 0, nullptr, 1));
-    uint32_t* cinv = q.modinv(K->pub->ms_nn, ksel, rows(cred, 128), ok);
-    rc = q.rc;
+    const uint32_t* cinv = nullptr; const uint8_t* ok = nullptr;
+    rc = invert_shared(ctx, K->pub, share_r1(s, c), sx, &cinv, &ok);
     if (rc == MPE_OK) {
-      (void)hipMemcpyAsync(a.cinv, cinv, c.nVI * 128 * 4, hipMemcpyDeviceToDevice, sx);
-      (void)hipMemcpyAsync(a.cinv_ok, ok, c.nVI, hipMemcpyDeviceToDevice, sx);
+      (void)hipMemcpyAsync(a.cinv, cinv, c.nCI * 128 * 4, hipMemcpyDeviceToDevice, sx);
+      (void)hipMemcpyAsync(a.cinv_ok, ok, c.nCI, hipMemcpyDeviceToDevice, sx);
       a.cinv_done = true;
     }
     gg_trace(s->ctx, sx, "round 1's inversion, ahead", rc);
@@ -930,42 +939,36 @@
   const int w = (int)(g % words), i = (int)(g / words);
   dst[g] = w < src_words ? row_of(src, i)[w] : 0u;
 }
-static size_t ws_need_round1_merged(const mpe_paillier* pk, size_t nVI, size_t nMB) {
-  return (nVI + nMB) * (size_t)(64 + 128 + 8 + 1 + 128) * 4 + nVI * (128 + 128 + 1) * 4 + modinv_ws_words(pk->ms_nn, (int)nVI) * 4 + 65536;
-}
-static int round1_merged_ladders(mpe_ctx* ctx, const mpe_paillier* pk, size_t nVI, const int32_t* kpub_vi, Rows cipher_vi, Rows s_vi, Rows e_vi,
+static size_t ws_need_round1_merged(const mpe_paillier* pk, size_t nVI, size_t nMB, size_t nCI) {
+  return (nVI + nMB) * (size_t)(64 + 128 + 8 + 1 + 128) * 4 + nVI + ws_need_invert_shared(pk, nCI) + 65536;
+}
+static int round1_merged_ladders(mpe_ctx* ctx, const mpe_paillier* pk, size_t nVI, const int32_t* kpub_vi, const InvShare& sh, Rows s_vi, Rows e_vi,
                                  size_t nMB, const int32_t* kpub_mb, Rows ca_mb, const uint32_t* bsel, const uint32_t* mb_r,
                                  const uint32_t** m_vi, const uint8_t** inv_ok_vi, const uint32_t** x_mb, hipStream_t st,
                                  Handed cinv_pre = {}, const uint8_t* cinv_ok_pre = nullptr) {
   const size_t n = nVI + nMB;
-  Seq q{ctx, st, (int)nVI};
-  const Rows ksel = sel_of(kpub_vi, pk->nkeys);
   const uint8_t* inv_ok = cinv_ok_pre;
   const uint32_t* cinv = cinv_pre.p;
   cinv_pre.wait(st);
-  if (!cinv_pre) {
-    uint8_t* ok = q.flags();
-    uint32_t* cred = q.modmul(pk->ms_nn, ksel, cipher_vi, rows(pk->ms_nn->one_words, 0, nullptr, 1));
-    cinv = q.modinv(pk->ms_nn, ksel, rows(cred, 128), ok);
-    inv_ok = ok;
-  }
-  if (q.rc != MPE_OK) return q.rc;
+  if (!cinv_pre) MPE_TRY(invert_shared(ctx, pk, sh, st, &cinv, &inv_ok));
+  uint8_t* ok_vi = ws_array<uint8_t>(ctx, nVI);
   uint32_t* b1 = ws_array<uint32_t>(ctx, n * 64);
   uint32_t* b2 = ws_array<uint32_t>(ctx, n * 128);
   uint32_t* e2 = ws_array<uint32_t>(ctx, n * 8);
   int32_t* key = ws_array<int32_t>(ctx, n);
   uint32_t* out = ws_array<uint32_t>(ctx, n * 128);
-  if (!b1 || !b2 || !e2 || !key || !out) { mpe_set_error_msg("round1: workspace under-reserved"); return MPE_E_NOMEM; }
+  if (!ok_vi || !b1 || !b2 || !e2 || !key || !out) { mpe_set_error_msg("round1: workspace under-reserved"); return MPE_E_NOMEM; }
+  if (nVI) hipLaunchKernelGGL(expand_flags_kernel, dim3(blocks_for((int)nVI, 64)), dim3(64), 0, st, (int)nVI, inv_ok, sh.of_item, ok_vi);
   auto gather = [&](size_t cnt, Rows src, int sw, int words, uint32_t* dst) {
     if (cnt) hipLaunchKernelGGL(gather_rows_kernel, dim3((unsigned)((cnt * words + 255) / 256)), dim3(256), 0, st, (int)cnt, src, sw, words, dst);
   };
   gather(nVI, s_vi, 64, 64, b1);              gather(nMB, rows(mb_r, 64), 64, 64, b1 + nVI * 64);
-  gather(nVI, rows(cinv, 128), 128, 128, b2); gather(nMB, ca_mb, 128, 128, b2 + nVI * 128);
+  gather(nVI, rows(cinv, 128, sh.of_item), 128, 128, b2); gather(nMB, ca_mb, 128, 128, b2 + nVI * 128);
   gather(nVI, e_vi, 8, 8, e2);                gather(nMB, rows(bsel, 8), 8, 8, e2 + nVI * 8);
   (void)hipMemcpyAsync(key, kpub_vi, nVI * 4, hipMemcpyDeviceToDevice, st);
   (void)hipMemcpyAsync(key + nVI, kpub_mb, nMB * 4, hipMemcpyDeviceToDevice, st);
   MPE_TRY(modexp_nn2(ctx, pk, (int)n, key_selector(pk, key), rows(b1, 64, nullptr, 64), key_rows(pk, pk->N, 64, key), 64, rows(b2, 128), rows(e2, 8), 8, out, st));
-  *m_vi = out; *inv_ok_vi = inv_ok; *x_mb = out + nVI * 128;
+  *m_vi = out; *inv_ok_vi = ok_vi; *x_mb = out + nVI * 128;
   return MPE_OK;
 }
 
@@ -989,14 +992,15 @@
   const bool merged = round1_merges(ctx, c);
   const bool ahead = merged && s->ahead.cinv_done;
   s->ahead.cinv_done = false;
-  if (par && !merged && rc == MPE_OK) { rc = ws_reserve(ctx, ws_need_alice_verify((int)c.nVI) + ws_need_mul_add_enc((int)c.nMB), st); if (rc == MPE_OK) ctx->ws_hold++; }
+  const InvShare sh = share_r1(s, c);
+  if (par && !merged && rc == MPE_OK) { rc = ws_reserve(ctx, ws_need_alice_verify(K->pub, c.nVI, c.nCI) + ws_need_mul_add_enc((int)c.nMB), st); if (rc == MPE_OK) ctx->ws_hold++; }
   bool held = par && !merged && rc == MPE_OK;
   const uint32_t *m_vi = nullptr, *x_mb = nullptr;
   const uint8_t* inv_ok_vi = nullptr;
   AliceProofRows pr{rows(d_in + M0A.z.off, SUB0, sub0_vi), rows(d_in + M0A.e.off, SUB0, sub0_vi), rows(d_in + M0A.s.off, SUB0, sub0_vi),
                     rows(d_in + M0A.s1.off, SUB0, sub0_vi), rows(d_in + M0A.s2.off, SUB0, sub0_vi)};
   if (merged && rc == MPE_OK) {
-    rc = ws_reserve(ctx, ws_need_alice_verify((int)c.nVI) + ws_need_mul_add_enc((int)c.nMB) + ws_need_round1_merged(K->pub, c.nVI, c.nMB), st);
+    rc = ws_reserve(ctx, ws_need_alice_verify(K->pub, c.nVI, c.nCI) + ws_need_mul_add_enc((int)c.nMB) + ws_need_round1_merged(K->pub, c.nVI, c.nMB, c.nCI), st);
     if (rc == MPE_OK) { ctx->ws_hold++; held = true; }
   }
   if (rc == MPE_OK && c.nMB > 0)
@@ -1013,7 +1017,7 @@
   {
     hipStream_t st2 = g.s(1);
     if (merged && rc == MPE_OK) {
-      rc = round1_merged_ladders(ctx, K->pub, c.nVI, s->ix.kpub_vi, rows(s->ca_all, 128, s->ix.ca_vi), with_words(pr.s, 64), pr.e, c.nMB, s->ix.kpub_mb,
+      rc = round1_merged_ladders(ctx, K->pub, c.nVI, s->ix.kpub_vi, sh, with_words(pr.s, 64), pr.e, c.nMB, s->ix.kpub_mb,
                                  rows(s->ca_all, 128, s->ix.ca_mb), bsel, Z.mb_r, &m_vi, &inv_ok_vi, &x_mb, st2,
                                  ahead ? Handed{s->ahead.cinv} : Handed{}, ahead ? s->ahead.cinv_ok : nullptr);
       if (rc == MPE_OK && g.on) { (void)hipEventRecord(ctx->ev_mid, st2); m_ready = ctx->ev_mid; }
@@ -1026,7 +1030,7 @@
     if (!dlog_first) dlog_proofs(st2);
   }
   if (rc == MPE_OK)
-    rc = alice_verify(ctx, K->pub, K->stm, (int)c.nVI, s->ix.kpub_vi, s->ix.st_vi, rows(s->ca_all, 128, s->ix.ca_vi), pr, ok_vi, st, Handed{m_vi, m_ready}, inv_ok_vi);
+    rc = alice_verify(ctx, K->pub, K->stm, (int)c.nVI, s->ix.kpub_vi, s->ix.st_vi, rows(s->ca_all, 128, s->ix.ca_vi), pr, ok_vi, st, Handed{m_vi, m_ready}, inv_ok_vi, sh);
   gg_trace(s->ctx, st, "alice_verify", rc);
   g.join();
   if (held) ctx->ws_hold--;
@@ -1141,7 +1145,7 @@
     hipLaunchKernelGGL(r5_prove_kernel, dim3(blocks_for((int)c.nPI, 64)), dim3(64), 0, g.s(1), d, s->R, s->sigma_i, s->lq, s->pedT, Z.heg_s1, Z.heg_s2, heg);
   if (rc == MPE_OK)
     rc = pdl_verify(ctx, K->pub, K->stm, (int)c.nPV, s->ix.kpub_pv, s->ix.st_pv, rows(s->ca_all, 128, s->ix.ca_pv), rows(d_in + M4R.R_dash.off, SUB4, rdash_pv),
-                    rows(s->R, 16, s->ix.pi_pv), pr, ok_pv, st);
+                    rows(s->R, 16, s->ix.pi_pv), pr, ok_pv, st, share_r5(s, c));
   gg_trace(s->ctx, st, "pdl_verify", rc);
   g.join();
   GG_LAUNCH(r5_status_kernel, c.nPI, d, in4, ok_pv, STAT(5), BADR(5));
diff --git a/multi_party_ecdsa_amd/csrc/mpe_gg20_msg.h b/multi_party_ecdsa_amd/csrc/mpe_gg20_msg.h
--- a/multi_party_ecdsa_amd/csrc/mpe_gg20_msg.h
+++ b/multi_party_ecdsa_amd/csrc/mpe_gg20_msg.h
@@ -75,12 +75,13 @@
   int32_t* i(size_t count) { return (int32_t*)take(count * 4); }
   uint8_t* f(size_t count) { return (uint8_t*)take(count); }
 };
-struct Counts { size_t nPI, nAP, nVI, nMB, nPP, nPV, SB; };
+struct Counts { size_t nPI, nAP, nVI, nMB, nPP, nPV, SB, nCI, nCJ; };
 inline Counts counts_of(int B, int S, int n, int L, int V, int PV) {
   const size_t P1 = S - 1;
   Counts c;
   c.nPI = (size_t)B * L; c.nAP = c.nPI * n; c.nPP = c.nPI * P1; c.nMB = c.nPP * 2; c.nVI = c.nPP * V * n;
   c.nPV = (size_t)B * PV * S * P1; c.SB = (size_t)S * B;
+  c.nCI = c.nPI * P1; c.nCJ = (size_t)B * PV * S;
   return c;
 }
 struct Round0Tmp {
diff --git a/multi_party_ecdsa_amd/csrc/mpe_mta.h b/multi_party_ecdsa_amd/csrc/mpe_mta.h
--- a/multi_party_ecdsa_amd/csrc/mpe_mta.h
+++ b/multi_party_ecdsa_amd/csrc/mpe_mta.h
@@ -101,7 +101,8 @@
   uint32_t* btq = (uint32_t*)take((size_t)batch * 8 * 4);
   mpe::WsTop hold(ctx, top);
   MPE_LAUNCH_1D(mpe::mta_idx_kernel, total, st, total, nst, pk->nkeys, d_key_idx, b_of, st_of, key_it);
-  MPE_TRY(mpe::alice_verify(ctx, pk, stm, total, key_it, st_of, mpe::rows(d_ca, 128, b_of), mpe::dense(range_proofs), ok_items, st));
+  MPE_TRY(mpe::alice_verify(ctx, pk, stm, total, key_it, st_of, mpe::rows(d_ca, 128, b_of), mpe::dense(range_proofs), ok_items, st, {}, nullptr,
+                            mpe::InvShare{batch, b_of, d_key_idx, mpe::rows(d_ca, 128)}));
   MPE_LAUNCH_1D(mpe::mta_all_kernel, batch, st, batch, nst, ok_items, d_ok);
   return mpe::mta_message_b_tail(ctx, pk, batch, d_key_idx, d_b, d_ca, d_r, d_beta_tag, d_nonce_b, d_nonce_bt, btq, d_cb, d_beta, b_proof, beta_tag_proof, st);
 }
diff --git a/multi_party_ecdsa_amd/csrc/mpe_proofs.h b/multi_party_ecdsa_amd/csrc/mpe_proofs.h
--- a/multi_party_ecdsa_amd/csrc/mpe_proofs.h
+++ b/multi_party_ecdsa_amd/csrc/mpe_proofs.h
@@ -265,8 +265,35 @@
   void wait(hipStream_t st) const { if (p && ready) (void)hipStreamWaitEvent(st, ready, 0); }
 };
 
+struct InvShare {
+  int n = 0; const int32_t* of_item = nullptr; const int32_t* key_idx = nullptr; Rows cipher{};
+  explicit operator bool() const { return of_item != nullptr; }
+};
+static inline size_t ws_need_invert_shared(const mpe_paillier* pk, size_t n) { return n * (128 + 128 + 1) * 4 + modinv_ws_words(pk->ms_nn, (int)n) * 4 + 16384; }
+__global__ void expand_flags_kernel(int B, const uint8_t* __restrict__ slot_ok, const int32_t* __restrict__ of_item, uint8_t* __restrict__ ok) {
+  const int i = blockIdx.x * blockDim.x + threadIdx.x;
+  if (i < B) ok[i] = slot_ok[of_item[i]];
+}
+static int invert_shared(mpe_ctx* ctx, const mpe_paillier* pk, const InvShare& sh, hipStream_t st, const uint32_t** cinv, const uint8_t** ok) {
+  Seq q{ctx, st, sh.n};
+  const Rows ksel = sel_of(sh.key_idx, pk->nkeys);
+  uint8_t* f = q.flags();
+  uint32_t* cred = q.modmul(pk->ms_nn, ksel, sh.cipher, rows(pk->ms_nn->one_words, 0, nullptr, 1));
+  *cinv = q.modinv(pk->ms_nn, ksel, rows(cred, 128), f);
+  *ok = f;
+  return q.rc;
+}
+static int invert_for_items(mpe_ctx* ctx, const mpe_paillier* pk, const InvShare& sh, int B, hipStream_t st, Rows* cinv_item, uint8_t* ok_item) {
+  const uint32_t* cinv = nullptr; const uint8_t* ok = nullptr;
+  MPE_TRY(invert_shared(ctx, pk, sh, st, &cinv, &ok));
+  *cinv_item = rows(cinv, 128, sh.of_item);
+  if (B > 0) hipLaunchKernelGGL(expand_flags_kernel, dim3(blocks_for(B, 64)), dim3(64), 0, st, B, ok, sh.of_item, ok_item);
+  return MPE_OK;
+}
+
 static inline size_t ws_need_alice_generate(int B) { return (size_t)B * (1400 + CRT_WS_WORDS + MODEXP_N_HOLDER_WS_WORDS) * 4 + 65536; }
-static inline size_t ws_need_alice_verify(int B) { return (size_t)B * 2200 * 4 + 65536; }
+static inline size_t ws_need_alice_verify(const mpe_paillier* pk, size_t B, size_t n_inv) { return B * (2200 - 256) * 4 + 65536 + ws_need_invert_shared(pk, n_inv); }
+static inline size_t ws_need_pdl_verify(const mpe_paillier* pk, size_t B, size_t n_inv) { return B * (2600 - 256) * 4 + 65536 + ws_need_invert_shared(pk, n_inv); }
 static int merge_rc(const Seq& a, const Seq& b, const Seq& c) { return a.rc != MPE_OK ? a.rc : (b.rc != MPE_OK ? b.rc : c.rc); }
 
 static int alice_generate(mpe_ctx* ctx, const mpe_paillier* pk, const mpe_statements* stm, int B, const int32_t* key_idx,
@@ -308,8 +335,8 @@
 
 static int alice_verify(mpe_ctx* ctx, const mpe_paillier* pk, const mpe_statements* stm, int B, const int32_t* key_idx,
                         const int32_t* st_idx, Rows cipher, const AliceProofRows& pr, uint8_t* ok, hipStream_t st,
-                        Handed m_pre = {}, const uint8_t* inv_ok_pre = nullptr) {
-  MPE_TRY(ws_reserve(ctx, ws_need_alice_verify(B), st));
+                        Handed m_pre = {}, const uint8_t* inv_ok_pre = nullptr, InvShare sh = {}) {
+  MPE_TRY(ws_reserve(ctx, ws_need_alice_verify(pk, B, sh ? sh.n : B), st));
   Fork f(ctx, st, 3, B <= ctx->par_items);
   Seq q{ctx, f.s(0), B}, q1{ctx, f.s(1), B}, q2{ctx, f.s(2), B};
   const Rows ksel = sel_of(key_idx, pk->nkeys), ssel = sel_of(st_idx, stm->count);
@@ -325,6 +352,15 @@
   uint32_t* gs1 = q.words(128);
   q.muladd(pr.s1, 25, Nrow, 64, no_rows(), 0, gs1, 128);
   uint32_t *u = nullptr, *b12 = nullptr, *cie = nullptr;
+  auto c_inverse = [&](Seq& qq) -> Rows {
+    if (sh) {
+      Rows r = no_rows();
+      if (qq.rc == MPE_OK) qq.rc = invert_for_items(ctx, pk, sh, B, qq.st, &r, inv_ok2);
+      return r;
+    }
+    uint32_t* cred = qq.modmul(pk->ms_nn, ksel, cipher, rows(pk->ms_nn->one_words, 0, nullptr, 1));
+    return rows(qq.modinv(pk->ms_nn, ksel, rows(cred, 128), inv_ok2), 128);
+  };
   if (m_pre) {
     inv_ok2 = const_cast<uint8_t*>(inv_ok_pre);
     m_pre.wait(f.s(0));
@@ -332,13 +368,9 @@
   } else if (f.on) {
     uint32_t* sn = q.modexp_nn(pk, ksel, with_words(pr.s, 64), Nrow, 64, false);
     b12 = q.modmul(pk->ms_nn, ksel, rows(gs1, 128), rows(sn, 128));
-    uint32_t* cred = q2.modmul(pk->ms_nn, ksel, cipher, rows(pk->ms_nn->one_words, 0, nullptr, 1));
-    uint32_t* cinv = q2.modinv(pk->ms_nn, ksel, rows(cred, 128), inv_ok2);
-    cie = q2.modexp_nn(pk, ksel, rows(cinv, 128), pr.e, 8, false);
+    cie = q2.modexp_nn(pk, ksel, c_inverse(q2), pr.e, 8, false);
   } else if (ctx->use_multiexp) {
-    uint32_t* cred = q.modmul(pk->ms_nn, ksel, cipher, rows(pk->ms_nn->one_words, 0, nullptr, 1));
-    uint32_t* cinv = q.modinv(pk->ms_nn, ksel, rows(cred, 128), inv_ok2);
-    uint32_t* m = q.modexp_nn2(pk, ksel, with_words(pr.s, 64), Nrow, 64, rows(cinv, 128), pr.e, 8);
+    uint32_t* m = q.modexp_nn2(pk, ksel, with_words(pr.s, 64), Nrow, 64, c_inverse(q), pr.e, 8);
     u = q.modmul(pk->ms_nn, ksel, rows(gs1, 128), rows(m, 128));
   } else {
     uint32_t* ce = q.modexp_nn(pk, ksel, cipher, pr.e, 8, false);
@@ -406,8 +438,8 @@
 
 static int pdl_verify(mpe_ctx* ctx, const mpe_paillier* pk, const mpe_statements* stm, int B, const int32_t* key_idx,
                       const int32_t* st_idx, Rows cipher, Rows Qp, Rows Gp, const PdlProofRows& pr, uint8_t* ok,
-                      hipStream_t st) {
-  MPE_TRY(ws_reserve(ctx, (size_t)B * 2600 * 4 + 65536, st));
+                      hipStream_t st, InvShare sh = {}) {
+  MPE_TRY(ws_reserve(ctx, ws_need_pdl_verify(pk, B, sh ? sh.n : B), st));
   const Rows ksel = sel_of(key_idx, pk->nkeys), ssel = sel_of(st_idx, stm->count);
   const Rows h1 = tab_rows(stm->h1, 64, st_idx, stm->count), h2 = tab_rows(stm->h2, 64, st_idx, stm->count);
   const Rows Nrow = tab_rows(pk->N, 64, key_idx, pk->nkeys);
@@ -431,22 +463,28 @@
   uint32_t* g1 = q.words(128);
   q.muladd(pr.s1, 25, Nrow, 64, no_rows(), 0, g1, 128);
   uint32_t *u2 = nullptr, *t2s = nullptr, *cies = nullptr;
+  auto c_inverse = [&](Seq& qq) -> Rows {
+    if (sh) {
+      Rows r = no_rows();
+      if (qq.rc == MPE_OK) qq.rc = invert_for_items(ctx, pk, sh, B, qq.st, &r, inv_ok1);
+      return r;
+    }
+    uint32_t* cred = qq.modmul(pk->ms_nn, ksel, cipher, rows(pk->ms_nn->one_words, 0, nullptr, 1));
+    return rows(qq.modinv(pk->ms_nn, ksel, rows(cred, 128), inv_ok1), 128);
+  };
   if (f.on) {
     uint32_t* s2n = q.modexp_nn(pk, ksel, with_words(pr.s2, 64), Nrow, 64, false);
     t2s = q.modmul(pk->ms_nn, ksel, rows(g1, 128), rows(s2n, 128));
-    uint32_t* cred = q1.modmul(pk->ms_nn, ksel, cipher, rows(pk->ms_nn->one_words, 0, nullptr, 1));
-    uint32_t* cinv = q1.modinv(pk->ms_nn, ksel, rows(cred, 128), inv_ok1);
-    cies = q1.modexp_nn(pk, ksel, rows(cinv, 128), rows(e, 8), 8, false);
+    cies = q1.modexp_nn(pk, ksel, c_inverse(q1), rows(e, 8), 8, false);
   } else {
-    uint32_t* cred = q.modmul(pk->ms_nn, ksel, cipher, rows(pk->ms_nn->one_words, 0, nullptr, 1));
-    uint32_t* cinv = q.modinv(pk->ms_nn, ksel, rows(cred, 128), inv_ok1);
+    const Rows cinv = c_inverse(q);
     if (ctx->use_multiexp) {
-      uint32_t* m = q.modexp_nn2(pk, ksel, with_words(pr.s2, 64), Nrow, 64, rows(cinv, 128), rows(e, 8), 8);
+      uint32_t* m = q.modexp_nn2(pk, ksel, with_words(pr.s2, 64), Nrow, 64, cinv, rows(e, 8), 8);
       u2 = q.modmul(pk->ms_nn, ksel, rows(g1, 128), rows(m, 128));
     } else {
       uint32_t* s2n = q.modexp_nn(pk, ksel, with_words(pr.s2, 64), Nrow, 64, false);
       uint32_t* t2 = q.modmul(pk->ms_nn, ksel, rows(g1, 128), rows(s2n, 128));
-      uint32_t* cie = q.modexp_nn(pk, ksel, rows(cinv, 128), rows(e, 8), 8, false);
+      uint32_t* cie = q.modexp_nn(pk, ksel, cinv, rows(e, 8), 8, false);
       u2 = q.modmul(pk->ms_nn, ksel, rows(t2, 128), rows(cie, 128));
     }
   }
```

New measurement: 19000 (median of 6 runs). About the same (+0.3%).
